# randa1/orleans

Measured on AMD Instinct MI355X. Metric: routed grain messages/sec (node), higher is better.
Workload: dtype u32/u64 integer; 1 GPU; config3: Zipf(1.1) over 16M long-key grains, 256M messages in total (256M per GPU), 8-silo ring, stages 1-4; grains=16000000, messages_total=268435456, messages_per_gpu=268435456, silos=8, ring=balanced (silo generations [5, 135, 167, 28, 221, 184, 42, 48]), parallelism=directory sharded by ring range over 1 GPU(s)

## Files before the change

### include/orleans_route.h

```cpp
#ifndef ORLEANS_ROUTE_H
#define ORLEANS_ROUTE_H

#include <stddef.h>
#include <stdint.h>

#ifdef __cplusplus
extern "C" {
#endif

#define ORL_ABI_VERSION 1u
#define ORL_MAX_SILOS 255u
#define ORL_NULL_SILO 0xFFu
#define ORL_NO_ACT 0xFFFFFFFFu
#define ORL_MAX_RING 256u

#define ORL_OK 0
#define ORL_E_INVALID (-1)
#define ORL_E_NOMEM (-2)
#define ORL_E_DEVICE (-3)
#define ORL_E_CAPACITY (-4)
#define ORL_E_STATE (-5)
#define ORL_E_OVERFLOW (-6)

#define ORL_CAT_NONE 0u
// ... 459 lines not shown
    uint64_t max_recv;
    uint32_t chunks;
    uint32_t flags;
} orl_node_config;

typedef struct orl_node_result {
    uint64_t n_owned;
    uint64_t n_hosted;
    uint64_t n_forwarded;
    uint64_t n_sent_remote;
    uint32_t hop2;
    uint32_t n_segments;
    const uint32_t* route;
    const uint32_t* act;
    const uint32_t* order;
    const uint32_t* bucket_offsets;
} orl_node_result;

typedef struct orl_node orl_node;
int orl_node_unique_id(uint8_t id[ORL_NODE_ID_BYTES]);
int orl_node_create(orl_ctx* ctx, const orl_node_config* cfg, orl_node** out);
int orl_node_destroy(orl_node* node);
const char* orl_node_last_error(const orl_node* node);
int orl_node_set_timeout(orl_node* node, uint32_t ms);
int orl_node_route_batch_device(orl_node* node, const orl_msg_hdr* d_in, size_t n, uint32_t opts, orl_node_result* out,
                                void* stream);
int orl_node_route_batch_keyext_device(orl_node* node, const orl_msg_hdr* d_in, size_t n, uint32_t opts, const orl_ext_ref* d_ext,
                                       const uint8_t* d_blob, uint64_t blob_bytes, orl_node_result* out, void* stream);
int orl_node_fanout_batch_device(orl_node* node, const uint64_t* d_csr_off, const uint32_t* d_csr_tgt,
                                 const orl_grain_key* d_follower_keys, uint64_t follower_tcd, const uint32_t* d_pubs,
                                 const uint8_t* d_pub_silo, size_t n_pub, uint32_t opts, uint64_t* d_pub_offsets,
                                 uint64_t* total, orl_node_result* out, void* stream);
int orl_node_segment(const orl_node* node, uint32_t i, const void** d_records, uint64_t* count, uint32_t* width);
typedef struct orl_node_stats {
    uint32_t comm_count;
    uint32_t chunks;
    uint64_t bytes_sent[ORL_NODE_MAX_RANKS];
    uint64_t host_wait_us;
    uint64_t host_waits;
    uint32_t exchange_mode;
    uint32_t reserved;
} orl_node_stats;
#define ORL_NODE_MODE_SPLIT_COMM 0x1u
#define ORL_NODE_MODE_HEAD_STREAM 0x2u
int orl_node_get_stats(const orl_node* node, orl_node_stats* out);

#define ORL_NODE_HEAD_WORDS 16u
typedef struct orl_node_chunk_plan {
    uint32_t width;
    uint32_t rewrite;
    uint64_t send[ORL_NODE_MAX_RANKS];
    uint64_t recv[ORL_NODE_MAX_RANKS];
    uint64_t n_recv;
    uint32_t act_lane;
    uint32_t ext_lane;
} orl_node_chunk_plan;
int orl_node_plan_chunk(const uint64_t* heads, uint32_t nranks, uint32_t me, uint32_t written, uint64_t max_recv,
                        uint64_t* owned_total, orl_node_chunk_plan* out);
typedef struct orl_node_hop2_plan {
    uint32_t forward;
    uint32_t width;
    uint64_t send[ORL_NODE_MAX_RANKS];
    uint64_t recv[ORL_NODE_MAX_RANKS];
    uint64_t n_hosted;
    uint64_t n_forwarded;
} orl_node_hop2_plan;
int orl_node_plan_hop2(const uint64_t* heads, uint32_t nranks, uint32_t me, uint64_t n_owned, uint32_t width_mask,
                       uint64_t max_recv, orl_node_hop2_plan* out);

int orl_sync(orl_ctx* ctx);

#define ORL_Q_PROBE_FORM 1u
#define ORL_Q_FULL_UPLOADS 2u
#define ORL_Q_SLOT_PATCHES 3u
#define ORL_Q_DEVICE 4u
#define ORL_Q_N_ACT 5u
#define ORL_Q_MAX_BATCH 6u
#define ORL_Q_RANK_MODE 7u
#define ORL_Q_WIRE_DIGEST 8u
#define ORL_Q_PART_ERROR 9u
#define ORL_Q_HOT_KEY 10u
#define ORL_Q_HOT_BATCHES 11u
#define ORL_Q_STAGE4_ERROR 12u
int orl_ctx_query(orl_ctx* ctx, uint32_t what, uint64_t* value);
int orl_ctx_set_rank_mode(orl_ctx* ctx, uint32_t mode);

#define ORL_TIMING_SLOTS 256u
int orl_set_timing(orl_ctx* ctx, int enable);
int orl_timing_summary(const orl_ctx* ctx, uint32_t* n_batches, float* route_kernel_ms, float* bucket_ms,
                       float* total_ms);

#ifdef __cplusplus
}
#endif
#endif
```

### orleans_amd/_lib.py

```python
from __future__ import annotations

import ctypes as C
import os

import numpy as np

LIB_NAME = "liborleans_route.so"
LIB_PATH = os.path.join(os.path.dirname(os.path.abspath(__file__)), LIB_NAME)

ABI_VERSION = 1
NULL_SILO = 0xFF
NO_ACT = 0xFFFFFFFF

OK, E_INVALID, E_NOMEM, E_DEVICE, E_CAPACITY, E_STATE, E_OVERFLOW = 0, -1, -2, -3, -4, -5, -6

CAT_NONE, CAT_SYSTEM_TARGET, CAT_SYSTEM_GRAIN, CAT_GRAIN, CAT_CLIENT, CAT_KEYEXT_GRAIN = 0, 1, 2, 3, 4, 6

HDR_ADDRESS_COMPLETE = 0x01
HDR_HASH_VALID = 0x02

ST_HIT = 0
ST_NEW_PLACEMENT = 1
ST_SYSTEM_TARGET = 2
ST_ADDRESS_COMPLETE = 3
ST_OWNER_NULL = 4
ST_NO_SEED = 5
ST_CLIENT_UNREGISTERED = 6
ST_KEYEXT_UNRESOLVED = 7
ST_REMOTE_OWNER = 8
ST_PAST_TOTAL = 9

RF_NEW_PLACEMENT = 0x01
RF_LOOPBACK = 0x02
RF_OWNER_IS_SEED = 0x04

POLICY_PREFER_LOCAL = 0
POLICY_HASH_SPREAD = 1

OPT_EXCLUDE_IF_STOPPING = 0x1
OPT_NO_BUCKETS = 0x2
OPT_TOTAL_GIVEN = 0x4
SPLIT_REMOVE = 0x1
RF_CACHED = 0x08
RF_CACHE_STALE = 0x10
RF_STATELESS = 0x20
MAX_SW_TYPES = 8
SW_MAX_LOCAL = 8
SW_ADDED, SW_DUPLICATE, SW_UNSUPPORTED = 0, 1, 2
RING_CONSISTENT, RING_VBUCKETS = 0, 1
CACHE_EVICT_DEVICE, CACHE_EVICT_HOST = 0, 1
CACHE_NO_ETAG = -1
TICKS_PER_SECOND = 10_000_000
OUTQ_LOOPBACK, OUTQ_PING, OUTQ_SYSTEM, OUTQ_REJECT, OUTQ_OVERFLOW, OUTQ_UNKNOWN_SILO = (
    0xFFFFFFF0, 0xFFFFFFF1, 0xFFFFFFF2, 0xFFFFFFF3, 0xFFFFFFF4, 0xFFFFFFF5)
DEC_OK, DEC_UNSUPPORTED, DEC_MALFORMED, DEC_UNKNOWN_SILO, DEC_NO_TARGET, DEC_NO_SENDER = 0, 1, 2, 3, 4, 5
SENDER_FROM_HEADER = 0xFF
STAMP_OK, STAMP_COMPLETE, STAMP_SKIPPED, STAMP_UNSUPPORTED, STAMP_MALFORMED, STAMP_OVERFLOW = 0, 1, 2, 3, 4, 5
STAMP_MAX_GROWTH = 72
MERGE_INSERTED, MERGE_KEPT, MERGE_REPLACED, MERGE_SAME, MERGE_DUPLICATE, MERGE_UNSUPPORTED = 0, 1, 2, 3, 4, 5
DIR_NO_ETAG = -1
LUM_UNCHANGED, LUM_ABSENT, LUM_UPDATED, LUM_UPDATED_EMPTY, LUM_UNSUPPORTED = 0, 1, 2, 3, 4

ACT_CREATE, ACT_ACTIVATING, ACT_VALID, ACT_DEACTIVATING, ACT_INVALID, ACT_ABSENT = 0, 1, 2, 3, 4, 5
ACTF_REENTRANT, ACTF_RUNNING_SET, ACTF_RUNNING_RO, ACTF_STATELESS = 0x01, 0x02, 0x04, 0x08
MF_DIR_MASK, MF_REQUEST, MF_RESPONSE, MF_ONE_WAY = 0x03, 0, 1, 2
MF_READ_ONLY, MF_ALWAYS_INTERLEAVE, MF_EXPIRED = 0x04, 0x08, 0x10
(ADM_RUN, ADM_ENQUEUE, ADM_RESPONSE, ADM_OVERLOADED, ADM_INVALID, ADM_NONEXISTENT, ADM_EXPIRED,
 ADM_UNRESOLVED) = range(8)
TOK_NONE, TOK_DRAIN = 0xFFFFFFFF, 0xFFFFFFFE
WQ_RUN, WQ_DRAINED = 0, 1
(CMP_COMPLETIONS, CMP_PUMPS, CMP_DRAINS, CMP_IGNORED, CMP_UNDERFLOWS, CMP_RUN, CMP_DRAINED,
 CMP_WAITING) = range(8)
COLF_EXEMPT, COLF_CANCELLED = 0x01, 0x02
COL_MOVED, COL_SAME, COL_EXPIRED, COL_CANCELLED_DROPPED, COL_BAD_TIMEOUT = 1, 2, 3, 4, 5
COL_TOUCHED, COL_RULE1_ONLY, COL_RULE7_ONLY = 0, 6, 7
COL_BECAME_IDLE, COL_IGNORED, COL_COMPLETIONS = 0, 6, 7
(SCAN_CANDIDATES, SCAN_BAD_STATE, SCAN_KEPT_ALIVE, SCAN_ACTIVE, SCAN_NOT_STALE, SCAN_CONDEMNED, SCAN_CANCELLED_SKIPPED,
 SCAN_UNSCHEDULED) = range(8)
(SCHED_DONE, SCHED_EXEMPT, SCHED_AGE_ZERO, SCHED_BAD_TIMEOUT, SCHED_TICKETED, SCHED_IGNORED) = range(6)
(CANCEL_DONE, CANCEL_EXEMPT, CANCEL_NO_TICKET, CANCEL_EXPIRED, CANCEL_ALREADY, CANCEL_IGNORED) = range(6)

Q_PROBE_FORM, Q_FULL_UPLOADS, Q_SLOT_PATCHES, Q_DEVICE, Q_N_ACT, Q_MAX_BATCH, Q_RANK_MODE = 1, 2, 3, 4, 5, 6, 7
Q_WIRE_DIGEST = 8
Q_PART_ERROR = 9
PART_CACHED = 0x8
Q_HOT_KEY = 10
Q_HOT_BATCHES = 11
Q_STAGE4_ERROR = 12
MAX_WIRE_TYPES = 16
PART_LOOKBACK_FAILED = 0x4
PART_KEYEXT = 0x10
PART_EXT_FULL = 0x20

INS_INSERTED, INS_EXISTING, INS_INVALID_SILO, INS_REMOTE_OWNER, INS_OWNER_NULL, INS_UNSUPPORTED = 0, 1, 2, 3, 4, 5

KEY_DTYPE = np.dtype([("tcd", "<u8"), ("n0", "<u8"), ("n1", "<u8")])
EXT_REF_DTYPE = np.dtype([("off", "<u4"), ("len", "<u4")])
MSG_DTYPE = np.dtype([("tcd", "<u8"), ("n0", "<u8"), ("n1", "<u8"), ("sending_silo", "u1"), ("category", "u1"),
                      ("flags", "u1"), ("target_silo", "u1"), ("aux", "<u4")])
assert KEY_DTYPE.itemsize == 24 and MSG_DTYPE.itemsize == 32
ACT_STATE_DTYPE = np.dtype([("state", "u1"), ("flags", "u1"), ("reserved", "<u2"), ("num_running", "<u4"),
                            ("in_flight", "<u4"), ("waiting", "<u4")])
assert ACT_STATE_DTYPE.itemsize == 16


class orl_config(C.Structure):
    _fields_ = [("abi_version", C.c_uint32), ("device", C.c_int32), ("dir_capacity", C.c_uint64),
                ("n_act", C.c_uint32), ("placement_policy", C.c_uint32), ("max_batch", C.c_uint64)]


NODE_ID_BYTES = 128
TRANSPORT_RCCL, TRANSPORT_LOCAL = 0, 1
NODE_WIDE_ONLY = 0x1
NODE_SPLIT_COMM = 0x2
NODE_MODE_SPLIT_COMM = 0x1
NODE_MODE_HEAD_STREAM = 0x2
NODE_MAX_RANKS = 8
NODE_MAX_CHUNKS = 16
NODE_HEAD_WORDS = 16


class orl_node_config(C.Structure):
    _fields_ = [("abi_version", C.c_uint32), ("nranks", C.c_uint32), ("rank", C.c_uint32), ("transport", C.c_uint32),
                ("group_id", C.c_uint8 * NODE_ID_BYTES), ("rank_of_silo", C.c_uint8 * 256), ("max_batch", C.c_uint64),
                ("max_recv", C.c_uint64), ("chunks", C.c_uint32), ("flags", C.c_uint32)]


class orl_node_result(C.Structure):
    _fields_ = [("n_owned", C.c_uint64), ("n_hosted", C.c_uint64), ("n_forwarded", C.c_uint64),
                ("n_sent_remote", C.c_uint64), ("hop2", C.c_uint32), ("n_segments", C.c_uint32), ("route", C.c_void_p),
                ("act", C.c_void_p), ("order", C.c_void_p), ("bucket_offsets", C.c_void_p)]


class orl_node_stats(C.Structure):
    _fields_ = [("comm_count", C.c_uint32), ("chunks", C.c_uint32), ("bytes_sent", C.c_uint64 * NODE_MAX_RANKS),
                ("host_wait_us", C.c_uint64), ("host_waits", C.c_uint64), ("exchange_mode", C.c_uint32),
                ("reserved", C.c_uint32)]


class orl_cache_stats(C.Structure):
    _fields_ = [("entries", C.c_uint64), ("tombstones", C.c_uint64), ("evictions", C.c_uint64),
                ("evict_batches", C.c_uint64), ("rebuilds", C.c_uint64), ("host_fallbacks", C.c_uint64)]


class orl_cache_sweep(C.Structure):
    _fields_ = [("d_keys", C.c_void_p), ("d_etags", C.c_void_p), ("d_owner_offsets", C.c_void_p), ("d_counts", C.c_void_p)]


class orl_admit_limits(C.Structure):
    _fields_ = [("hard", C.c_int32), ("hard_stateless", C.c_int32)]


class orl_waitq_view(C.Structure):
    _fields_ = [("d_off", C.c_void_p), ("d_tok", C.c_void_p), ("d_act", C.c_void_p), ("d_mflags", C.c_void_p),
                ("d_running_tok", C.c_void_p), ("d_out_tok", C.c_void_p), ("d_out_act", C.c_void_p),
                ("d_out_mflags", C.c_void_p), ("d_out_kind", C.c_void_p), ("d_out_n", C.c_void_p),
                ("d_waiting_n", C.c_void_p)]


class orl_collector_view(C.Structure):
    _fields_ = [("d_ticket", C.c_void_p), ("d_became_idle", C.c_void_p), ("d_keep_alive_until", C.c_void_p),
                ("d_age_limit", C.c_void_p), ("d_cflags", C.c_void_p), ("d_out_act", C.c_void_p), ("d_out_n", C.c_void_p),
                ("quantum", C.c_int64), ("next_ticket", C.c_int64)]


class orl_node_chunk_plan(C.Structure):
    _fields_ = [("width", C.c_uint32), ("rewrite", C.c_uint32), ("send", C.c_uint64 * NODE_MAX_RANKS),
                ("recv", C.c_uint64 * NODE_MAX_RANKS), ("n_recv", C.c_uint64), ("act_lane", C.c_uint32),
                ("ext_lane", C.c_uint32)]


# ... 196 lines not shown
```

### orleans_amd/csrc/orl_api.cpp

```cpp
#include <hip/hip_runtime.h>

#include <algorithm>
#include <cstdarg>
#include <cstdlib>
#include <cstdio>
#include <cstring>
#include <map>
#include <mutex>
#include <new>
#include <string>
#include <tuple>
#include <vector>

#include "orl_internal.h"
#include "cache_adaptive.h"
#include "admit.h"
#include "waitq.h"
#include "collect.h"
#include "dir_versions.h"
#include "cache_evict.h"

using namespace orl;

namespace {
// ... 758 lines not shown
        return ORL_E_NOMEM;
    }
    c->mask = slots - 1;
    rebuild_params(c);
    if (cfg->device >= 0) {
        c->device_mode = true;
        auto bail = [&](hipError_t e, const char* what) {
            int r = hipfail(c, e, what);
            free_device(c);
            delete c;
            return r;
        };
        hipError_t e;
        if ((e = hipSetDevice(cfg->device)) != hipSuccess) return bail(e, "hipSetDevice");
        if ((e = hipStreamCreateWithFlags(&c->stream, hipStreamNonBlocking)) != hipSuccess) return bail(e, "hipStreamCreate");
        if ((e = (hipError_t)ensure_rank_mode(cfg->device)) != hipSuccess) return bail(e, "stage-4 rank self-check");
        if ((e = hipMalloc((void**)&c->d_table, slots * sizeof(DirSlot))) != hipSuccess) return bail(e, "hipMalloc(directory)");
        if ((e = hipMalloc((void**)&c->d_probe, slots * sizeof(ProbeSlot))) != hipSuccess) return bail(e, "hipMalloc(probe table)");
        if ((e = hipMalloc((void**)&c->d_probe_bad, 4)) != hipSuccess) return bail(e, "hipMalloc(probe flag)");
        if ((e = hipMalloc((void**)&c->d_probe8, slots * 8)) != hipSuccess) return bail(e, "hipMalloc(probe table 8)");
        const char* np = getenv("ORL_NO_PROBE16");
        c->probe_off = np && np[0] == '1';
        const char* np8 = getenv("ORL_NO_PROBE8");
        c->probe8_off = np8 && np8[0] == '1';
        if ((e = hipMalloc((void**)&c->d_claim, slots * 4)) != hipSuccess) return bail(e, "hipMalloc(claim)");
        if ((e = hipMemset(c->d_claim, 0xFF, slots * 4)) != hipSuccess) return bail(e, "hipMemset(claim)");
        if ((e = hipMalloc((void**)&c->d_vr_hash, ORL_MAX_SILOS * ORL_MAX_VBUCKETS_PER_SILO * 4)) != hipSuccess)
            return bail(e, "hipMalloc(vring)");
        if ((e = hipMalloc((void**)&c->d_vr_silo, ORL_MAX_SILOS * ORL_MAX_VBUCKETS_PER_SILO)) != hipSuccess)
            return bail(e, "hipMalloc(vring silos)");
        if ((e = hipMalloc((void**)&c->d_silo_hash, 1024)) != hipSuccess) return bail(e, "hipMalloc(silo hashes)");
        if ((e = hipMalloc((void**)&c->d_silo_known, 256)) != hipSuccess) return bail(e, "hipMalloc(silo known)");
        if ((e = hipMalloc((void**)&c->d_silo_tab, kSiloAddrSlots * sizeof(SiloAddrEntry))) != hipSuccess)
            return bail(e, "hipMalloc(silo addresses)");
        if ((e = hipMalloc((void**)&c->d_decode_flag, 4)) != hipSuccess) return bail(e, "hipMalloc(decode flag)");
        if ((e = hipMalloc((void**)&c->d_silo_words, 256 * 24)) != hipSuccess) return bail(e, "hipMalloc(silo words)");
        if ((e = hipMalloc((void**)&c->d_gt, kGrainTypeSlots * sizeof(GrainTypeEntry))) != hipSuccess)
            return bail(e, "hipMalloc(grain types)");
        if ((e = hipMalloc((void**)&c->d_gt_blob, kGrainTypeBlob)) != hipSuccess) return bail(e, "hipMalloc(grain type names)");
        if ((e = hipMalloc((void**)&c->d_dirstate, 32)) != hipSuccess) return bail(e, "hipMalloc(dirstate)");
        if ((e = hipMemset(c->d_dirstate, 0, 32)) != hipSuccess) return bail(e, "hipMemset(dirstate)");
        if ((e = hipMalloc((void**)&c->d_params, sizeof(RouteParams))) != hipSuccess) return bail(e, "hipMalloc(params)");
        if ((e = hipMalloc((void**)&c->d_rank_of_silo, 256)) != hipSuccess) return bail(e, "hipMalloc(rank map)");
        const uint64_t mb = std::max<uint64_t>(cfg->max_batch, kTile);
        const uint64_t tiles = (mb + kTile - 1) / kTile;
        c->s.max_batch = mb;
        c->s.max_tiles = tiles;
        c->s.device = cfg->device;
        c->s.gap_cap = env_gap_cap();
        c->s.fan_u = env_fan_u();
        const uint64_t rows = std::max<uint64_t>(tiles, std::min<uint64_t>(kMaxRouteRows, (mb + 255) / 256));
        const uint64_t hist_words = (1ull << kMaxDigitBits) * rows;
        if ((e = hipMalloc((void**)&c->s.pairs_a, mb * 8)) != hipSuccess) return bail(e, "hipMalloc(pairs_a)");
        if ((e = hipMalloc((void**)&c->s.pairs_b, mb * 8)) != hipSuccess) return bail(e, "hipMalloc(pairs_b)");
        if ((e = hipMalloc((void**)&c->s.idx_a, (mb + 1) * 4)) != hipSuccess) return bail(e, "hipMalloc(idx)");
        if ((e = hipMalloc((void**)&c->s.sorted_keys, mb * 4)) != hipSuccess) return bail(e, "hipMalloc(sorted)");
        if ((e = hipMalloc((void**)&c->s.tile_hist, hist_words * 4)) != hipSuccess) return bail(e, "hipMalloc(tile_hist)");
        if ((e = hipMalloc((void**)&c->s.tile_cnt, hist_words * 2)) != hipSuccess) return bail(e, "hipMalloc(tile_cnt)");
        const uint64_t scan_words = std::max<uint64_t>(std::max<uint64_t>(hist_words, mb + 1), (uint64_t)cfg->n_act + 2);
        if ((e = hipMalloc((void**)&c->s.scan_sums, ((scan_words + 4095) / 4096 + 2) * 4)) != hipSuccess) return bail(e, "hipMalloc(scan)");
        const BucketPlan bp = make_bucket_plan(cfg->n_act);
        const uint64_t seg_rows = std::max<uint64_t>(max_segments(mb, bp.hb), max_segments(std::min<uint64_t>(mb, (16u << 20) - 1), bp.hb));
        const uint64_t seg_words = bp.two_level ? seg_rows << bp.lb : 1;
        if ((e = hipMalloc((void**)&c->s.seg_hist, seg_words * 4)) != hipSuccess) return bail(e, "hipMalloc(seg_hist)");
        const uint64_t lb_cap = bp.two_level ? (seg_rows + kSegLbMinRows - 1) / kSegLbMinRows + 1 : 1;
        c->s.seg_lb_cap = (uint32_t)lb_cap;
        const uint64_t carry_words = bp.two_level ? lb_cap << bp.lb : 1;
        if ((e = hipMalloc((void**)&c->s.seg_carry, carry_words * 4)) != hipSuccess) return bail(e, "hipMalloc(seg_carry)");
        if ((e = hipMalloc((void**)&c->s.seg_meta, (lb_cap + 1) * 4)) != hipSuccess) return bail(e, "hipMalloc(seg_meta)");
        if ((e = hipMalloc((void**)&c->s.seg_lb, 2 * carry_words * 4)) != hipSuccess) return bail(e, "hipMalloc(seg_lb)");
        if ((e = hipMalloc((void**)&c->s.seg_lbctl, (4 + lb_cap) * 4)) != hipSuccess) return bail(e, "hipMalloc(seg_lbctl)");
        if ((e = hipMemset(c->s.seg_lbctl, 0, (4 + lb_cap) * 4)) != hipSuccess) return bail(e, "hipMemset(seg_lbctl)");
        if ((e = hipMalloc((void**)&c->s.bstart, 4097 * 4)) != hipSuccess) return bail(e, "hipMalloc(bstart)");
        c->s.fan_blk_cap = (uint32_t)((mb + 255) / 256 + 2);
        if ((e = hipMalloc((void**)&c->s.fan_blk, (size_t)c->s.fan_blk_cap * 4)) != hipSuccess) return bail(e, "hipMalloc(fan_blk)");
        if ((e = hipMalloc((void**)&c->s.sstart, 4098 * 4)) != hipSuccess) return bail(e, "hipMalloc(sstart)");
        if ((e = hipMalloc((void**)&c->d_dslot, mb * 4)) != hipSuccess) return bail(e, "hipMalloc(dslot)");
        if ((e = hipMalloc((void**)&c->d_dflag, mb)) != hipSuccess) return bail(e, "hipMalloc(dflag)");
        for (auto& L : c->s.lb) {
            if ((e = hipMalloc((void**)&L.state, 16 + ((mb + 2047) / 2048) * 64)) != hipSuccess) return bail(e, "hipMalloc(lb_state)");
            if ((e = hipMemset(L.state, 0, 16 + ((mb + 2047) / 2048) * 64)) != hipSuccess) return bail(e, "hipMemset(lb_state)");
            if ((e = hipEventCreateWithFlags(&L.ev, hipEventDisableTiming)) != hipSuccess) return bail(e, "hipEventCreate(lb)");
        }
        if (const char* lh = getenv("ORL_LSD_HOT"); lh && lh[0] == '1')
            if ((e = hipMalloc((void**)&c->s.lsd_hot, 16)) != hipSuccess) return bail(e, "hipMalloc(lsd_hot)");
        if ((e = hipMalloc((void**)&c->s.s4_err, 4)) != hipSuccess) return bail(e, "hipMalloc(s4_err)");
        if ((e = hipMemset(c->s.s4_err, 0, 4)) != hipSuccess) return bail(e, "hipMemset(s4_err)");
        if ((e = hipMalloc((void**)&c->s.gap_q, kGapQueueWords * 4)) != hipSuccess) return bail(e, "hipMalloc(gap_q)");
        if ((e = hipMemset(c->s.gap_q, 0, kGapQueueWords * 4)) != hipSuccess) return bail(e, "hipMemset(gap_q)");
        if ((e = hipMalloc((void**)&c->s.digits, mb)) != hipSuccess) return bail(e, "hipMalloc(digits)");
        if ((e = hipMalloc((void**)&c->s.col_sums, ((rows + 63) / 64) * (1ull << kMaxDigitBits) * 4)) != hipSuccess)
            return bail(e, "hipMalloc(col_sums)");
        if ((e = hipMalloc((void**)&c->s.col_tot, ((1ull << kMaxDigitBits) + 1) * 4)) != hipSuccess) return bail(e, "hipMalloc(col_tot)");
        if ((e = hipMalloc((void**)&c->s.hot, 16)) != hipSuccess) return bail(e, "hipMalloc(hot)");
        {
            const uint32_t init[4] = {0xFFFFFFFFu, 0xFFFFFFFFu, 0u, 0u};
            if ((e = hipMemcpy(c->s.hot, init, 16, hipMemcpyHostToDevice)) != hipSuccess) return bail(e, "hipMemcpy(hot)");
        }
        if ((e = hipMalloc((void**)&c->s.hot_bmax, (((uint64_t)cfg->n_act + 2 + 4095) / 4096 + 1) * 8)) != hipSuccess)
            return bail(e, "hipMalloc(hot_bmax)");
        if ((e = hipMalloc((void**)&c->s.pick_word, 8)) != hipSuccess) return bail(e, "hipMalloc(pick_word)");
        if ((e = hipMemset(c->s.pick_word, 0, 8)) != hipSuccess) return bail(e, "hipMemset(pick_word)");
        if ((e = hipMalloc((void**)&c->s.hot_rows, (rows + (rows + 63) / 64 + 1) * 4)) != hipSuccess) return bail(e, "hipMalloc(hot_rows)");
        if ((e = hipHostMalloc((void**)&c->s.hot_host, 8, hipHostMallocMapped | hipHostMallocCoherent)) != hipSuccess)
            return bail(e, "hipHostMalloc(hot_host)");
        c->s.hot_host[0] = 0xFFFFFFFFu;
        c->s.hot_host[1] = 1u;
        if ((e = hipHostGetDevicePointer((void**)&c->s.hot_host_dev, c->s.hot_host, 0)) != hipSuccess)
            return bail(e, "hipHostGetDevicePointer(hot_host)");
        if ((e = hipMalloc((void**)&c->st_off, ((size_t)cfg->n_act + 2) * 4)) != hipSuccess) return bail(e, "hipMalloc(offsets)");
    }
    *out = c;
    return ORL_OK;
}

int orl_ctx_destroy(orl_ctx* c) {
    if (!c) return ORL_E_INVALID;
    if (c->device_mode) {
        (void)hipSetDevice(c->cfg.device);
        (void)hipStreamSynchronize(c->stream);
        free_device(c);
    }
    delete c;
    return ORL_OK;
}

const char* orl_last_error(const orl_ctx* c) { return c ? c->err.c_str() : "null context"; }

int orl_silos_set(orl_ctx* c, uint32_t n, const uint8_t* running, const uint8_t* functional, const uint8_t* local,
                  uint32_t seed) {
    if (!c) return ORL_E_INVALID;
    if (n == 0 || n > ORL_MAX_SILOS) return fail(c, ORL_E_INVALID, "n_silos must be in [1, %u]", ORL_MAX_SILOS);
    if (seed != ORL_NULL_SILO && seed >= n) return fail(c, ORL_E_INVALID, "seed %u out of range", seed);
    for (auto& e : c->ring)
        if (e.second >= n) return fail(c, ORL_E_STATE, "ring holds silo %u >= n_silos", e.second);
    c->n_silos = n;
    c->running.assign(n, 1); c->functional.assign(n, 1); c->local.assign(n, 1);
    for (uint32_t i = 0; i < n; ++i) {
        if (running) c->running[i] = running[i] ? 1 : 0;
        if (functional) c->functional[i] = functional[i] ? 1 : 0;
        if (local) c->local[i] = local[i] ? 1 : 0;
    }
    c->seed = seed;
    rebuild_params(c);
    return ORL_OK;
}

int orl_ring_add_server(orl_ctx* c, uint32_t silo, int32_t hash) {
    if (!c) return ORL_E_INVALID;
    if (!silo_ok(c, silo)) return fail(c, ORL_E_INVALID, "silo %u not in the silo table (call orl_silos_set first)", silo);
    for (auto& e : c->ring)
        if (e.second == silo) return ORL_OK;
    if (c->ring.size() >= ORL_MAX_RING) return fail(c, ORL_E_CAPACITY, "ring full");
    int idx = -1;
    for (int i = 0; i < (int)c->ring.size(); ++i)
        if (c->ring[i].first < hash) idx = i;
    c->ring.insert(c->ring.begin() + (idx + 1), std::make_pair(hash, (uint8_t)silo));
    c->silo_hash[silo] = hash;
    c->silo_known[silo] = 1;
    c->silo_hash_dirty = true;
    rebuild_params(c);
    return ORL_OK;
}

int orl_silo_hash_set(orl_ctx* c, uint32_t silo, int32_t hash) {
    if (!c) return ORL_E_INVALID;
    if (silo >= 256) return fail(c, ORL_E_INVALID, "silo %u out of range", silo);
    c->silo_hash[silo] = hash;
    c->silo_known[silo] = 1;
    c->silo_hash_dirty = true;
    return ORL_OK;
}

int orl_ring_remove_server(orl_ctx* c, uint32_t silo) {
    if (!c) return ORL_E_INVALID;
    auto it = std::find_if(c->ring.begin(), c->ring.end(), [&](const std::pair<int32_t, uint8_t>& e) { return e.second == silo; });
    if (it != c->ring.end()) c->ring.erase(it);
    rebuild_params(c);
    return ORL_OK;
}

int orl_ring_get(const orl_ctx* c, int32_t* hashes, uint8_t* silos, uint32_t cap, uint32_t* n_out) {
    if (!c || !n_out) return ORL_E_INVALID;
    *n_out = (uint32_t)c->ring.size();
    for (uint32_t i = 0; i < c->ring.size() && i < cap; ++i) {
        if (hashes) hashes[i] = c->ring[i].first;
        if (silos) silos[i] = c->ring[i].second;
    }
    return ORL_OK;
// ... 2195 lines not shown
    ORL_HIP(c, hipDeviceSynchronize());
    (void)hipFree(c->d_csr_off); (void)hipFree(c->d_csr_tgt);
    c->d_csr_off = nullptr; c->d_csr_tgt = nullptr; c->csr_nodes = 0;
    ORL_HIP(c, hipMalloc((void**)&c->d_csr_off, (n_nodes + 1) * 8));
    ORL_HIP(c, hipMalloc((void**)&c->d_csr_tgt, std::max<size_t>(n_edges, 1) * 4));
    ORL_HIP(c, hipMemcpy(c->d_csr_off, off, (n_nodes + 1) * 8, hipMemcpyHostToDevice));
    if (n_edges) ORL_HIP(c, hipMemcpy(c->d_csr_tgt, tgt, n_edges * 4, hipMemcpyHostToDevice));
    c->csr_nodes = n_nodes;
    c->h_csr_off.assign(off, off + n_nodes + 1);
    return ORL_OK;
}

int orl_fanout_batch(orl_ctx* c, const uint32_t* pubs, const uint8_t* pub_silo, size_t n_pub, uint64_t follower_tcd,
                     uint32_t opts, uint64_t* pub_offsets, uint32_t* route, uint32_t* act, uint32_t* order, uint32_t* offsets,
                     size_t cap, uint64_t* n_out) {
    if (!c || !n_out || !pub_offsets) return ORL_E_INVALID;
    if (!c->device_mode) return fail(c, ORL_E_STATE, "context was created without a device (device < 0)");
    if (!c->d_csr_off) return fail(c, ORL_E_STATE, "no follower graph (orl_csr_set)");
    const bool buckets = !(opts & ORL_OPT_NO_BUCKETS);
    if (n_pub && (!pubs || !pub_silo)) return fail(c, ORL_E_INVALID, "null publisher array");
    if (!route || !act || (buckets && (!order || !offsets))) return fail(c, ORL_E_INVALID, "null output array");
    uint64_t total = 0;
    for (size_t p = 0; p < n_pub; ++p) {
        if (pubs[p] >= c->csr_nodes) return fail(c, ORL_E_INVALID, "publisher %u >= %zu nodes", pubs[p], c->csr_nodes);
        total += c->h_csr_off[pubs[p] + 1] - c->h_csr_off[pubs[p]];
    }
    *n_out = total;
    if (total > cap) return fail(c, ORL_E_CAPACITY, "fan-out emits %llu > cap %zu", (unsigned long long)total, cap);
    if (total > c->s.max_batch || n_pub + 1 > c->s.max_batch) return fail(c, ORL_E_CAPACITY, "fan-out larger than max_batch");
    ORL_HIP(c, hipSetDevice(c->cfg.device));
    const size_t in_bytes = n_pub * 5 + 16, out_words = 3 * std::max<uint64_t>(total, 1) + 1 + 2 * (n_pub + 1);
    if (int r = ensure_staging(c, in_bytes, out_words)) return r;
    uint32_t* d_pubs = reinterpret_cast<uint32_t*>(c->st_in);
    uint8_t* d_psilo = c->st_in + ((n_pub * 4 + 15) & ~size_t(15));
    uint32_t* d_route = c->st_out;
    uint32_t* d_act = d_route + total;
    uint32_t* d_order = d_act + total;
    uint64_t* d_poff = reinterpret_cast<uint64_t*>(d_order + total + (total & 1));
    hipStream_t st = c->stream;
    if (n_pub) {
        ORL_HIP(c, hipMemcpyAsync(d_pubs, pubs, n_pub * 4, hipMemcpyHostToDevice, st));
        ORL_HIP(c, hipMemcpyAsync(d_psilo, pub_silo, n_pub, hipMemcpyHostToDevice, st));
    }
    uint64_t n_dev = total;
    int r = orl_fanout_route_device(c, c->d_csr_off, c->d_csr_tgt, d_pubs, d_psilo, n_pub, follower_tcd, opts | ORL_OPT_TOTAL_GIVEN,
                                    d_poff, d_route, d_act, d_order, c->st_off, &n_dev, st);
    if (r) return r;
    if (total) {
        ORL_HIP(c, hipMemcpyAsync(route, d_route, total * 4, hipMemcpyDeviceToHost, st));
        ORL_HIP(c, hipMemcpyAsync(act, d_act, total * 4, hipMemcpyDeviceToHost, st));
        if (buckets) ORL_HIP(c, hipMemcpyAsync(order, d_order, total * 4, hipMemcpyDeviceToHost, st));
    }
    ORL_HIP(c, hipMemcpyAsync(pub_offsets, d_poff, (n_pub + 1) * 8, hipMemcpyDeviceToHost, st));
    if (buckets) ORL_HIP(c, hipMemcpyAsync(offsets, c->st_off, ((size_t)c->cfg.n_act + 2) * 4, hipMemcpyDeviceToHost, st));
    ORL_HIP(c, hipStreamSynchronize(st));
    return ORL_OK;
}

int orl_ctx_query(orl_ctx* c, uint32_t what, uint64_t* v) {
    if (!c || !v) return ORL_E_INVALID;
    switch (what) {
        case ORL_Q_DEVICE: *v = (uint64_t)(int64_t)c->cfg.device; return ORL_OK;
        case ORL_Q_N_ACT: *v = c->cfg.n_act; return ORL_OK;
        case ORL_Q_MAX_BATCH: *v = c->s.max_batch; return ORL_OK;
        case ORL_Q_WIRE_DIGEST: *v = c->hp.wire_digest; return ORL_OK;
        case ORL_Q_RANK_MODE: {
            if (!c->device_mode) return fail(c, ORL_E_STATE, "no device");
            std::lock_guard<std::mutex> lk(g_rank_mu);
            *v = (uint64_t)(int64_t)g_rank_state[c->cfg.device];
            return ORL_OK;
        }
        case ORL_Q_HOT_BATCHES:
            *v = c->s.hot_batches;
            return ORL_OK;
        case ORL_Q_HOT_KEY: {
            if (!c->device_mode) return fail(c, ORL_E_STATE, "no device");
            ORL_HIP(c, hipSetDevice(c->cfg.device));
            ORL_HIP(c, hipDeviceSynchronize());
            uint32_t w = 0;
            ORL_HIP(c, hipMemcpy(&w, c->s.hot + (c->s.hot_parity & 1u), 4, hipMemcpyDeviceToHost));
            *v = w;
            return ORL_OK;
        }
        case ORL_Q_PART_ERROR: {
            if (!c->device_mode) return fail(c, ORL_E_STATE, "no device");
            ORL_HIP(c, hipSetDevice(c->cfg.device));
            ORL_HIP(c, hipDeviceSynchronize());
            uint32_t any = 0;
            for (auto& L : c->s.lb) {
                uint32_t w = 0;
                ORL_HIP(c, hipMemcpy(&w, L.state + 1, 4, hipMemcpyDeviceToHost));
                if (w) ORL_HIP(c, hipMemset(L.state + 1, 0, 4));
                any |= w;
            }
            *v = any ? 1u : 0u;
            return ORL_OK;
        }
        case ORL_Q_STAGE4_ERROR: {
            if (!c->device_mode) return fail(c, ORL_E_STATE, "no device");
            ORL_HIP(c, hipSetDevice(c->cfg.device));
            ORL_HIP(c, hipDeviceSynchronize());
            uint32_t w = 0;
            ORL_HIP(c, hipMemcpy(&w, c->s.s4_err, 4, hipMemcpyDeviceToHost));
            if (w) ORL_HIP(c, hipMemset(c->s.s4_err, 0, 4));
            *v = w ? 1u : 0u;
            return ORL_OK;
        }
        default: break;
    }
    if (int r = sync_device_state(c)) return r;
    switch (what) {
        case ORL_Q_PROBE_FORM:
            *v = c->probe8_valid ? 8 : c->probe_valid ? 16 : (c->probe_dev || c->probe_dev_stale) ? 17 : 32;
            return ORL_OK;
        case ORL_Q_FULL_UPLOADS: *v = c->n_full_uploads; return ORL_OK;
        case ORL_Q_SLOT_PATCHES: *v = c->n_patches; return ORL_OK;
        default: return fail(c, ORL_E_INVALID, "unknown query %u", what);
    }
}

int orl_ctx_set_rank_mode(orl_ctx* c, uint32_t mode) {
    if (!c || mode > 1) return ORL_E_INVALID;
    if (!c->device_mode) return fail(c, ORL_E_STATE, "no device");
    std::lock_guard<std::mutex> lk(g_rank_mu);
    const int st = g_rank_state[c->cfg.device];
    if (mode == 0 && (st & 2)) return fail(c, ORL_E_STATE, "the LDS lane-order self-check failed on this device: ballot ranking only");
    ORL_HIP(c, hipSetDevice(c->cfg.device));
    ORL_HIP(c, hipDeviceSynchronize());
    ORL_HIP(c, (hipError_t)set_rank_mode(c->cfg.device, mode));
    g_rank_state[c->cfg.device] = (int)(mode | (st & 2));
    return ORL_OK;
}

int orl_set_timing(orl_ctx* c, int enable) {
    if (!c) return ORL_E_INVALID;
    if (!c->device_mode) return fail(c, ORL_E_STATE, "no device");
    if (enable && c->tev.empty()) {
        c->tev.assign(4 * (size_t)ORL_TIMING_SLOTS, nullptr);
        for (auto& e : c->tev) ORL_HIP(c, hipEventCreate(&e));
    }
    c->timing = enable != 0;
    c->tcount = 0;
    return ORL_OK;
}

int orl_timing_summary(const orl_ctx* cc, uint32_t* n_batches, float* route_ms, float* bucket_ms, float* total_ms) {
    orl_ctx* c = const_cast<orl_ctx*>(cc);
    if (!c) return ORL_E_INVALID;
    if (n_batches) *n_batches = c->tcount;
    if (c->tcount == 0) return fail(c, ORL_E_STATE, "no timed batch");
    ORL_HIP(c, hipEventSynchronize(c->tev[4 * (size_t)(c->tcount - 1) + 3]));
    double a = 0, b = 0, t = 0;
    for (uint32_t i = 0; i < c->tcount; ++i) {
        const hipEvent_t* ev = &c->tev[4 * (size_t)i];
        float x = 0, y = 0, z = 0;
        ORL_HIP(c, hipEventElapsedTime(&x, ev[1], ev[2]));
        ORL_HIP(c, hipEventElapsedTime(&y, ev[2], ev[3]));
        ORL_HIP(c, hipEventElapsedTime(&z, ev[0], ev[3]));
        a += x; b += y; t += z;
    }
    if (route_ms) *route_ms = (float)(a / c->tcount);
    if (bucket_ms) *bucket_ms = (float)(b / c->tcount);
    if (total_ms) *total_ms = (float)(t / c->tcount);
    return ORL_OK;
}

// ... 2 lines not shown
```

### orleans_amd/csrc/orl_internal.h

```cpp
#pragma once

#include <hip/hip_runtime.h>
#include <stddef.h>
#include <stdint.h>
#include <stdlib.h>

#include <algorithm>

#include "../../include/orleans_route.h"

namespace orl {

enum : uint8_t { SLOT_EMPTY = 0, SLOT_FULL = 1, SLOT_TOMB = 2,
                 SLOT_CLAIMING = 3,
                 SLOT_CLAIMED = 4 };

struct alignas(32) DirSlot {
    uint64_t tcd;
    uint64_t n0;
    uint64_t n1;
    uint32_t act;
    uint8_t silo;
    uint8_t state;
    uint16_t pad;
// ... 157 lines not shown
    while ((max_key >> total) != 0 && total < 32) ++total;
    if (total == 0) total = 1;
    BucketPlan p{};
    p.two_level = total <= 2 * (int)kMaxDigitBits;
    static const bool lb_ceil = [] { const char* e = getenv("ORL_LB_CEIL"); return e && e[0] == '1'; }();
    p.lb = total <= (int)kMaxDigitBits ? total : lb_ceil ? (total + 1) / 2 : total / 2;
    p.hb = total - p.lb;
    p.lsd = make_plan(max_key);
    return p;
}

inline uint32_t seg_elems(uint64_t) { return kSegChunk; }
inline uint64_t max_segments(uint64_t n, int hb) {
    const uint64_t s = seg_elems(n);
    return (n + s - 1) / s + std::min<uint64_t>(1ull << hb, n);
}

inline uint64_t pad_to(uint64_t v, uint64_t m) { return (v + m - 1) / m * m; }

struct Carve {
    uint8_t* p;
    explicit Carve(void* base) : p(static_cast<uint8_t*>(base)) {}
    template <class T = uint8_t>
    T* take(uint64_t bytes) {
        T* r = reinterpret_cast<T*>(p);
        p += bytes;
        return r;
    }
};

struct SegAgg;

struct DirView {
    const DirSlot* dir;
    uint64_t mask;
    const DirSlot* cache;
    uint64_t cmask;
    const ProbeSlot* probe = nullptr;
    const uint32_t* probe_bad = nullptr;
    const void* probe8 = nullptr;
    bool lru = false;
};

struct CacheAdaptive {
    int64_t* ttl;
    int64_t* last_refreshed;
    unsigned long long* seen;
    int32_t* etag;
};
__host__ __device__ inline CacheAdaptive cache_adaptive(const DirSlot* cache, uint64_t mask) {
    const uint64_t slots = mask + 1;
    uint8_t* p = reinterpret_cast<uint8_t*>(const_cast<DirSlot*>(cache + slots)) + (slots + 1) * 8;
    CacheAdaptive a;
    a.ttl = reinterpret_cast<int64_t*>(p);
    a.last_refreshed = a.ttl + slots;
    a.seen = reinterpret_cast<unsigned long long*>(a.last_refreshed + slots);
    a.etag = reinterpret_cast<int32_t*>(a.seen + slots);
    return a;
}
inline size_t cache_table_bytes(uint64_t slots, bool adaptive) {
    return slots * sizeof(DirSlot) + (slots + 1) * 8 + (adaptive ? slots * 28 : 0);
}
struct CacheFresh {
    const int32_t* etags = nullptr;
    int64_t now = 0;
    int64_t initial_ttl = 0;
    uint32_t on = 0;
    uint32_t pad = 0;
};

struct DirTags {
    int32_t* slot = nullptr;
    const int32_t* in = nullptr;
    const int32_t* draws = nullptr;
    int32_t* winner = nullptr;
};

struct ExtSlot {
    uint64_t tcd, n0, n1;
    uint32_t hash, act, off, len;
    uint8_t silo, state, pad[6];
};
static_assert(sizeof(ExtSlot) == 48, "KeyExt slot layout");

constexpr uint32_t kSegLbMinRows = 8;

struct Scratch {
    uint2* pairs_a;
    uint2* pairs_b;
    uint32_t* idx_a;
    uint32_t* sorted_keys;
    uint32_t* tile_hist;
    uint16_t* tile_cnt;
    uint32_t* scan_sums;
    uint32_t* col_sums;
    uint32_t* col_tot;
    uint8_t* digits;
    uint32_t* seg_hist;
    uint32_t* seg_carry;
    uint32_t* seg_meta;
    uint32_t* seg_lb = nullptr;
    uint32_t* seg_lbctl = nullptr;
    uint32_t seg_lb_cap = 0;
    mutable uint32_t seg_epoch = 0;
    uint32_t* bstart;
    uint32_t* sstart;
    uint32_t* gap_q;
    struct LbSet {
        uint32_t* state = nullptr;
        uint32_t ticket = 0;
        uint32_t epoch = 0;
        hipStream_t stream = nullptr;
        hipEvent_t ev = nullptr;
        uint64_t last = 0;
    };
    static constexpr int kLbSets = 2;
    LbSet lb[kLbSets];
    uint64_t lb_clock = 0;
    uint64_t max_batch;
    uint64_t max_tiles;
    int device = -1;
    uint32_t* hot = nullptr;
    mutable uint32_t hot_parity = 0;
    unsigned long long* hot_bmax = nullptr;
    unsigned long long* pick_word = nullptr;
    uint32_t* hot_rows = nullptr;
    uint32_t* lsd_hot = nullptr;
    uint32_t* hot_host = nullptr;
    uint32_t* hot_host_dev = nullptr;
    mutable uint64_t hot_batches = 0;
    uint32_t* fan_blk = nullptr;
    uint32_t fan_blk_cap = 0;
    uint32_t gap_cap = 4096;
    int fan_u = 1;
    uint32_t* s4_err = nullptr;
};

uint32_t env_gap_cap();
int env_fan_u();

int launch_hash(const orl_grain_key* d_keys, size_t n, uint32_t* d_out, void* stream);
int launch_rank_selfcheck(int device, int mode, uint32_t* ballot_out);
int set_rank_mode(int device, uint32_t ballot);
int launch_dir_patch(const uint32_t* d_idx, const DirSlot* d_slots, const ProbeSlot* d_p16, const uint2* d_p8, uint32_t n,
                     DirSlot* d_dir, ProbeSlot* d_probe, uint2* d_probe8, void* stream);
int launch_probe_build(const DirSlot* d_dir, uint64_t slots, const RouteParams* d_params, ProbeSlot* d_probe,
                       uint32_t* d_bad, void* stream);
int launch_route_bucket(const RouteParams* d_params, const DirView& dv,
                        const void* d_in, int fmt, size_t n, uint32_t opts, uint32_t n_act, uint32_t* d_route,
                        uint32_t* d_act, uint32_t* d_order, uint32_t* d_offsets, const Scratch& s, void* stream,
                        void* ev_route_begin, void* ev_route_end, const uint32_t* d_in_act = nullptr,
                        const SwView* sw = nullptr);
int launch_fanout_route_bucket(const RouteParams* d_params, const DirView& dv, const orl_msg_hdr* d_direct, size_t n_direct,
                               const uint64_t* d_csr_off, const uint32_t* d_csr_tgt, const orl_grain_key* d_follower_keys,
                               const uint32_t* d_pubs, const uint8_t* d_pub_silo, size_t n_pub, uint64_t follower_tcd,
                               uint32_t opts, uint32_t n_act, uint64_t* d_pub_offsets, uint32_t* d_route, uint32_t* d_act,
                               uint32_t* d_order, uint32_t* d_offsets, uint64_t* n_out, uint64_t max_out,
                               const Scratch& s, void* stream, void* ev_route_begin, void* ev_route_end);
int launch_fanout_expand(const uint64_t* d_csr_off, const uint32_t* d_csr_tgt, const orl_grain_key* d_follower_keys,
                         const uint32_t* d_pubs, const uint8_t* d_pub_silo, size_t n_pub, uint64_t follower_tcd, uint32_t opts,
                         uint64_t* d_pub_offsets, orl_msg_hdr* d_out, uint64_t* n_out, uint64_t cap, const Scratch& s,
                         void* stream);
int launch_dir_insert(const RouteParams* d_params, DirSlot* d_dir, uint64_t dir_mask, uint32_t* d_claim, uint64_t* d_cnt,
                      const orl_grain_key* d_keys, const uint32_t* d_acts, const uint8_t* d_silos, size_t n, uint32_t n_act,
                      uint32_t n_silos, uint32_t* d_slot, uint32_t* d_wact, uint8_t* d_wsilo, uint8_t* d_status, uint32_t* d_err,
                      void* stream, const DirTags& vt = DirTags{});
// ... 87 lines not shown
```

### orleans_amd/csrc/route_kernels.hip

```cpp
#include <hip/hip_runtime.h>

#include <cstdlib>

#include "dir_table_dev.h"

namespace orl {

namespace {

constexpr uint32_t kWaves = kRouteThreads / 64;

__device__ __forceinline__ uint32_t pack_route(uint32_t owner, uint32_t host, uint32_t st, uint32_t fl) {
    return (owner & 0xFFu) | ((host & 0xFFu) << 8) | ((st & 0xFFu) << 16) | ((fl & 0xFFu) << 24);
}

struct Msg {
    uint64_t tcd, n0, n1;
    uint32_t meta;
    uint32_t aux;
};

using u32x4 = unsigned int __attribute__((ext_vector_type(4)));

__device__ __forceinline__ Msg decode_hdr(const u32x4& a, const u32x4& b) {
// ... 451 lines not shown
                ra = counter_add<true>(&ca[w][0], d, 1u);
                rb = wave_rank_ballot<10, true>(&cb[w][0], d, active, lt);
            } else {
                ra = counter_add<false>(&ca[w][0], d, 1u);
                rb = wave_rank_ballot<3, false>(&cb[w][0], d, active, lt);
            }
            bad |= ra != rb;
        }
        __syncthreads();
    }
    if (bad) atomicOr(err, 1u);
}

__device__ __forceinline__ uint32_t packed_get(const uint32_t* row, uint32_t d) { return (row[d >> 1] >> ((d & 1u) << 4)) & 0xFFFFu; }

__global__ __launch_bounds__(256) void k_probe_build(const DirSlot* __restrict__ dir, uint64_t slots,
                                                     const RouteParams* __restrict__ gp, ProbeSlot* __restrict__ probe,
                                                     uint32_t* __restrict__ bad) {
    __shared__ uint64_t types[kProbeTypes];
    __shared__ uint32_t nt;
    if (threadIdx.x < kProbeTypes) types[threadIdx.x] = gp->probe_tcd[threadIdx.x];
    if (threadIdx.x == 0) nt = gp->n_probe_types;
    __syncthreads();
    const uint32_t ntypes = nt;
    bool miss = false;
    for (uint64_t i = (uint64_t)blockIdx.x * 256u + threadIdx.x; i < slots; i += (uint64_t)gridDim.x * 256u) {
        const u32x4* d4 = reinterpret_cast<const u32x4*>(dir + i);
        const u32x4 a = d4[0], b = d4[1];
        const uint32_t st = (b.w >> 8) & 0xFFu;
        const uint64_t tcd = (uint64_t)a.x | ((uint64_t)a.y << 32);
        uint32_t t = 0;
        u32x4 q = {0u, 0u, 0u, st == SLOT_EMPTY ? (uint32_t)SLOT_EMPTY : (uint32_t)SLOT_TOMB};
        if (st == SLOT_FULL) {
            while (t < ntypes && types[t] != tcd) ++t;
            if (t == ntypes || (a.z | a.w) != 0u) {
                miss = true;
                t = 0;
            }
            q = u32x4{b.x, b.y, b.z, (uint32_t)SLOT_FULL | ((b.w & 0xFFu) << 8) | (t << 16)};
        }
        reinterpret_cast<u32x4*>(probe)[i] = q;
    }
    if (miss) atomicOr(bad, 1u);
}

__global__ __launch_bounds__(256) void k_dir_patch(const uint32_t* __restrict__ idx, const DirSlot* __restrict__ slots,
                                                   const ProbeSlot* __restrict__ p16, const uint2* __restrict__ p8, uint32_t n,
                                                   DirSlot* __restrict__ dir, ProbeSlot* __restrict__ probe,
                                                   uint2* __restrict__ probe8) {
    const uint32_t k = blockIdx.x * 256u + threadIdx.x;
    if (k >= n) return;
    const uint32_t i = idx[k];
    dir[i] = slots[k];
    if (probe) probe[i] = p16[k];
    if (probe8) probe8[i] = p8[k];
}

__global__ __launch_bounds__(256) void k_hash(const orl_grain_key* __restrict__ keys, uint32_t n, uint32_t* __restrict__ out) {
    const uint32_t i = blockIdx.x * blockDim.x + threadIdx.x;
    if (i < n) out[i] = jenkins3(keys[i].type_code_data, keys[i].n0, keys[i].n1);
}

__device__ __forceinline__ void store_drop(uint32_t* p, uint32_t v) {
#ifdef ORL_ROUTE_STORE_SC1
    __hip_atomic_store(p, v, __ATOMIC_RELAXED, __HIP_MEMORY_SCOPE_AGENT);
#else
    __builtin_nontemporal_store(v, p);
#endif
}

template <int HB>
struct RouteSmem {
    RouteParams P;
    uint32_t hist[HB ? (1u << HB) : 1u];
    uint32_t hot;
};

constexpr uint32_t kNoHotKey = 0xFFFFFFFFu;

__device__ __forceinline__ uint32_t hot_key_of(const uint32_t* hot) {
    return hot ? __builtin_amdgcn_readfirstlane(__hip_atomic_load(hot, __ATOMIC_RELAXED, __HIP_MEMORY_SCOPE_AGENT)) : kNoHotKey;
}

__device__ __forceinline__ void wave_add_hot(uint32_t* dst, uint32_t mine) {
    uint32_t v = mine;
#pragma unroll
    for (uint32_t d = 32; d >= 1; d >>= 1) v += (uint32_t)__shfl_xor((int)v, (int)d, 64);
    if ((threadIdx.x & 63u) == 0 && v) atomicAdd(dst, v);
}

template <int FMT>
__device__ __forceinline__ Msg load_msg(const RouteParams& P, const void* __restrict__ in, uint32_t e) {
    if (FMT == 16) return load_wire(static_cast<const orl_wire_msg*>(in), e);
    if (FMT == 8) return load_narrow(P, static_cast<const orl_wire8*>(in), e);
    return load_hdr(static_cast<const orl_msg_hdr*>(in), e);
}

#ifndef ORL_ROUTE_PF
#define ORL_ROUTE_PF 1
#endif
template <int FMT>
__device__ __forceinline__ void pf_record(const void* __restrict__ in, uint32_t e, u32x4* region) {
    using lds_t = __attribute__((address_space(3))) void*;
    if (FMT == 32) {
        const u32x4* g = reinterpret_cast<const u32x4*>(static_cast<const orl_msg_hdr*>(in) + e);
        __builtin_amdgcn_global_load_lds(g, (lds_t)region, 16, 0, 2);
        __builtin_amdgcn_global_load_lds(g + 1, (lds_t)(region + 64), 16, 0, 2);
    } else if (FMT == 16) {
        __builtin_amdgcn_global_load_lds(static_cast<const orl_wire_msg*>(in) + e, (lds_t)region, 16, 0, 2);
    } else {
        const uint32_t* g = reinterpret_cast<const uint32_t*>(static_cast<const orl_wire8*>(in) + e);
        __builtin_amdgcn_global_load_lds(g, (lds_t)region, 4, 0, 2);
        __builtin_amdgcn_global_load_lds(g + 1, (lds_t)(reinterpret_cast<uint32_t*>(region) + 64), 4, 0, 2);
    }
}

template <int FMT>
__device__ __forceinline__ Msg pf_decode(const RouteParams& P, const u32x4* region, uint32_t lane) {
    if (FMT == 32) return decode_hdr(region[lane], region[64u + lane]);
    if (FMT == 16) return decode_wire(region[lane]);
    const uint32_t* r = reinterpret_cast<const uint32_t*>(region);
    return decode_narrow(P, (uint64_t)r[lane] | ((uint64_t)r[64u + lane] << 32));
}

#define ORL_SGPR80 __attribute__((amdgpu_num_sgpr(80)))
#ifndef ORL_ROUTE_ATTR
#define ORL_ROUTE_ATTR ORL_SGPR80
#endif
#ifndef ORL_FAN_ATTR
#define ORL_FAN_ATTR __attribute__((amdgpu_num_sgpr(96)))
#endif
#ifndef ORL_PART_ATTR
#define ORL_PART_ATTR
#endif
template <int HB, int FMT, int PW, bool CIN, bool LRU, bool SW>
__device__ __forceinline__ void route_body(const RouteParams* __restrict__ gp, const DirSlot* __restrict__ dir,
                                           uint64_t dmask, const DirSlot* __restrict__ cache, uint64_t cmask,
                                           const ProbeSlot* __restrict__ probe, const uint32_t* __restrict__ probe_bad,
                                           const void* __restrict__ in, uint32_t n, uint32_t excl,
                                           uint32_t* __restrict__ route, uint32_t* __restrict__ act_out,
                                           uint16_t* __restrict__ tile_cnt, uint32_t bins, uint32_t shift, uint32_t items,
                                           const uint32_t* __restrict__ hot_words, uint32_t* __restrict__ hot_rows,
                                           const uint32_t* __restrict__ in_act, const SwView* sw) {
    static_assert(!SW || PW == 0, "the stateless-worker forms read the 32-B directory table");
    __shared__ RouteSmem<HB> sm;
    constexpr bool HIST = HB > 0;
    constexpr bool PF = ORL_ROUTE_PF == 2 || (ORL_ROUTE_PF == 1 && FMT == 32);
    constexpr uint32_t PFW = FMT == 32 ? 128u : FMT == 16 ? 64u : 32u;
    __shared__ u32x4 pre[PF ? kWaves * PFW : 1];
    u32x4* const pregion = pre + (PF ? (threadIdx.x >> 6) * PFW : 0u);
    const uint32_t plane = threadIdx.x & 63u;
    uint32_t pend_e = 0, pend_rr = 0, pend_act = 0;
    bool pend = false;
    stage_params(&sm.P, gp);
    if (HIST)
        for (uint32_t b = threadIdx.x; b < bins; b += blockDim.x) sm.hist[b] = 0;
    if (threadIdx.x == 0) sm.hot = 0;
    __syncthreads();
    const uint32_t n_act = sm.P.n_act;
    const uint32_t hk = (HIST && hot_rows) ? hot_key_of(hot_words) : kNoHotKey;
    uint32_t hot_mine = 0;
    const bool use16 = PW == 16 && (probe_bad == nullptr || *probe_bad == 0u);
    const uint32_t base = blockIdx.x * (kRouteThreads * items) + threadIdx.x;
    if (PF) pf_record<FMT>(in, base < n ? base : n - 1u, pregion);
    for (uint32_t j = 0; j < items; ++j) {
        const uint32_t e = base + j * kRouteThreads;
        Msg m;
        if (PF) {
            asm volatile("s_waitcnt vmcnt(0)" ::: "memory");
            if (pend) {
                store_drop(route + pend_e, pend_rr);
                store_drop(act_out + pend_e, pend_act);
                pend = false;
            }
            m = pf_decode<FMT>(sm.P, pregion, plane);
            asm volatile("s_waitcnt lgkmcnt(0)" ::: "memory");
            if (j + 1u < items) {
                const uint32_t en = e + kRouteThreads;
                pf_record<FMT>(in, en < n ? en : n - 1u, pregion);
            }
        } else if (e < n) {
            m = load_msg<FMT>(sm.P, in, e);
        }
        uint32_t h = 0, own = 0, rf = 0, r = 0;
        uint64_t slot = 0, mask = dmask;
        u32x4 sa, sb;
        const u32x4* dir4 = reinterpret_cast<const u32x4*>(dir);
        if (PW == 8) {
            bool can = false;
            uint2 q;
            uint32_t cact = ORL_NO_ACT, vact = ORL_NO_ACT;
            if (e < n) {
                r = route_head(sm.P, m, excl != 0, h, own, rf);
                if (CIN) r = sender_cached(sm.P, m, in_act[e], h, own, rf, r, cact, vact);
                if (r == kNeedProbe) {
                    can = probe8_key(sm.P, m);
                    slot = dir_slot(h, dmask);
                    if (can) q = reinterpret_cast<const uint2*>(probe)[slot];
                }
            }
            const uint32_t kb = (uint32_t)m.n1;
            int st = 3;
            uint32_t fact = 0, fsilo = 0;
            if (r == kNeedProbe) st = can ? probe_slot8(q, kb, fact, fsilo) : 1;
            for (uint64_t step = 0; st == 2 && step < dmask; ++step) {
                slot = (slot + 1) & dmask;
                q = reinterpret_cast<const uint2*>(probe)[slot];
                st = probe_slot8(q, kb, fact, fsilo);
            }
            if (e < n) {
                uint32_t act = cact, rr = r;
                if (rr == kNeedProbe) {
                    rr = route_tail(sm.P, m, h, own, rf, st == 0, fact, fsilo, act, false);
                    if (CIN) rr = cached_verdict(sm.P, m, h, own, rf, rr, act, vact, st == 0, fact, fsilo);
                } else if (rr == kNeedProbeCache) {
                    rr = route_msg<LRU>(sm.P, dir, dmask, cache, cmask, m, excl != 0, act, e);
                }
                if (PF) {
                    pend_e = e, pend_rr = rr, pend_act = act, pend = true;
                } else {
                    store_drop(route + e, rr);
                    store_drop(act_out + e, act);
                }
                if (HIST) {
                    const uint32_t k = bucket_key(act, n_act);
                    if (k == hk) ++hot_mine;
                    else atomicAdd(&sm.hist[(k >> shift) & (bins - 1)], 1u);
                }
            }
            continue;
        }
        if (use16) {
            uint32_t mk = kNoType;
            uint32_t cact = ORL_NO_ACT, vact = ORL_NO_ACT;
            if (e < n) {
                r = route_head(sm.P, m, excl != 0, h, own, rf);
                if (CIN) r = sender_cached(sm.P, m, in_act[e], h, own, rf, r, cact, vact);
                if (r == kNeedProbe) {
                    mk = probe_type(sm.P, m);
                    slot = dir_slot(h, dmask);
                    if (mk != kNoType) sa = reinterpret_cast<const u32x4*>(probe)[slot];
                }
            }
            int st = 3;
            uint32_t fact = 0, fsilo = 0;
            if (r == kNeedProbe) st = mk == kNoType ? 1 : probe_slot16(sa, m.n1, mk, fact, fsilo);
            for (uint64_t step = 0; st == 2 && step < dmask; ++step) {
                slot = (slot + 1) & dmask;
                sa = reinterpret_cast<const u32x4*>(probe)[slot];
                st = probe_slot16(sa, m.n1, mk, fact, fsilo);
            }
            if (e < n) {
                uint32_t act = cact, rr = r;
                if (rr == kNeedProbe) {
                    rr = route_tail(sm.P, m, h, own, rf, st == 0, fact, fsilo, act, false);
                    if (CIN) rr = cached_verdict(sm.P, m, h, own, rf, rr, act, vact, st == 0, fact, fsilo);
                } else if (rr == kNeedProbeCache) {
                    rr = route_msg<LRU>(sm.P, dir, dmask, cache, cmask, m, excl != 0, act, e);
                }
                if (PF) {
                    pend_e = e, pend_rr = rr, pend_act = act, pend = true;
                } else {
                    store_drop(route + e, rr);
                    store_drop(act_out + e, act);
                }
                if (HIST) {
                    const uint32_t k = bucket_key(act, n_act);
                    if (k == hk) ++hot_mine;
                    else atomicAdd(&sm.hist[(k >> shift) & (bins - 1)], 1u);
                }
            }
            continue;
        }
        uint32_t cact = ORL_NO_ACT, vact = ORL_NO_ACT;
        if (e < n) {
            r = route_head<SW>(sm.P, m, excl != 0, h, own, rf, sw);
            if (SW && r == kStateless) r = sw_route(*sw, m, h, cact);
            else if (CIN) r = sender_cached(sm.P, m, in_act[e], h, own, rf, r, cact, vact);
            if (r >= kNeedProbeCache) {
                if (r == kNeedProbeCache) {
                    dir4 = reinterpret_cast<const u32x4*>(cache);
                    mask = cmask;
                }
                slot = dir_slot(h, mask);
                sa = dir4[2 * slot];
                sb = dir4[2 * slot + 1];
            }
        }
        int st = 3;
        uint32_t fact = 0, fsilo = 0;
        if (r >= kNeedProbeCache) st = probe_slot(sa, sb, m, fact, fsilo);
        for (uint64_t step = 0; st == 2 && step < mask; ++step) {
            slot = (slot + 1) & mask;
            sa = dir4[2 * slot];
            sb = dir4[2 * slot + 1];
            st = probe_slot(sa, sb, m, fact, fsilo);
        }
        if (LRU && r == kNeedProbeCache && st == 0) cache_touch(cache, cmask, slot, e);
        if (e < n) {
            uint32_t act = cact, rr = r;
            if (rr >= kNeedProbeCache) {
                const bool vc = rr == kNeedProbeCache;
                rr = route_tail(sm.P, m, h, own, rf, st == 0, fact, fsilo, act, vc);
                if (CIN && !vc) rr = cached_verdict(sm.P, m, h, own, rf, rr, act, vact, st == 0, fact, fsilo);
            }
            if (PF) {
                pend_e = e, pend_rr = rr, pend_act = act, pend = true;
            } else {
                store_drop(route + e, rr);
                store_drop(act_out + e, act);
            }
            if (HIST) {
                const uint32_t k = bucket_key(act, n_act);
                if (k == hk) ++hot_mine;
                else atomicAdd(&sm.hist[(k >> shift) & (bins - 1)], 1u);
            }
        }
    }
    if (PF && pend) {
        store_drop(route + pend_e, pend_rr);
        store_drop(act_out + pend_e, pend_act);
    }
    if (HIST) {
        if (hot_rows) wave_add_hot(&sm.hot, hot_mine);
        __syncthreads();
        store_count_row(tile_cnt + (size_t)blockIdx.x * bins, sm.hist, bins);
        if (hot_rows && threadIdx.x == 0) hot_rows[blockIdx.x] = sm.hot;
    }
}

template <int HB, int FMT, int PW, bool CIN = false, bool LRU = false>
__global__ __launch_bounds__(kRouteThreads) ORL_ROUTE_ATTR void k_route(const RouteParams* __restrict__ gp, const DirSlot* __restrict__ dir,
                                                         uint64_t dmask, const DirSlot* __restrict__ cache, uint64_t cmask,
                                                         const ProbeSlot* __restrict__ probe,
                                                         const uint32_t* __restrict__ probe_bad,
                                                         const void* __restrict__ in, uint32_t n,
                                                         uint32_t excl, uint32_t* __restrict__ route,
                                                         uint32_t* __restrict__ act_out, uint16_t* __restrict__ tile_cnt,
                                                         uint32_t bins, uint32_t shift, uint32_t items,
                                                         const uint32_t* __restrict__ hot_words, uint32_t* __restrict__ hot_rows,
                                                         const uint32_t* __restrict__ in_act) {
    route_body<HB, FMT, PW, CIN, LRU, false>(gp, dir, dmask, cache, cmask, probe, probe_bad, in, n, excl, route, act_out, tile_cnt,
                                             bins, shift, items, hot_words, hot_rows, in_act, nullptr);
}

template <int HB, int FMT, bool CIN = false, bool LRU = false>
__global__ __launch_bounds__(kRouteThreads) ORL_ROUTE_ATTR void k_route_sw(const RouteParams* __restrict__ gp, const DirSlot* __restrict__ dir,
                                                            uint64_t dmask, const DirSlot* __restrict__ cache, uint64_t cmask,
                                                            const void* __restrict__ in, uint32_t n,
                                                            uint32_t excl, uint32_t* __restrict__ route,
                                                            uint32_t* __restrict__ act_out, uint16_t* __restrict__ tile_cnt,
                                                            uint32_t bins, uint32_t shift, uint32_t items,
                                                            const uint32_t* __restrict__ hot_words, uint32_t* __restrict__ hot_rows,
                                                            const uint32_t* __restrict__ in_act, SwView sw) {
    route_body<HB, FMT, 0, CIN, LRU, true>(gp, dir, dmask, cache, cmask, nullptr, nullptr, in, n, excl, route, act_out, tile_cnt,
                                           bins, shift, items, hot_words, hot_rows, in_act, &sw);
}

constexpr uint32_t kScanChunk = 4096;

__device__ __forceinline__ uint32_t wave_incl_scan(uint32_t v) {
    const uint32_t lane = threadIdx.x & 63u;
#pragma unroll
    for (uint32_t d = 1; d < 64; d <<= 1) {
        const uint32_t t = __shfl_up(v, d, 64);
        if (lane >= d) v += t;
    }
    return v;
}

__device__ __forceinline__ uint32_t block_excl_scan(uint32_t v, uint32_t* wsum, uint32_t& total) {
    const uint32_t lane = threadIdx.x & 63u, w = threadIdx.x >> 6;
    const uint32_t incl = wave_incl_scan(v);
    if (lane == 63) wsum[w] = incl;
    __syncthreads();
    uint32_t pre = 0;
    total = 0;
    for (uint32_t i = 0; i < kWaves; ++i) {
        const uint32_t s = wsum[i];
        if (i < w) pre += s;
        total += s;
    }
    __syncthreads();
    return pre + incl - v;
}

__device__ __forceinline__ unsigned long long wave_max_u64(unsigned long long v) {
#pragma unroll
    for (uint32_t d = 32; d >= 1; d >>= 1) {
        const unsigned long long o = __shfl_xor(v, (int)d, 64);
        v = o > v ? o : v;
    }
    return v;
}

template <int SRC, uint32_t CH = kScanChunk>
__global__ __launch_bounds__(256) void k_scan_reduce(uint32_t* __restrict__ a, uint64_t m, uint32_t* __restrict__ sums,
                                                     const uint64_t* __restrict__ csr_off, const uint32_t* __restrict__ pubs,
                                                     uint64_t* __restrict__ pstart, unsigned long long* __restrict__ bmax = nullptr,
                                                     uint32_t nkeys = 0, uint32_t* __restrict__ zero_p = nullptr,
                                                     uint32_t zero_n = 0) {
    __shared__ uint32_t wsum[kWaves];
    __shared__ unsigned long long wmax[kWaves];
    for (uint32_t i = blockIdx.x * 256u + threadIdx.x; i < zero_n; i += gridDim.x * 256u) zero_p[i] = 0;
    const uint64_t base = (uint64_t)blockIdx.x * CH;
    constexpr uint32_t J = CH / 256;
    uint32_t s = 0;
    if (SRC != 1) {
        unsigned long long best = 0;
#pragma unroll
        for (uint32_t j = 0; j < J; ++j) {
            const uint64_t e = base + j * 256 + threadIdx.x;
            const uint32_t v = e < m ? a[e] : 0u;
            s += v;
            if (SRC == 2 && e < nkeys) {
                const unsigned long long c = ((unsigned long long)v << 32) | (uint32_t)e;
                best = c > best ? c : best;
            }
        }
        if (SRC == 2) {
            best = wave_max_u64(best);
            if ((threadIdx.x & 63u) == 0) wmax[threadIdx.x >> 6] = best;
            __syncthreads();
            if (threadIdx.x == 0) {
                for (uint32_t q = 1; q < kWaves; ++q) best = wmax[q] > best ? wmax[q] : best;
// ... 91 lines not shown
        unsigned long long best = 0;
        for (uint32_t i = threadIdx.x; i < gridDim.x; i += 256) best = bmax[i] > best ? bmax[i] : best;
        best = wave_max_u64(best);
        if ((threadIdx.x & 63u) == 0) wmax[threadIdx.x >> 6] = best;
        __syncthreads();
        if (threadIdx.x == 0) {
            for (uint32_t q = 1; q < kWaves; ++q) best = wmax[q] > best ? wmax[q] : best;
            const uint32_t c = (uint32_t)(best >> 32), k = (uint32_t)best;
            const uint32_t key = ((uint64_t)c * kHotShare >= n && c >= kHotMinCount) ? k : kNoHotKey;
            __hip_atomic_store(next_key, key, __ATOMIC_RELAXED, __HIP_MEMORY_SCOPE_AGENT);
            if (host_word) __hip_atomic_store(host_word, key, __ATOMIC_RELAXED, __HIP_MEMORY_SCOPE_SYSTEM);
        }
    }
    constexpr int E = (int)(CH / 256);
    const uint64_t base = (uint64_t)blockIdx.x * CH + (uint64_t)threadIdx.x * E;
    uint32_t v[E];
    load_e<E>(a, base, m, 0u, v);
    uint32_t s = 0;
#pragma unroll
    for (int i = 0; i < E; ++i) s += v[i];
    uint32_t pre;
    if (DIRECT) {
        uint32_t q = 0;
        for (uint32_t i = threadIdx.x; i < blockIdx.x; i += 256) q += sums[i];
        block_excl_scan(q, wsum, pre);
    } else {
        pre = sums[blockIdx.x];
    }
    uint32_t total;
    uint32_t run = block_excl_scan(s, wsum, total) + pre;
    uint32_t o[E];
#pragma unroll
    for (int i = 0; i < E; ++i) {
        o[i] = run;
        const bool live = base + i < m;
        if (WIDEN && live) out64[base + i] = add64 + run;
        if (WIDEN && fblk) {
            const uint32_t k0 = (run + kFanBlk - 1u) >> kFanBlkShift;
            uint32_t k1 = k0;
            if (live && base + i + 1 < m)
                k1 = (uint32_t)std::min<uint64_t>(((uint64_t)run + v[i] + kFanBlk - 1u) >> kFanBlkShift, fblk_cap);
            else if (live && m > 1 && k0 < fblk_cap)
                fblk[k0] = (uint32_t)(m - 2);
            const uint32_t cnt = k1 > k0 ? k1 - k0 : 0u;
            if (cnt <= kFblkSerial)
                for (uint32_t k = k0; k < k1; ++k) fblk[k] = (uint32_t)(base + i);
            uint64_t big = __ballot(cnt > kFblkSerial);
            while (big) {
                const int src = __builtin_ctzll(big);
                big &= big - 1;
                const uint32_t b0 = __shfl(k0, src, 64), b1 = __shfl(k1, src, 64);
                const uint32_t p = __shfl((uint32_t)(base + i), src, 64);
                for (uint32_t k = b0 + (threadIdx.x & 63u); k < b1; k += 64u) fblk[k] = p;
            }
        }
        run += v[i];
    }
    store_e<E>(a, base, m, o);
}

#ifndef ORL_STAGE4_NT
#define ORL_STAGE4_NT 1
#endif
__device__ __forceinline__ uint32_t ld_s4(const uint32_t* p) {
    if (ORL_STAGE4_NT) return __builtin_nontemporal_load(p);
    return *p;
}
__device__ __forceinline__ uint2 ld_s4(const uint2* p) {
    using v2 = unsigned int __attribute__((ext_vector_type(2)));
    if (ORL_STAGE4_NT) {
        const v2 v = __builtin_nontemporal_load(reinterpret_cast<const v2*>(p));
        return make_uint2(v.x, v.y);
    }
    return *p;
}
__device__ __forceinline__ uint4 ld_s4(const uint4* p) {
    if (ORL_STAGE4_NT) {
        const u32x4 v = __builtin_nontemporal_load(reinterpret_cast<const u32x4*>(p));
        return make_uint4(v.x, v.y, v.z, v.w);
    }
    return *p;
}

template <bool ACTS>
__global__ __launch_bounds__(256) void k_hist_pairs(const void* __restrict__ in, uint32_t n, uint32_t n_act, uint32_t shift,
                                                    uint32_t bins, uint16_t* __restrict__ tile_cnt,
                                                    const uint32_t* __restrict__ hot_words = nullptr,
                                                    uint32_t* __restrict__ hot_rows = nullptr,
                                                    const uint32_t* __restrict__ n_dev = nullptr) {
    if (n_dev) n = min(__builtin_amdgcn_readfirstlane(__hip_atomic_load(n_dev, __ATOMIC_RELAXED, __HIP_MEMORY_SCOPE_AGENT)), n);
    __shared__ uint32_t hist[1u << kMaxDigitBits];
    __shared__ uint32_t hot;
    for (uint32_t b = threadIdx.x; b < bins; b += 256) hist[b] = 0;
    if (threadIdx.x == 0) hot = 0;
    __syncthreads();
    const uint32_t hk = (ACTS && hot_rows) ? hot_key_of(hot_words) : kNoHotKey;
    uint32_t hot_mine = 0;
    const uint32_t base = blockIdx.x * kTile;
    uint32_t k[kItems];
    if (ACTS) {
#pragma unroll
        for (uint32_t j = 0; j < kItems; ++j) {
            const uint32_t e = base + j * 256 + threadIdx.x;
            k[j] = bucket_key(ld_s4(static_cast<const uint32_t*>(in) + (e < n ? e : n - 1)), n_act);
        }
#pragma unroll
        for (uint32_t j = 0; j < kItems; ++j)
            if (base + j * 256 + threadIdx.x < n) {
                if (k[j] == hk) ++hot_mine;
                else atomicAdd(&hist[(k[j] >> shift) & (bins - 1)], 1u);
            }
        if (hot_rows) wave_add_hot(&hot, hot_mine);
    } else {
        const uint32_t lane = threadIdx.x & 63u;
#pragma unroll
        for (uint32_t j = 0; j < kItems; ++j) {
            const uint32_t e = base + j * 256 + threadIdx.x;
            k[j] = ld_s4(static_cast<const uint2*>(in) + (e < n ? e : (n ? n - 1 : 0u))).x;
        }
#pragma unroll
        for (uint32_t j = 0; j < kItems; ++j) {
            const uint32_t e = base + j * 256 + threadIdx.x;
            const uint32_t d = e < n ? (k[j] >> shift) & (bins - 1) : 0xFFFFFFFFu;
            const uint32_t prev = __shfl_up(d, 1, 64);
            const bool head = lane == 0 || d != prev;
            const uint64_t heads = __ballot(head);
            if (head && d != 0xFFFFFFFFu) {
                const uint64_t after = lane == 63 ? 0ull : heads >> (lane + 1);
                const uint32_t len = after ? (uint32_t)__builtin_ctzll(after) + 1u : 64u - lane;
                atomicAdd(&hist[d], len);
            }
        }
    }
    __syncthreads();
    store_count_row(tile_cnt + (size_t)blockIdx.x * bins, hist, bins);
    if (ACTS && hot_rows && threadIdx.x == 0) hot_rows[blockIdx.x] = hot;
}

template <uint32_t Q = 4, uint32_t TW = 1>
__global__ __launch_bounds__(256) void k_hist_dig8_wave(const uint8_t* __restrict__ dig, uint32_t n, uint32_t bins,
                                                        uint32_t ntiles, uint16_t* __restrict__ tile_cnt,
                                                        const uint32_t* __restrict__ n_dev) {
    constexpr uint32_t PL = 16u * Q;
    if (n_dev) n = min(__builtin_amdgcn_readfirstlane(__hip_atomic_load(n_dev, __ATOMIC_RELAXED, __HIP_MEMORY_SCOPE_AGENT)), n);
    __shared__ uint32_t hist[kWaves][256];
    const uint32_t lane = threadIdx.x & 63u, w = threadIdx.x >> 6;
    const uint32_t tile0 = (blockIdx.x * kWaves + w) * TW;
    if (tile0 >= ntiles) return;
    uint32_t* h = hist[w];
    uint32_t v[TW][4 * Q];
#pragma unroll
    for (uint32_t tw = 0; tw < TW; ++tw) {
        const uint32_t e0 = (tile0 + tw) * (64u * PL) + lane * PL;
        if (e0 + PL <= n) {
            const uint4* p = reinterpret_cast<const uint4*>(dig + e0);
#pragma unroll
            for (uint32_t q = 0; q < Q; ++q) {
                const uint4 x = ld_s4(p + q);
                v[tw][4 * q] = x.x; v[tw][4 * q + 1] = x.y; v[tw][4 * q + 2] = x.z; v[tw][4 * q + 3] = x.w;
            }
        } else {
#pragma unroll
            for (uint32_t q = 0; q < 4 * Q; ++q) v[tw][q] = 0;
            for (uint32_t i = 0; e0 + i < n && i < PL; ++i) v[tw][i >> 2] |= (uint32_t)dig[e0 + i] << (8u * (i & 3u));
        }
    }
#pragma unroll
    for (uint32_t tw = 0; tw < TW; ++tw) {
        const uint32_t tile = tile0 + tw;
        if (tile >= ntiles) break;
#pragma unroll
        for (uint32_t q = 0; q < 4; ++q) h[lane + 64u * q] = 0;
        __builtin_amdgcn_wave_barrier();
        asm volatile("s_waitcnt lgkmcnt(0)" ::: "memory");
        const uint32_t e0 = tile * (64u * PL) + lane * PL;
        const uint32_t m = e0 < n ? min(PL, n - e0) : 0u;
        if (m) {
            uint32_t cur = v[tw][0] & 0xFFu, len = 1;
#pragma unroll
            for (uint32_t i = 1; i < PL; ++i) {
                if (i < m) {
                    const uint32_t b = (v[tw][i >> 2] >> (8u * (i & 3u))) & 0xFFu;
                    if (b == cur) {
                        ++len;
                    } else {
                        atomicAdd(&h[cur], len);
                        cur = b;
                        len = 1;
                    }
                }
            }
            atomicAdd(&h[cur], len);
// ... 72 lines not shown
        tot += v;
    }
    if (d < bins) {
#pragma unroll 8
        for (uint32_t c = c0; c < c1; ++c) {
            const uint32_t v = S[(size_t)c * bins + d];
            S[(size_t)c * bins + d] = pre;
            pre += v;
        }
        if (grp == 0) T[d] = tot;
    }
}

template <uint32_t NT>
__device__ void seg_plan_body(const uint32_t* __restrict__ col_tot, uint32_t nbk, uint32_t n, uint32_t seg,
                              uint32_t* __restrict__ bstart, uint32_t* __restrict__ sstart, uint32_t (*wsum)[16]);

constexpr uint32_t kSelfScanChunks = 64;
constexpr uint32_t kApplyCols = 64;
constexpr uint32_t kApplyGroups = 256 / kApplyCols;
constexpr uint32_t kApplyRows = kScanRows / kApplyGroups;

__global__ __launch_bounds__(256) void k_col_apply(const uint16_t* __restrict__ C, uint32_t* __restrict__ M, uint32_t ntiles, uint32_t bins,
                                                   const uint32_t* __restrict__ S, const uint32_t* __restrict__ T,
                                                   uint32_t row_step, uint32_t* __restrict__ hot_rows, uint32_t plan_n,
                                                   uint32_t plan_seg, uint32_t* __restrict__ plan_bstart,
                                                   uint32_t* __restrict__ plan_sstart) {
    __shared__ uint32_t red;
    __shared__ uint32_t gsum[kApplyGroups][kApplyCols];
    __shared__ uint32_t pw[3][16];
    if (plan_bstart && blockIdx.x == gridDim.x - 1) {
        if (blockIdx.y == 0) seg_plan_body<256>(T, bins, plan_n, plan_seg, plan_bstart, plan_sstart, pw);
        return;
    }
    if (hot_rows && blockIdx.y == gridDim.y - 1) {
        if (threadIdx.x >= 64) return;
        const uint32_t t = blockIdx.x * kScanRows + threadIdx.x;
        const uint32_t v = t < ntiles ? hot_rows[t] : 0u;
        const uint32_t ex = wave_incl_scan(v) - v + hot_rows[ntiles + blockIdx.x];
        if (t < ntiles) hot_rows[t] = ex;
        return;
    }
    const uint32_t col = threadIdx.x % kApplyCols, grp = threadIdx.x / kApplyCols;
    const uint32_t d0 = blockIdx.y * kApplyCols;
    const uint32_t d = d0 + col;
    const bool live = d < bins;
    uint32_t before = 0;
    for (uint32_t i = threadIdx.x; i < d0; i += 256) before += T[i];
    if (threadIdx.x == 0) red = 0;
    const uint32_t t0 = blockIdx.x * kScanRows + grp * kApplyRows;
    const uint32_t t1 = min(t0 + kApplyRows, ntiles);
    uint32_t v[kApplyRows];
#pragma unroll
    for (uint32_t k = 0; k < kApplyRows; ++k) v[k] = live && t0 + k < t1 ? C[(size_t)(t0 + k) * bins + d] : 0u;
    uint32_t rs = 0;
#pragma unroll
    for (uint32_t k = 0; k < kApplyRows; ++k) rs += v[k];
    gsum[grp][col] = rs;
    __syncthreads();
    atomicAdd(&red, before);
    const uint32_t tot_d = live ? T[d] : 0u;
    const uint32_t ex = wave_incl_scan(tot_d) - tot_d;
    uint32_t gpre = 0;
    for (uint32_t g = 0; g < grp; ++g) gpre += gsum[g][col];
    __syncthreads();
    if (!live) return;
    uint32_t run = red + ex + S[(size_t)blockIdx.x * bins + d] + gpre;
#pragma unroll
    for (uint32_t k = 0; k < kApplyRows; ++k) {
        if (t0 + k < t1 && (t0 + k) % row_step == 0) M[(size_t)(t0 + k) * bins + d] = run;
        run += v[k];
    }
}

__device__ __forceinline__ uint32_t xcd_tile(uint32_t b, uint32_t nb) {
#ifdef ORL_NO_XCD_TILE
    return b;
#endif
    const uint32_t q = nb / 8, r = nb % 8, x = b % 8;
    return (x < r ? x * (q + 1) : r * (q + 1) + (x - r) * q) + b / 8;
}

enum : int { IN_ACT = 0, IN_PAIR = 1 };
enum : int { OUT_PAIR = 0, OUT_FINAL = 1, OUT_LSD_PAIR = 4, OUT_PAIR_SMALL = 5, OUT_FINAL_GAPS = 6, OUT_PAIR_DIG = 7 };

__device__ __forceinline__ uint32_t wave_find_pub(const uint32_t* __restrict__ poff, uint32_t n_pub, uint32_t v) {
    const uint32_t lane = threadIdx.x & 63u;
    uint32_t lo = 0, hi = n_pub - 1;
    while (lo < hi) {
        const uint32_t step = (hi - lo + 64u) / 64u;
        const uint32_t sl = min(lo + lane * step, hi);
        const uint64_t le = __ballot(poff[sl] <= v);
        const uint32_t L = 63u - (uint32_t)__builtin_clzll(le);
        const uint32_t nlo = min(lo + L * step, hi);
        if (L < 63u) {
            const uint32_t nx = min(lo + (L + 1u) * step, hi);
            if (nx > nlo) hi = nx - 1u;
        }
        lo = nlo;
    }
    return lo;
}


template <int BITS>
constexpr uint32_t kDigitsPerThread = (1u << BITS) / 256u > 2u ? (1u << BITS) / 256u : 2u;

template <int BITS>
__device__ __forceinline__ void round_starts(uint32_t (*cnt)[(1u << BITS) / 2u], uint32_t* wsum,
                                             uint32_t (&tot)[kDigitsPerThread<BITS>],
                                             uint32_t (&start)[kDigitsPerThread<BITS>]) {
    constexpr uint32_t B = 1u << BITS, P = kDigitsPerThread<BITS>;
    const uint32_t d0 = threadIdx.x * P;
    uint32_t s = 0;
#pragma unroll
    for (uint32_t q = 0; q < P; q += 2) {
        uint32_t lo = 0, hi = 0;
        if (d0 + q < B) {
            const uint32_t k = (d0 + q) >> 1;
#pragma unroll
            for (uint32_t ww = 0; ww < kWaves; ++ww) {
                const uint32_t c = cnt[ww][k];
                cnt[ww][k] = lo | (hi << 16);
                lo += c & 0xFFFFu;
                hi += c >> 16;
            }
        }
        tot[q] = lo;
        tot[q + 1] = hi;
        s += lo + hi;
    }
    uint32_t total;
    uint32_t run = block_excl_scan(s, wsum, total);
#pragma unroll
    for (uint32_t q = 0; q < P; ++q) {
        start[q] = run;
        run += tot[q];
    }
#pragma unroll
    for (uint32_t q = 0; q < P; q += 2) {
        if (d0 + q < B) {
            const uint32_t add = start[q] | (start[q + 1] << 16);
#pragma unroll
            for (uint32_t ww = 0; ww < kWaves; ++ww) cnt[ww][(d0 + q) >> 1] += add;
        }
    }
}

constexpr uint32_t kScatterLdsFloor = 160u * 1024u / 4u + 16u;

template <int BITS, int ITEMS>
struct PassSmemCore {
    uint32_t cnt[kWaves][(1u << BITS) / 2u];
    uint2 stage[256 * ITEMS];
};

template <int BITS, int ITEMS>
struct PassSmem : PassSmemCore<BITS, ITEMS> {
    static constexpr uint32_t kCore = sizeof(PassSmemCore<BITS, ITEMS>);
    uint8_t pad[BITS == 10 && kCore < kScatterLdsFloor ? kScatterLdsFloor - kCore : 4];
};

constexpr uint32_t kFlEmpty = 0x0000FFFFu;
constexpr uint32_t kGapWave = 16, kGapChunk = 32768, kGapCap = 4096, kGapLds = 4096, kGapPer = 8, kGapBlock = 256 * kGapPer;

__device__ __forceinline__ void write_gap(uint32_t* __restrict__ offsets, uint32_t lo, uint32_t len, uint32_t val,
                                          uint32_t* __restrict__ q, uint32_t cap) {
    const uint32_t lane = threadIdx.x & 63u;
    if (len <= kGapWave)
        for (uint32_t b = 0; b < len; ++b) offsets[lo + b] = val;
    uint64_t m = __ballot(len > kGapWave);
    while (m) {
        const uint32_t src = (uint32_t)__builtin_ctzll(m);
        m &= m - 1;
        const uint32_t glo = (uint32_t)__shfl((int)lo, (int)src, 64);
        const uint32_t gl = (uint32_t)__shfl((int)len, (int)src, 64);
        const uint32_t gv = (uint32_t)__shfl((int)val, (int)src, 64);
        uint32_t done = 0;
        if (gl > kGapChunk) {
            const uint32_t pieces = gl / kGapChunk;
            uint32_t first = 0;
            if (lane == 0) first = atomicAdd(&q[0], pieces);
            first = (uint32_t)__shfl((int)first, 0, 64);
            const uint32_t took = first >= cap ? 0u : min(pieces, cap - first);
            for (uint32_t p = lane; p < took; p += 64) {
                uint32_t* t = q + 2 + 3 * (size_t)(first + p);
                t[0] = glo + p * kGapChunk;
                t[1] = kGapChunk;
                t[2] = gv;
            }
            done = took * kGapChunk;
        }
        for (uint32_t b = done + lane; b < gl; b += 64) offsets[glo + b] = gv;
    }
}

template <int BITS, int IN, int OUT, int ITEMS, int RM>
__global__ __launch_bounds__(256) void k_radix_pass(const void* __restrict__ in, uint32_t n_all, uint32_t n_act, uint32_t shift,
                                                    const uint32_t* __restrict__ tile_off, uint32_t row_step, uint32_t ntiles,
                                                    uint2* __restrict__ pair_out, uint32_t* __restrict__ order_out,
                                                    uint32_t* __restrict__ key_out, const uint32_t* __restrict__ hot_words,
                                                    const uint32_t* __restrict__ hot_rows, uint32_t* __restrict__ hot_idx,
                                                    uint32_t* __restrict__ offsets, uint32_t nb, uint32_t* __restrict__ gap_q,
                                                    uint32_t gap_cap, uint32_t dsel, const uint32_t* __restrict__ lsd_hot) {
    constexpr uint32_t B = 1u << BITS;
    constexpr uint32_t PER = kDigitsPerThread<BITS>;
    constexpr uint32_t TILE = 256u * ITEMS;
    constexpr bool HOTP = IN == IN_ACT && (OUT == OUT_PAIR || OUT == OUT_PAIR_DIG);
    const bool lh = IN != IN_ACT && lsd_hot != nullptr;
    const uint32_t lhk = lh ? __builtin_amdgcn_readfirstlane(lsd_hot[0]) : kNoHotKey;
    const uint32_t lhc = lh ? __builtin_amdgcn_readfirstlane(lsd_hot[1]) : 0u;
    const uint32_t n = lh ? min(__builtin_amdgcn_readfirstlane(lsd_hot[2]), n_all) : n_all;
    __shared__ PassSmem<BITS, ITEMS> sm;
    __shared__ uint32_t hotw[kWaves];
    const uint32_t rflags = rank_flags();
    const uint32_t lane = threadIdx.x & 63u, w = threadIdx.x >> 6;
    const uint32_t tile = xcd_tile(blockIdx.x, ntiles);
    for (uint32_t b = threadIdx.x; b < B / 2u; b += 256) {
#pragma unroll
        for (uint32_t q = 0; q < kWaves; ++q) sm.cnt[q][b] = 0;
    }
    const uint32_t tbase = tile * TILE;
    const uint32_t wbase = tbase + w * (ITEMS * 64u);
    uint32_t key[ITEMS], idx[ITEMS], rank[ITEMS];
#pragma unroll
    for (uint32_t j = 0; j < ITEMS; ++j) {
        const uint32_t e = wbase + j * 64u + lane;
        const uint32_t ec = e < n ? e : (n ? n - 1 : 0u);
        if (IN == IN_ACT) {
            key[j] = bucket_key(ld_s4(static_cast<const uint32_t*>(in) + ec), n_act);
            idx[j] = e;
        } else {
            const uint2 v = ld_s4(static_cast<const uint2*>(in) + ec);
            key[j] = v.x;
            idx[j] = v.y;
        }
    }
    const uint32_t hk = (HOTP && hot_rows) ? hot_key_of(hot_words) : kNoHotKey;
    bool ishot[ITEMS];
    uint32_t hrank[ITEMS];
    if (HOTP && hk != kNoHotKey) {
        uint32_t run = 0;
#pragma unroll
        for (uint32_t j = 0; j < ITEMS; ++j) {
            ishot[j] = wbase + j * 64u + lane < n && key[j] == hk;
            const uint64_t b = __ballot(ishot[j]);
            hrank[j] = run + (uint32_t)__popcll(b & lanes_below());
            run += (uint32_t)__popcll(b);
        }
        if (lane == 0) hotw[w] = run;
    }
    __syncthreads();
    {
        uint32_t dg[ITEMS];
#pragma unroll
        for (uint32_t j = 0; j < ITEMS; ++j) dg[j] = (key[j] >> shift) & (B - 1u);
        if (HOTP && hk != kNoHotKey) rank_steps<BITS, true, ITEMS, RM>(&sm.cnt[w][0], dg, n > wbase ? n - wbase : 0u, rank, rflags, ishot);
        else rank_steps<BITS, true, ITEMS, RM>(&sm.cnt[w][0], dg, n > wbase ? n - wbase : 0u, rank, rflags);
    }
    __syncthreads();
    const uint32_t* orow = tile_off + (size_t)tile * row_step * B;
    uint32_t tile_hot = 0;
    if (HOTP && hk != kNoHotKey) {
        uint32_t before = 0;
#pragma unroll
        for (uint32_t q = 0; q < kWaves; ++q) {
            before += q < w ? hotw[q] : 0u;
            tile_hot += hotw[q];
        }
        const uint32_t hb = hot_rows[(size_t)tile * row_step] + before;
#pragma unroll
        for (uint32_t j = 0; j < ITEMS; ++j)
            if (ishot[j] && hb + hrank[j] < n) hot_idx[hb + hrank[j]] = idx[j];
    }
    uint32_t tot[PER], start[PER], dl[PER];
    round_starts<BITS>(sm.cnt, reinterpret_cast<uint32_t*>(&sm.stage[0]), tot, start);
#pragma unroll
    for (uint32_t q = 0; q < PER; ++q) {
        const uint32_t b = threadIdx.x * PER + q;
        dl[q] = b < B ? orow[b] - start[q] : 0u;
    }
    __syncthreads();
#pragma unroll
    for (uint32_t j = 0; j < ITEMS; ++j) {
        if (wbase + j * 64u + lane < n && !(HOTP && hk != kNoHotKey && ishot[j])) {
            const uint32_t d = (key[j] >> shift) & (B - 1u);
            const uint32_t lpos = packed_get(sm.cnt[w], d) + rank[j];
            sm.stage[lpos] = make_uint2(key[j], idx[j]);
        }
    }
    __syncthreads();
    if (OUT == OUT_FINAL_GAPS) {
#pragma unroll
        for (uint32_t q = 0; q < PER; ++q) {
            const uint32_t d = threadIdx.x * PER + q;
            if (d < B)
                key_out[(size_t)tile * B + d] = tot[q] ? (sm.stage[start[q]].x & 0xFFFFu) |
                                                             ((sm.stage[start[q] + tot[q] - 1u].x & 0xFFFFu) << 16)
                                                       : kFlEmpty;
        }
    }
    uint32_t* delta = &sm.cnt[0][0];
#pragma unroll
    for (uint32_t q = 0; q < PER; ++q)
        if (threadIdx.x * PER + q < B) delta[threadIdx.x * PER + q] = dl[q];
    __syncthreads();
    const uint32_t cnt = (n > tbase ? min(n - tbase, TILE) : 0u) - tile_hot;
#pragma unroll
    for (uint32_t j = 0; j < ITEMS; ++j) {
        const uint32_t i = j * 256u + threadIdx.x;
        if (OUT == OUT_FINAL_GAPS) {
            uint32_t lo = 0, len = 0, g = 0;
            if (i < cnt) {
                const uint2 kv = sm.stage[i];
                const uint32_t d = (kv.x >> shift) & (B - 1u);
                g = delta[d] + i;
                if (g < n) {
                    const uint32_t ga = g + (kv.x > lhk && lhk != kNoHotKey ? lhc : 0u);
                    if (ga < n_all) order_out[ga] = kv.y;
                    if (i > 0) {
                        const uint32_t pk = sm.stage[i - 1u].x;
                        if (((pk >> shift) & (B - 1u)) == d && pk < kv.x) {
                            lo = pk + 1u;
                            len = lo < nb ? min(kv.x - pk, nb - lo) : 0u;
                        }
                    }
                }
            }
            write_gap(offsets, lo, len, g, gap_q, gap_cap);
            continue;
        }
        if (i < cnt) {
            const uint2 kv = sm.stage[i];
            const uint32_t k = kv.x;
            const uint32_t g = delta[(k >> shift) & (B - 1u)] + i;
            if (g >= n) continue;
            if (OUT == OUT_PAIR) {
                pair_out[g] = kv;
            } else if (OUT == OUT_PAIR_DIG) {
                pair_out[g] = kv;
                reinterpret_cast<uint8_t*>(key_out)[g] = (uint8_t)((k >> (dsel & 31u)) & ((1u << (dsel >> 8)) - 1u));
            } else {
                key_out[g] = k;
                order_out[g] = kv.y;
            }
        }
    }
}

static_assert(kGapQueueWords == 2 + 3 * (size_t)kGapCap, "gap queue size");

__global__ __launch_bounds__(256) void k_offsets_gaps(const uint32_t* __restrict__ sorted, uint32_t n, uint32_t nb,
                                                      uint32_t* __restrict__ offsets, uint32_t* __restrict__ q, uint32_t cap) {
    __shared__ uint32_t span[kGapLds];
    __shared__ uint32_t range[2];
    const uint64_t p0 = (uint64_t)blockIdx.x * kGapBlock, i0 = p0 + threadIdx.x * kGapPer;
    const uint32_t lane = threadIdx.x & 63u, top = nb - 1u;
    if (threadIdx.x == 0) {
        const uint64_t pl = min<uint64_t>(p0 + kGapBlock - 1u, n);
        range[0] = p0 == 0 ? 0u : min(sorted[p0 - 1], top) + 1u;
        range[1] = (pl < n ? min(sorted[pl], top) : top) + 1u;
    }
    uint32_t k[kGapPer];
    if (i0 + kGapPer <= n) {
        const uint4* p = reinterpret_cast<const uint4*>(sorted + i0);
#pragma unroll
        for (uint32_t j = 0; j < kGapPer / 4; ++j) {
            const uint4 v = ld_s4(p + j);
            k[4 * j] = v.x; k[4 * j + 1] = v.y; k[4 * j + 2] = v.z; k[4 * j + 3] = v.w;
        }
    } else {
#pragma unroll
        for (uint32_t j = 0; j < kGapPer; ++j) k[j] = (i0 + j < n) ? sorted[i0 + j] : top;
    }
    uint32_t lo = i0 == 0 ? 0u : i0 <= n ? min(sorted[i0 - 1], top) + 1u : nb;
    __syncthreads();
    const uint32_t r0 = range[0], r1 = range[1];
    const bool in_lds = r1 - r0 <= kGapLds;
    auto put = [&](uint32_t b, uint32_t v) {
        if (in_lds) span[b - r0] = v; else offsets[b] = v;
    };
#pragma unroll
    for (uint32_t j = 0; j < kGapPer; ++j) {
        const uint32_t hi = min(k[j], top) + 1u;
        const uint32_t len = hi > lo ? hi - lo : 0u, val = (uint32_t)(i0 + j);
        if (len <= kGapWave)
            for (uint32_t b = 0; b < len; ++b) put(lo + b, val);
        uint64_t m = __ballot(len > kGapWave);
        while (m) {
            const uint32_t src = (uint32_t)__builtin_ctzll(m);
            m &= m - 1;
            const uint32_t glo = (uint32_t)__shfl((int)lo, (int)src, 64);
            const uint32_t gl = (uint32_t)__shfl((int)len, (int)src, 64);
            const uint32_t gv = (uint32_t)__shfl((int)val, (int)src, 64);
            uint32_t done = 0;
            if (!in_lds && gl > kGapChunk) {
                const uint32_t pieces = gl / kGapChunk;
                uint32_t first = 0;
                if (lane == 0) first = atomicAdd(&q[0], pieces);
                first = (uint32_t)__shfl((int)first, 0, 64);
                const uint32_t took = first >= cap ? 0u : min(pieces, cap - first);
                for (uint32_t p = lane; p < took; p += 64) {
                    uint32_t* t = q + 2 + 3 * (size_t)(first + p);
                    t[0] = glo + p * kGapChunk;
                    t[1] = kGapChunk;
                    t[2] = gv;
                }
                done = took * kGapChunk;
            }
            for (uint32_t b = done + lane; b < gl; b += 64) put(glo + b, gv);
        }
        lo = hi > lo ? hi : lo;
    }
    if (in_lds) {
        __syncthreads();
        for (uint32_t b = threadIdx.x; b < r1 - r0; b += 256u) offsets[r0 + b] = span[b];
    }
// ... 1908 lines not shown
                                                        uint32_t* __restrict__ bucket) {
    const uint32_t e = blockIdx.x * 256u + threadIdx.x;
    if (e >= n) return;
    const Msg m = load_hdr(msgs, e);
    const uint32_t u = ((m.meta >> 16) & ORL_HDR_HASH_VALID) ? m.aux : jenkins3(m.tcd, m.n0, m.n1);
    const int32_t key = (int32_t)u, mod = (int32_t)n_buckets;
    bucket[e] = (uint32_t)(((key % mod) + mod) % mod);
}

inline uint32_t ceil_div(uint64_t a, uint64_t b) { return (uint32_t)((a + b - 1) / b); }

constexpr uint32_t kScanDirectChunks = 1024;
constexpr uint32_t kScanSmallChunk = 1024;

int scan_inplace(uint32_t* a, uint64_t m, const Scratch& s, hipStream_t st) {
    const uint32_t nb = ceil_div(m, kScanChunk);
    if (nb == 0) return 0;
    hipLaunchKernelGGL(k_scan_reduce<0>, dim3(nb), dim3(256), 0, st, a, m, s.scan_sums, nullptr, nullptr, nullptr, nullptr, 0u);
    if (nb <= kScanDirectChunks) {
        hipLaunchKernelGGL((k_scan_down<true, false>), dim3(nb), dim3(256), 0, st, a, m, s.scan_sums, nullptr, 0ull, nullptr, 0u,
                           nullptr, nullptr);
    } else {
        hipLaunchKernelGGL(k_scan_sums, dim3(1), dim3(256), 0, st, s.scan_sums, nb);
        hipLaunchKernelGGL((k_scan_down<false, false>), dim3(nb), dim3(256), 0, st, a, m, s.scan_sums, nullptr, 0ull, nullptr, 0u,
                           nullptr, nullptr);
    }
    return (int)hipGetLastError();
}

uint32_t* hot_cur(const Scratch& s) { return s.hot + (s.hot_parity & 1u); }

int scan_offsets_pick(uint32_t* a, uint64_t m, uint32_t nkeys, uint32_t n, const Scratch& s, hipStream_t st) {
    const uint32_t nb = ceil_div(m, kScanChunk);
    if (nb == 0) return 0;
    uint32_t* next = s.hot + ((s.hot_parity + 1u) & 1u);
    hipLaunchKernelGGL(k_scan_reduce<2>, dim3(nb), dim3(256), 0, st, a, m, s.scan_sums, nullptr, nullptr, nullptr, s.hot_bmax, nkeys);
    if (nb <= kScanDirectChunks) {
        hipLaunchKernelGGL((k_scan_down<true, false, true>), dim3(nb), dim3(256), 0, st, a, m, s.scan_sums, nullptr, 0ull,
                           s.hot_bmax, n, next, s.hot_host_dev);
    } else {
        hipLaunchKernelGGL(k_scan_sums, dim3(1), dim3(256), 0, st, s.scan_sums, nb);
        hipLaunchKernelGGL((k_scan_down<false, false, true>), dim3(nb), dim3(256), 0, st, a, m, s.scan_sums, nullptr, 0ull,
                           s.hot_bmax, n, next, s.hot_host_dev);
    }
    s.hot_parity ^= 1u;
    return (int)hipGetLastError();
}

constexpr uint32_t kMsdItems = 16;
constexpr uint32_t kMsdItemsSmall = 8;
constexpr uint32_t kMsdSmallMax = 8u << 20;
uint32_t msd_items(uint32_t n, uint32_t route_items) {
    static const bool off = [] { const char* e = getenv("ORL_MSD_SMALL"); return e && e[0] == '0'; }();
    return (!off && n <= kMsdSmallMax && route_items <= kMsdItemsSmall) ? kMsdItemsSmall : kMsdItems;
}
static_assert(kRouteThreads * kMsdItems <= 65535u, "a route tile's digit counts must fit the u16 count rows (store_count_row)");

__global__ void k_hot_finish(const uint32_t* __restrict__ hot_words, const uint32_t* __restrict__ hot_total, uint32_t nb,
                             uint32_t* __restrict__ offsets) {
    const uint32_t hk = hot_key_of(hot_words);
    if (threadIdx.x == 0 && hk < nb) offsets[hk] += *hot_total;
}

constexpr uint32_t kTailUnroll = 8;
__global__ __launch_bounds__(256) void k_hot_tail(const uint32_t* __restrict__ hot_words, const uint32_t* __restrict__ hot_total,
                                                  uint32_t n, uint32_t nkeys, const uint32_t* __restrict__ hot_idx,
                                                  const uint32_t* __restrict__ offsets, uint32_t* __restrict__ order) {
    const uint32_t hk = hot_key_of(hot_words);
    if (hk >= nkeys) return;
    const uint32_t cnt = *hot_total, off = offsets[hk];
    if (cnt > n || off > n - cnt) return;
    const uint32_t stride = gridDim.x * 256u;
    uint32_t i = blockIdx.x * 256u + threadIdx.x;
    for (; i + (kTailUnroll - 1) * stride < cnt; i += kTailUnroll * stride) {
        uint32_t v[kTailUnroll];
#pragma unroll
        for (uint32_t u = 0; u < kTailUnroll; ++u) v[u] = ld_s4(hot_idx + i + u * stride);
#pragma unroll
        for (uint32_t u = 0; u < kTailUnroll; ++u) order[off + i + u * stride] = v[u];
    }
    for (; i < cnt; i += stride) order[off + i] = hot_idx[i];
}

__global__ void k_lsd_hot_prep(const uint32_t* __restrict__ hot_words, const uint32_t* __restrict__ hot_total, uint32_t n,
                               uint32_t* __restrict__ out) {
    if (threadIdx.x != 0) return;
    const uint32_t hk = hot_key_of(hot_words);
    const uint32_t hc = hk == kNoHotKey ? 0u : min(*hot_total, n);
    out[0] = hk;
    out[1] = hc;
    out[2] = n - hc;
}

__global__ __launch_bounds__(256) void k_lsd_hot_fix(uint32_t* __restrict__ offsets, uint32_t nb, const uint32_t* __restrict__ lh) {
    const uint32_t hk = __builtin_amdgcn_readfirstlane(lh[0]), hc = __builtin_amdgcn_readfirstlane(lh[1]);
    if (hk == kNoHotKey || hc == 0) return;
    for (uint32_t b = hk + 1u + blockIdx.x * 256u + threadIdx.x; b < nb; b += gridDim.x * 256u) offsets[b] += hc;
}

__global__ __launch_bounds__(256) void k_lsd_pick(const uint32_t* __restrict__ offsets, uint32_t nkeys,
                                                  unsigned long long* __restrict__ pick_word) {
    __shared__ unsigned long long wbest[kWaves];
    unsigned long long best = 0;
    for (uint32_t b = blockIdx.x * 256u + threadIdx.x; b < nkeys; b += gridDim.x * 256u) {
        const unsigned long long c = (unsigned long long)(offsets[b + 1] - offsets[b]) << 32 | b;
        best = c > best ? c : best;
    }
    best = wave_max_u64(best);
    if ((threadIdx.x & 63u) == 0) wbest[threadIdx.x >> 6] = best;
    __syncthreads();
    if (threadIdx.x == 0) {
        for (uint32_t q = 1; q < kWaves; ++q) best = wbest[q] > best ? wbest[q] : best;
        if (best >> 32) atomicMax(pick_word, best);
    }
}

__global__ void k_lsd_pick_finish(unsigned long long* __restrict__ pick_word, uint32_t n, uint32_t* __restrict__ next_key,
                                  uint32_t* __restrict__ host_word) {
    if (threadIdx.x != 0) return;
    const unsigned long long best = *pick_word;
    *pick_word = 0;
    const uint32_t c = (uint32_t)(best >> 32), k = (uint32_t)best;
    const uint32_t key = ((uint64_t)c * kHotShare >= n && c >= kHotMinCount) ? k : kNoHotKey;
    __hip_atomic_store(next_key, key, __ATOMIC_RELAXED, __HIP_MEMORY_SCOPE_AGENT);
    if (host_word) __hip_atomic_store(host_word, key, __ATOMIC_RELAXED, __HIP_MEMORY_SCOPE_SYSTEM);
}

uint32_t max_route_items(uint32_t n_act) {
    const BucketPlan bp = make_bucket_plan(n_act);
    return bp.two_level && bp.hb > 0 ? kMsdItems : kItems;
}

uint32_t route_min_wgs() {
    static const uint32_t v = [] {
        const char* e = getenv("ORL_ROUTE_MIN_WG");
        const long x = e ? atol(e) : 0;
        return x > 0 ? (uint32_t)x : 2048u;
    }();
    return v;
}

bool fan_probe16() {
    static const bool on = [] {
        const char* e = getenv("ORL_FAN_PROBE16");
        return e && e[0] == '1';
    }();
    return on;
}

uint32_t fan_min_wgs() {
    static const uint32_t v = [] {
        const char* e = getenv("ORL_FAN_MIN_WG");
        const long x = e ? atol(e) : 0;
        return x > 0 ? (uint32_t)x : 4096u;
    }();
    return v;
}

uint32_t route_items(uint64_t n, uint32_t max_items, uint32_t min_wg = 0) {
    uint32_t items = max_items;
    if (min_wg == 0) min_wg = route_min_wgs();
    while (items > 1 && ceil_div(n, (uint64_t)kRouteThreads * items) < min_wg &&
           ceil_div(n, (uint64_t)kRouteThreads * (items >> 1)) <= kMaxRouteRows)
        items >>= 1;
    return items;
}

constexpr uint32_t kItems12 = 12;

template <int BITS>
void launch_pass_bits(int rm, int in, int out, const void* kin, uint32_t n, uint32_t n_act, uint32_t shift, const uint32_t* toff,
                      uint32_t row_step, uint32_t ntiles, uint2* pout, uint32_t* order, uint32_t* keys, hipStream_t st,
                      const uint32_t* hot_words, const uint32_t* hot_rows, uint32_t* hot_idx, uint32_t* offsets, uint32_t nb,
                      uint32_t* gap_q, uint32_t gap_cap, uint32_t dsel, const uint32_t* lsd_hot, uint32_t items) {
    const dim3 g(ntiles), b(256);
#define ORL_RP3(I, O, IT, R) hipLaunchKernelGGL((k_radix_pass<BITS, I, O, IT, R>), g, b, 0, st, kin, n, n_act, shift, toff,    \
                                                row_step, ntiles, pout, order, keys, hot_words, hot_rows, hot_idx, offsets, nb,   \
                                                gap_q, gap_cap, dsel, lsd_hot)
#define ORL_RP(I, O, IT) do { const int rm_ = rm; if (rm_ == kRmPlain) ORL_RP3(I, O, IT, kRmPlain);                      \
                              else if (rm_ == kRmHot) ORL_RP3(I, O, IT, kRmHot); else ORL_RP3(I, O, IT, kRmBallot); } while (0)
    if (in == IN_ACT) {
        switch (out) {
            case OUT_PAIR: ORL_RP(IN_ACT, OUT_PAIR, kMsdItems); break;
            case OUT_PAIR_SMALL: ORL_RP(IN_ACT, OUT_PAIR, kMsdItemsSmall); break;
            case OUT_LSD_PAIR: ORL_RP(IN_ACT, OUT_PAIR, kItems); break;
            case OUT_PAIR_DIG: ORL_RP(IN_ACT, OUT_PAIR_DIG, kItems); break;
            default: ORL_RP(IN_ACT, OUT_FINAL, kItems); break;
        }
    } else if (out == OUT_PAIR || out == OUT_LSD_PAIR) {
        ORL_RP(IN_PAIR, OUT_PAIR, kItems);
    } else if (out == OUT_PAIR_DIG) {
        if (items == kItems12) ORL_RP(IN_PAIR, OUT_PAIR_DIG, kItems12);
        else ORL_RP(IN_PAIR, OUT_PAIR_DIG, kItems);
    } else if (out == OUT_FINAL_GAPS) {
        if (items == kItems12) ORL_RP(IN_PAIR, OUT_FINAL_GAPS, kItems12);
        else ORL_RP(IN_PAIR, OUT_FINAL_GAPS, kItems);
    } else {
        ORL_RP(IN_PAIR, OUT_FINAL, kItems);
    }
#undef ORL_RP
#undef ORL_RP3
}

void launch_pass(int rm, int bits, int in, int out, const void* kin, uint32_t n, uint32_t n_act, uint32_t shift, const uint32_t* toff,
                 uint32_t row_step, uint32_t ntiles, uint2* pout, uint32_t* order, uint32_t* keys, hipStream_t st,
                 const uint32_t* hot_words = nullptr, const uint32_t* hot_rows = nullptr, uint32_t* hot_idx = nullptr,
                 uint32_t* offsets = nullptr, uint32_t nb = 0, uint32_t* gap_q = nullptr, uint32_t gap_cap = 0,
                 uint32_t dsel = 0, const uint32_t* lsd_hot = nullptr, uint32_t items = kItems) {
    switch (bits) {
#define ORL_CASE(B) case B: launch_pass_bits<B>(rm, in, out, kin, n, n_act, shift, toff, row_step, ntiles, pout, order, keys, st, \
                                                hot_words, hot_rows, hot_idx, offsets, nb, gap_q, gap_cap, dsel, lsd_hot, items); break;
        ORL_CASE(1) ORL_CASE(2) ORL_CASE(3) ORL_CASE(4) ORL_CASE(5) ORL_CASE(6)
        ORL_CASE(7) ORL_CASE(8) ORL_CASE(9) ORL_CASE(10) ORL_CASE(11)
#undef ORL_CASE
        default: break;
    }
}

void col_scan(uint32_t* M, uint32_t ntiles, uint32_t bins, uint32_t row_step, const Scratch& s, hipStream_t st,
              uint32_t* hot_rows = nullptr, uint32_t plan_n = 0, uint32_t plan_seg = 0, bool self_sums = false) {
    const uint16_t* C = s.tile_cnt;
    const uint32_t nch = ceil_div(ntiles, kScanRows);
    const uint32_t cb = ceil_div(bins, 256);
    const uint32_t hy = hot_rows ? 1u : 0u;
    if (!self_sums || hot_rows || nch > kSelfScanChunks)
        hipLaunchKernelGGL(k_col_sum, dim3(nch, cb + hy), dim3(256), 0, st, C, ntiles, bins, s.col_sums, hot_rows);
    hipLaunchKernelGGL(k_col_scan, dim3(ceil_div(bins, kColScanCols) + hy), dim3(256), 0, st, s.col_sums, nch, bins, s.col_tot,
                       hot_rows, ntiles);
    const bool plan = plan_n > 0;
    hipLaunchKernelGGL(k_col_apply, dim3(nch + (plan ? 1u : 0u), ceil_div(bins, kApplyCols) + hy), dim3(256), 0, st, C, M, ntiles,
                       bins, s.col_sums, s.col_tot, row_step, hot_rows, plan_n, plan_seg, plan ? s.bstart : nullptr,
                       plan ? s.sstart : nullptr);
}

struct RouteHist {
    bool on;
    uint32_t bins, shift;
};

RouteHist route_hist(uint32_t n_act) {
    const BucketPlan bp = make_bucket_plan(n_act);
    if (bp.two_level) return {bp.hb > 0, 1u << bp.hb, (uint32_t)bp.lb};
    return {true, 1u << bp.lsd.bits[0], (uint32_t)bp.lsd.shift[0]};
}

uint32_t next_seg_epoch(const Scratch& s) {
    s.seg_epoch = (s.seg_epoch + 1u) & 0x3FFFFFFFu;
    if (s.seg_epoch == 0) s.seg_epoch = 1;
    return s.seg_epoch;
}

template <int LB>
void launch_seg_bits(int in, const void* kin, uint32_t n, uint32_t n_act, uint32_t nbk, uint32_t seg, uint32_t grid,
                     uint32_t* d_order, uint32_t* d_offsets, const Scratch& s, hipStream_t st, bool hot, bool pick) {
    const uint32_t nb = n_act + 2;
    const uint32_t solo = s.hot_host && !__atomic_load_n(s.hot_host + 1, __ATOMIC_ACQUIRE) ? 1u : 0u;
    const uint32_t direct = solo && !hot ? 1u : 0u;
    unsigned long long* pick_word = direct && pick ? s.pick_word : nullptr;
    uint32_t* next_key = s.hot + ((s.hot_parity + 1u) & 1u);
    uint32_t* skew_host = s.hot_host_dev ? s.hot_host_dev + 1 : nullptr;
    const uint32_t fgrid = std::max(nbk, std::min(solo ? ceil_div(grid, kLbRows) : grid, solo ? 2048u : 1024u));
    const uint32_t epoch = solo ? next_seg_epoch(s) : 0u;
#define ORL_SF(I) hipLaunchKernelGGL((k_seg_count_scan<LB, I>), dim3(fgrid), dim3(256), 0, st, kin, n, n_act, nbk, nb, seg, s.bstart, \
                                     s.sstart, s.seg_hist, d_offsets, solo, direct, skew_host, pick_word, n_act + 1, s.seg_carry,  \
                                     s.seg_meta, s.seg_lb, s.seg_lbctl, s.seg_lb_cap, epoch, s.s4_err)
#define ORL_SS3(I, R) hipLaunchKernelGGL((k_seg_scatter<LB, I, R>), dim3(grid), dim3(256), 0, st, kin, n, n_act, nbk, seg, s.bstart,\
                                         s.sstart, s.seg_hist, d_offsets, nb, n, s.seg_carry, s.seg_meta, d_order,         \
                                         solo ? kLbRows : kScanRows,                                                         \
                                         pick_word, next_key, s.hot_host_dev)
#define ORL_SS(I) do { const int rm_ = host_rm(s.device); if (rm_ == kRmPlain) ORL_SS3(I, kRmPlain); else if (rm_ == kRmHot)             \
                           ORL_SS3(I, kRmHot); else ORL_SS3(I, kRmBallot); } while (0)
    if (in == IN_ACT) ORL_SF(IN_ACT); else ORL_SF(IN_PAIR);
    const uint32_t cb = ceil_div(1u << LB, 256);
    const uint32_t nch = ceil_div(grid, kScanRows);
    if (!solo) {
        hipLaunchKernelGGL((k_seg_scan<LB>), dim3(nch, cb), dim3(256), 0, st, s.seg_hist, s.sstart, nbk, nb,
                           s.seg_carry, s.seg_meta, d_offsets);
        hipLaunchKernelGGL((k_seg_carry<LB>), dim3(ceil_div(1u << LB, 16)), dim3(256), 0, st, s.sstart, nbk, nb, s.seg_meta,
                           s.seg_carry, d_offsets);
    }
    const uint32_t* hw = hot_cur(s);
    if (hot) hipLaunchKernelGGL(k_hot_finish, dim3(1), dim3(64), 0, st, hw, s.col_tot + nbk, nb, d_offsets);
    if (pick && !direct)
        scan_offsets_pick(d_offsets, nb, n_act + 1, n, s, st);
    else if (pick)
        s.hot_parity ^= 1u;
    else if (!direct)
        scan_inplace(d_offsets, nb, s, st);
    if (in == IN_ACT) ORL_SS(IN_ACT); else ORL_SS(IN_PAIR);
    if (hot)
        hipLaunchKernelGGL(k_hot_tail, dim3(std::min<uint32_t>(ceil_div(n / 4u, 256u * kTailUnroll), 2048u)), dim3(256), 0, st,
                           hw, s.col_tot + nbk, n, n_act + 1, s.sorted_keys, d_offsets, d_order);
#undef ORL_SF
#undef ORL_SS
#undef ORL_SS3
}

void launch_seg(int lb, int in, const void* kin, uint32_t n, uint32_t n_act, uint32_t nbk, uint32_t seg, uint32_t grid,
                uint32_t* d_order, uint32_t* d_offsets, const Scratch& s, hipStream_t st, bool hot, bool pick) {
    switch (lb) {
#define ORL_CASE(B) case B: launch_seg_bits<B>(in, kin, n, n_act, nbk, seg, grid, d_order, d_offsets, s, st, hot, pick); break;
        ORL_CASE(1) ORL_CASE(2) ORL_CASE(3) ORL_CASE(4) ORL_CASE(5) ORL_CASE(6)
        ORL_CASE(7) ORL_CASE(8) ORL_CASE(9) ORL_CASE(10) ORL_CASE(11)
#undef ORL_CASE
        default: break;
    }
}

bool lsd_gaps(const RadixPlan& plan, uint64_t n, uint32_t n_act) {
    return plan.shift[plan.passes - 1] <= 16 && n >= 2ull * (n_act + 2ull);
}

bool hot_path_on(uint64_t n, uint32_t n_act, const Scratch& s) {
    static const bool off = [] {
        const char* e = getenv("ORL_NO_HOT");
        return e && e[0] == '1';
    }();
    if (off || !s.hot || n < kHotMinBatch) return false;
    const BucketPlan bp = make_bucket_plan(n_act);
    if (bp.two_level) return bp.hb > 0;
    return s.lsd_hot && lsd_gaps(bp.lsd, n, n_act);
}

bool hot_known(const Scratch& s) {
    const bool on = s.hot_host && __atomic_load_n(s.hot_host, __ATOMIC_ACQUIRE) != kNoHotKey;
    s.hot_batches += on ? 1u : 0u;
    return on;
}

int bucket_after_route(const uint32_t* d_act, uint32_t n, uint32_t n_act, uint32_t route_items, uint32_t* d_order,
                       uint32_t* d_offsets, const Scratch& s, hipStream_t st, bool hot, bool pick = false,
                       bool self_cols = false) {
    const BucketPlan bp = make_bucket_plan(n_act);
    const uint32_t ntiles = ceil_div(n, kTile);
    const uint32_t nb = n_act + 2;
    const uint32_t nrows0 = ceil_div(n, kRouteThreads * route_items);
    if (bp.two_level) {
        const uint32_t mitems = msd_items(n, route_items);
        const uint32_t row_step0 = mitems / route_items;
        const uint32_t ntiles = ceil_div(n, kRouteThreads * mitems);
        const uint32_t nbk = 1u << bp.hb;
        const uint32_t seg = seg_elems(n);
        const uint32_t grid = (uint32_t)max_segments(n, bp.hb);
        const void* kin = d_act;
        if (bp.hb > 0) {
            col_scan(s.tile_hist, nrows0, nbk, row_step0, s, st, hot ? s.hot_rows : nullptr, n, seg, self_cols);
            launch_pass(host_rm(s.device), bp.hb, IN_ACT, mitems == kMsdItems ? OUT_PAIR : OUT_PAIR_SMALL, d_act, n, n_act, (uint32_t)bp.lb, s.tile_hist,
                        row_step0, ntiles, s.pairs_a, nullptr, nullptr, st, hot ? hot_cur(s) : nullptr, hot ? s.hot_rows : nullptr,
                        hot ? s.sorted_keys : nullptr);
            kin = s.pairs_a;
        }
        if (bp.hb == 0)
            hipLaunchKernelGGL(k_seg_plan, dim3(1), dim3(1024), 0, st, nullptr, nbk, n, seg, s.bstart, s.sstart);
        launch_seg(bp.lb, bp.hb == 0 ? IN_ACT : IN_PAIR, kin, n, n_act, nbk, seg, grid, d_order, d_offsets, s, st, hot && bp.hb > 0, (hot || pick) && bp.hb > 0);
        return (int)hipGetLastError();
    }
    const RadixPlan& plan = bp.lsd;
    const uint32_t row_step0 = kItems / route_items;
    const bool gaps = lsd_gaps(plan, n, n_act);
    const bool lhot = hot && gaps && s.lsd_hot;
    const bool lpick = pick && gaps && s.lsd_hot;
    const uint32_t* hw = hot_cur(s);
    uint2* pbuf[2] = {s.pairs_a, s.pairs_b};
    uint8_t* dig = reinterpret_cast<uint8_t*>(s.sorted_keys);
    bool have_dig = false;
    bool t12 = gaps && plan.passes >= 2;
    for (int p = 1; p < plan.passes; ++p) t12 = t12 && plan.bits[p] <= 8;
    const uint32_t ntiles12 = ceil_div(n, kRouteThreads * kItems12);
    const uint32_t ntl = t12 ? ntiles12 : ntiles;
    for (int p = 0; p < plan.passes; ++p) {
        const uint32_t bins = 1u << plan.bits[p];
        const uint32_t row_step = (p == 0) ? row_step0 : 1u;
        const uint32_t ntp = p == 0 ? ntiles : ntl;
        const uint32_t nrows = (p == 0) ? nrows0 : ntl;
        const uint32_t* n_dev = (p > 0 && lhot) ? s.lsd_hot + 2 : nullptr;
        if (p > 0 && t12)
            hipLaunchKernelGGL((k_hist_dig8_wave<3, 1>), dim3(ceil_div(ntl, kWaves)), dim3(256), 0, st, dig, n, bins, ntl,
                               s.tile_cnt, n_dev);
        else if (p > 0 && have_dig)
            hipLaunchKernelGGL((k_hist_dig8_wave<4, 1>), dim3(ceil_div(ntiles, kWaves)), dim3(256), 0, st, dig, n, bins, ntiles,
                               s.tile_cnt, n_dev);
        else if (p > 0)
            hipLaunchKernelGGL(k_hist_pairs<false>, dim3(ntiles), dim3(256), 0, st, pbuf[(p - 1) & 1], n, n_act,
                               (uint32_t)plan.shift[p], bins, s.tile_cnt, nullptr, nullptr, n_dev);
        col_scan(s.tile_hist, nrows, bins, row_step, s, st, (p == 0 && lhot) ? s.hot_rows : nullptr, 0, 0, p == 0 && self_cols);
        if (p == 0 && lhot)
            hipLaunchKernelGGL(k_lsd_hot_prep, dim3(1), dim3(64), 0, st, hw, s.col_tot + bins, n, s.lsd_hot);
        const bool last = p == plan.passes - 1;
        const bool wdig = !last && plan.bits[p + 1] <= 8;
        const void* kin = (p == 0) ? static_cast<const void*>(d_act) : static_cast<const void*>(pbuf[(p - 1) & 1]);
        const int out = !last ? (wdig ? OUT_PAIR_DIG : OUT_LSD_PAIR) : gaps ? OUT_FINAL_GAPS : OUT_FINAL;
        const uint32_t dsel = wdig ? (uint32_t)plan.shift[p + 1] | ((uint32_t)plan.bits[p + 1] << 8) : 0u;
        const bool hp = p == 0 && lhot;
        launch_pass(host_rm(s.device), plan.bits[p], p == 0 ? IN_ACT : IN_PAIR, out, kin, n, n_act, (uint32_t)plan.shift[p],
                    s.tile_hist, row_step, ntp, pbuf[p & 1], d_order, wdig ? reinterpret_cast<uint32_t*>(dig) : s.sorted_keys,
                    st, hp ? hw : nullptr, hp ? s.hot_rows : nullptr, hp ? s.idx_a : nullptr, d_offsets, nb, s.gap_q, s.gap_cap,
                    dsel, (p > 0 && lhot) ? s.lsd_hot : nullptr, (p > 0 && t12) ? kItems12 : kItems);
        have_dig = wdig;
    }
    if (gaps) {
        const int lp = plan.passes - 1;
        const uint32_t ntiles = ntl;
        const uint32_t bins = 1u << plan.bits[lp], nch = ceil_div(ntiles, kScanRows);
        const bool bt = bins % kBoundCols == 0;
        if (bt) hipLaunchKernelGGL(k_bound_last_t, dim3(nch), dim3(256), 0, st, s.sorted_keys, ntiles, bins, s.col_sums);
        else hipLaunchKernelGGL(k_bound_last, dim3(nch), dim3(256), 0, st, s.sorted_keys, ntiles, bins, s.col_sums);
        hipLaunchKernelGGL(k_bound_scan, dim3(ceil_div(bins, kColScanCols)), dim3(256), 0, st, s.col_sums, nch, bins,
                           s.sorted_keys + (size_t)ntiles * bins);
        if (bt)
            hipLaunchKernelGGL(k_bound_apply_t, dim3(nch), dim3(256), 0, st, s.sorted_keys, s.tile_hist, s.col_sums, ntiles, bins,
                               (uint32_t)plan.shift[lp], nb, d_offsets, s.gap_q, s.gap_cap);
        else
            hipLaunchKernelGGL(k_bound_apply, dim3(nch), dim3(256), 0, st, s.sorted_keys, s.tile_hist, s.col_sums, ntiles, bins,
                               (uint32_t)plan.shift[lp], nb, d_offsets, s.gap_q, s.gap_cap);
        hipLaunchKernelGGL(k_offsets_tail, dim3(bins), dim3(256), 0, st, s.col_tot, s.sorted_keys + (size_t)ntiles * bins,
                           (uint32_t)plan.bits[lp], (uint32_t)plan.shift[lp], nb, d_offsets, s.gap_q, s.gap_cap);
        if (lhot) {
            hipLaunchKernelGGL(k_lsd_hot_fix, dim3(std::min<uint32_t>(ceil_div(nb, 256u * 16u), 2048u)), dim3(256), 0, st, d_offsets,
                               nb, s.lsd_hot);
            hipLaunchKernelGGL(k_hot_tail, dim3(std::min<uint32_t>(ceil_div(n / 4u, 256u * kTailUnroll), 2048u)), dim3(256), 0,
                               st, hw, s.lsd_hot + 1, n, n_act + 1, s.idx_a, d_offsets, d_order);
        }
        if (lpick) {
            hipLaunchKernelGGL(k_lsd_pick, dim3(std::min<uint32_t>(ceil_div(n_act + 1u, 256u * 16u), 512u)), dim3(256), 0, st,
                               d_offsets, n_act + 1u, s.pick_word);
            hipLaunchKernelGGL(k_lsd_pick_finish, dim3(1), dim3(64), 0, st, s.pick_word, n, s.hot + ((s.hot_parity + 1u) & 1u),
                               s.hot_host_dev);
            s.hot_parity ^= 1u;
        }
        return (int)hipGetLastError();
    }
    hipLaunchKernelGGL(k_offsets_gaps, dim3(ceil_div(n + 1, kGapBlock)), dim3(256), 0, st, s.sorted_keys, n, nb,
                       d_offsets, s.gap_q, s.gap_cap);
    hipLaunchKernelGGL(k_offsets_long, dim3(256), dim3(256), 0, st, d_offsets, s.gap_q, s.gap_cap);
    return (int)hipGetLastError();
}

}

uint32_t env_gap_cap() {
    const char* e = getenv("ORL_GAP_CAP");
    const long v = e ? atol(e) : (long)kGapCap;
    return (uint32_t)std::min<long>(std::max<long>(v, 0), (long)kGapCap);
}


int env_fan_u() {
    const char* e = getenv("ORL_FAN_U");
    const int v = e ? atoi(e) : kFanIlp;
    return v == 4 ? 4 : v == 2 ? 2 : 1;
}

int launch_rank_selfcheck(int device, int mode, uint32_t* ballot_out) {
    uint32_t* d_err = nullptr;
    uint32_t err = 0;
    hipError_t e = hipMalloc((void**)&d_err, 4);
    if (e == hipSuccess) e = hipMemset(d_err, 0, 4);
    if (e == hipSuccess) {
        hipLaunchKernelGGL(k_rank_selfcheck, dim3(1024), dim3(256), 0, nullptr, 0x5EEDu, d_err);
        e = hipGetLastError();
    }
    if (e == hipSuccess) e = hipMemcpy(&err, d_err, 4, hipMemcpyDeviceToHost);
    if (d_err) (void)hipFree(d_err);
    if (e != hipSuccess) return (int)e;
    const uint32_t ballot = (mode == 1 || err) ? 1u : 0u;
    e = (hipError_t)set_rank_mode(device, ballot);
    *ballot_out = ballot | (err << 1);
    return (int)e;
}

int set_rank_mode(int device, uint32_t ballot) {
    if (device < 0 || device >= kMaxDevices) return (int)hipErrorInvalidDevice;
    const char* u = getenv("ORL_RANK_UNIFORM");
    const uint32_t flags = (ballot ? kRankBallot : 0u) | ((u && u[0] == '0') ? 0u : kRankUniform);
    const hipError_t e = hipMemcpyToSymbol(HIP_SYMBOL(g_rank_flags), &flags, 4);
    if (e == hipSuccess) __atomic_store_n(&g_host_rank_flags[device], flags | kRankSet, __ATOMIC_RELEASE);
    return (int)e;
}

int launch_hash(const orl_grain_key* d_keys, size_t n, uint32_t* d_out, void* stream) {
    if (n == 0) return 0;
    hipLaunchKernelGGL(k_hash, dim3(ceil_div(n, 256)), dim3(256), 0, (hipStream_t)stream, d_keys, (uint32_t)n, d_out);
    return (int)hipGetLastError();
}

int launch_dir_patch(const uint32_t* d_idx, const DirSlot* d_slots, const ProbeSlot* d_p16, const uint2* d_p8, uint32_t n,
                     DirSlot* d_dir, ProbeSlot* d_probe, uint2* d_probe8, void* stream) {
    if (n == 0) return 0;
    hipLaunchKernelGGL(k_dir_patch, dim3(ceil_div(n, 256)), dim3(256), 0, (hipStream_t)stream, d_idx, d_slots, d_p16, d_p8, n,
                       d_dir, d_probe, d_probe8);
    return (int)hipGetLastError();
}

int launch_probe_build(const DirSlot* d_dir, uint64_t slots, const RouteParams* d_params, ProbeSlot* d_probe,
                       uint32_t* d_bad, void* stream) {
    hipStream_t st = (hipStream_t)stream;
    int e = (int)hipMemsetAsync(d_bad, 0, 4, st);
    if (e) return e;
    const uint64_t blocks = std::min<uint64_t>((slots + 255) / 256, 256ull * 64ull);
    hipLaunchKernelGGL(k_probe_build, dim3((uint32_t)blocks), dim3(256), 0, st, d_dir, slots, d_params, d_probe, d_bad);
    return (int)hipGetLastError();
}

int launch_route_bucket(const RouteParams* d_params, const DirView& dv, const void* d_in, int fmt,
                        size_t n, uint32_t opts, uint32_t n_act, uint32_t* d_route, uint32_t* d_act, uint32_t* d_order,
                        uint32_t* d_offsets, const Scratch& s, void* stream, void* ev_begin, void* ev_end,
                        const uint32_t* d_in_act, const SwView* sw) {
    hipStream_t st = (hipStream_t)stream;
    const bool buckets = !(opts & ORL_OPT_NO_BUCKETS);
    const uint32_t excl = (opts & ORL_OPT_EXCLUDE_IF_STOPPING) ? 1u : 0u;
    if (fmt != 8 && fmt != 16 && fmt != 32) return (int)hipErrorInvalidValue;
    if (n == 0) {
        if (buckets) return (int)hipMemsetAsync(d_offsets, 0, sizeof(uint32_t) * ((size_t)n_act + 2), st);
        return 0;
    }
    const uint32_t items = route_items(n, max_route_items(n_act));
    const uint32_t nwg = ceil_div(n, kRouteThreads * items);
    const RouteHist rh = route_hist(n_act);
    if (ev_begin) (void)hipEventRecord((hipEvent_t)ev_begin, st);
    const bool hist = buckets && rh.on;
    const bool pick = hist && hot_path_on(n, n_act, s);
    const bool hot = pick && hot_known(s);
    const uint32_t* hw = hot ? hot_cur(s) : nullptr;
    uint32_t* hr = hot ? s.hot_rows : nullptr;
    uint16_t* th = hist ? s.tile_cnt : nullptr;
    const uint32_t bins = hist ? rh.bins : 1u, shift = hist ? rh.shift : 0u;
    if (d_in_act && hist) return (int)hipErrorInvalidValue;
#define ORL_ROUTE_L(H, W, Q, C, LR) hipLaunchKernelGGL((k_route<H, W, Q, C, LR>), dim3(nwg), dim3(kRouteThreads), 0, st, d_params,\
                                                   dv.dir, dv.mask, dv.cache, dv.cmask, dv.probe, dv.probe_bad, d_in,                 \
                                                   (uint32_t)n, excl, d_route, d_act, th, bins, shift, items, hw, hr, d_in_act)
#define ORL_ROUTE_C(H, W, Q, C) do { if (dv.lru) ORL_ROUTE_L(H, W, Q, C, true); else ORL_ROUTE_L(H, W, Q, C, false); } while (0)
#define ORL_ROUTE(H, W, Q) do { if (H == 0 && d_in_act) ORL_ROUTE_C(0, W, Q, true); else ORL_ROUTE_C(H, W, Q, false); } while (0)
#define ORL_ROUTE_W(H, Q) do { if (fmt == 16) ORL_ROUTE(H, 16, Q); else if (fmt == 8) ORL_ROUTE(H, 8, Q); else ORL_ROUTE(H, 32, Q); } while (0)
    if (sw && sw->n) {
        const SwView swv = *sw;
#define ORL_ROUTE_SL(H, W, C, LR) hipLaunchKernelGGL((k_route_sw<H, W, C, LR>), dim3(nwg), dim3(kRouteThreads), 0, st, d_params,  \
                                                 dv.dir, dv.mask, dv.cache, dv.cmask, d_in, (uint32_t)n, excl, d_route, d_act, th,  \
                                                 bins, shift, items, hw, hr, d_in_act, swv)
#define ORL_ROUTE_SC(H, W, C) do { if (dv.lru) ORL_ROUTE_SL(H, W, C, true); else ORL_ROUTE_SL(H, W, C, false); } while (0)
#define ORL_ROUTE_SW(W) do { if (hist) ORL_ROUTE_SC(kMaxDigitBits, W, false); else if (d_in_act) ORL_ROUTE_SC(0, W, true);           \
                             else ORL_ROUTE_SC(0, W, false); } while (0)
        if (fmt == 16) ORL_ROUTE_SW(16); else if (fmt == 8) ORL_ROUTE_SW(8); else ORL_ROUTE_SW(32);
#undef ORL_ROUTE_SW
#undef ORL_ROUTE_SC
#undef ORL_ROUTE_SL
    } else if (dv.probe8) {
        const ProbeSlot* p8 = static_cast<const ProbeSlot*>(dv.probe8);
#define ORL_ROUTE8L(H, W, C, LR) hipLaunchKernelGGL((k_route<H, W, 8, C, LR>), dim3(nwg), dim3(kRouteThreads), 0, st, d_params,   \
                                                dv.dir, dv.mask, dv.cache, dv.cmask, p8, nullptr, d_in, (uint32_t)n, excl, d_route,  \
                                                d_act, th, bins, shift, items, hw, hr, d_in_act)
#define ORL_ROUTE8C(H, W, C) do { if (dv.lru) ORL_ROUTE8L(H, W, C, true); else ORL_ROUTE8L(H, W, C, false); } while (0)
#define ORL_ROUTE8(H, W) do { if (H == 0 && d_in_act) ORL_ROUTE8C(0, W, true); else ORL_ROUTE8C(H, W, false); } while (0)
        if (hist) {
            if (fmt == 16) ORL_ROUTE8(kMaxDigitBits, 16); else if (fmt == 8) ORL_ROUTE8(kMaxDigitBits, 8); else ORL_ROUTE8(kMaxDigitBits, 32);
        } else {
            if (fmt == 16) ORL_ROUTE8(0, 16); else if (fmt == 8) ORL_ROUTE8(0, 8); else ORL_ROUTE8(0, 32);
        }
#undef ORL_ROUTE8
#undef ORL_ROUTE8C
#undef ORL_ROUTE8L
    } else if (dv.probe) {
        if (hist) ORL_ROUTE_W(kMaxDigitBits, 16); else ORL_ROUTE_W(0, 16);
    } else {
        if (hist) ORL_ROUTE_W(kMaxDigitBits, 0); else ORL_ROUTE_W(0, 0);
    }
#undef ORL_ROUTE_W
#undef ORL_ROUTE
#undef ORL_ROUTE_C
#undef ORL_ROUTE_L
    if (ev_end) (void)hipEventRecord((hipEvent_t)ev_end, st);
    int e = (int)hipGetLastError();
    if (e) return e;
    if (!buckets) return 0;
    return bucket_after_route(d_act, (uint32_t)n, n_act, items, d_order, d_offsets, s, st, hot, pick);
}

int launch_fanout_route_bucket(const RouteParams* d_params, const DirView& dv, const orl_msg_hdr* d_direct, size_t n_direct,
                               const uint64_t* d_csr_off, const uint32_t* d_csr_tgt, const orl_grain_key* d_follower_keys,
                               const uint32_t* d_pubs, const uint8_t* d_pub_silo, size_t n_pub, uint64_t follower_tcd,
                               uint32_t opts, uint32_t n_act,
                               uint64_t* d_pub_offsets, uint32_t* d_route, uint32_t* d_act, uint32_t* d_order,
                               uint32_t* d_offsets, uint64_t* n_out, uint64_t max_out, const Scratch& s, void* stream,
                               void* ev_route_begin, void* ev_route_end) {
    hipStream_t st = (hipStream_t)stream;
    const bool buckets = !(opts & ORL_OPT_NO_BUCKETS);
    const uint32_t excl = (opts & ORL_OPT_EXCLUDE_IF_STOPPING) ? 1u : 0u;
    uint32_t* poff32 = s.idx_a;
    uint64_t* pstart = reinterpret_cast<uint64_t*>(s.pairs_b);
    const uint32_t m = (uint32_t)n_pub + 1;
    const uint32_t fcap = s.fan_blk ? (uint32_t)std::min<uint64_t>((max_out + kFanBlk - 1) / kFanBlk + 1, s.fan_blk_cap) : 0u;
    const bool small = m <= kScanSmallChunk * kScanDirectChunks;
    const uint32_t nbs = ceil_div(m, small ? kScanSmallChunk : kScanChunk);
    const RouteHist rh = route_hist(n_act);
    const uint64_t nch_max = ceil_div(ceil_div(std::max<uint64_t>(max_out, 1), (uint64_t)kRouteThreads), (uint64_t)kScanRows);
    const uint32_t zero_n = (buckets && rh.on) ?(uint32_t)std::min<uint64_t>(nch_max, kSelfScanChunks) * rh.bins : 0u;
    uint32_t* zero_p = zero_n ? s.col_sums : nullptr;
    if (small) {
        hipLaunchKernelGGL((k_scan_reduce<1, kScanSmallChunk>), dim3(nbs), dim3(256), 0, st, poff32, (uint64_t)m, s.scan_sums,
                           d_csr_off, d_pubs, pstart, nullptr, 0u, zero_p, zero_n);
        hipLaunchKernelGGL((k_scan_down<true, true, false, kScanSmallChunk>), dim3(nbs), dim3(256), 0, st, poff32, (uint64_t)m,
                           s.scan_sums, d_pub_offsets, (uint64_t)n_direct, nullptr, 0u, nullptr, nullptr, s.fan_blk, fcap);
    } else if (nbs <= kScanDirectChunks) {
        hipLaunchKernelGGL(k_scan_reduce<1>, dim3(nbs), dim3(256), 0, st, poff32, (uint64_t)m, s.scan_sums, d_csr_off, d_pubs, pstart,
                           nullptr, 0u, zero_p, zero_n);
        hipLaunchKernelGGL((k_scan_down<true, true>), dim3(nbs), dim3(256), 0, st, poff32, (uint64_t)m, s.scan_sums,
                           d_pub_offsets, (uint64_t)n_direct, nullptr, 0u, nullptr, nullptr, s.fan_blk, fcap);
    } else {
        hipLaunchKernelGGL(k_scan_reduce<1>, dim3(nbs), dim3(256), 0, st, poff32, (uint64_t)m, s.scan_sums, d_csr_off, d_pubs, pstart,
                           nullptr, 0u, zero_p, zero_n);
        hipLaunchKernelGGL(k_scan_sums, dim3(1), dim3(256), 0, st, s.scan_sums, nbs);
        hipLaunchKernelGGL((k_scan_down<false, true>), dim3(nbs), dim3(256), 0, st, poff32, (uint64_t)m, s.scan_sums,
                           d_pub_offsets, (uint64_t)n_direct, nullptr, 0u, nullptr, nullptr, s.fan_blk, fcap);
    }
    uint64_t total = *n_out;
    if (!(opts & ORL_OPT_TOTAL_GIVEN)) {
        uint32_t t32 = 0;
        int e = (int)hipMemcpyAsync(&t32, poff32 + n_pub, sizeof(uint32_t), hipMemcpyDeviceToHost, st);
        if (e) return e;
        e = (int)hipStreamSynchronize(st);
        if (e) return e;
        total = n_direct + t32;
        *n_out = total;
    }
    if (total > max_out) return -1;
    if (total == 0) {
        if (buckets) return (int)hipMemsetAsync(d_offsets, 0, sizeof(uint32_t) * ((size_t)n_act + 2), st);
        return 0;
    }
    const uint32_t items = route_items(total, max_route_items(n_act), fan_min_wgs());
    const uint32_t* fblk = (fcap && (total + kFanBlk - 1) / kFanBlk < fcap) ? s.fan_blk : nullptr;
    const uint32_t nwg = ceil_div(total, kRouteThreads * items);
    if (ev_route_begin) (void)hipEventRecord((hipEvent_t)ev_route_begin, st);
    const bool hist = buckets && rh.on;
    const bool self_cols = hist && zero_n && (uint64_t)ceil_div(nwg, kScanRows) * rh.bins <= zero_n;
    uint32_t* col_atomic = self_cols ? s.col_sums : nullptr;

#define ORL_FAN(H, TH, BINS, SHIFT) do { const int u_ = s.fan_u;                                                          \
        if (dv.probe8 && !fan_probe16()) ORL_FAN_(H, 8, 1, static_cast<const ProbeSlot*>(dv.probe8), nullptr, TH, BINS, SHIFT);        \
        else if (dv.probe) { if (u_ == 4) ORL_FAN_(H, 16, 4, dv.probe, dv.probe_bad, TH, BINS, SHIFT);                            \
                             else if (u_ == 2) ORL_FAN_(H, 16, 2, dv.probe, dv.probe_bad, TH, BINS, SHIFT);                       \
                             else ORL_FAN_(H, 16, 1, dv.probe, dv.probe_bad, TH, BINS, SHIFT); }                                  \
        else ORL_FAN_(H, 0, 1, dv.probe, dv.probe_bad, TH, BINS, SHIFT); } while (0)
#define ORL_FAN_(H, Q, U, PROBE, PBAD, TH, BINS, SHIFT) hipLaunchKernelGGL((k_fanout_route<H, Q, U>), dim3(nwg), dim3(kRouteThreads), 0, st, d_params, dv.dir, \
                                                       dv.mask, dv.cache, dv.cmask, PROBE, PBAD, pstart, d_csr_tgt, d_pub_silo, poff32, (uint32_t)n_pub,            \
                                                       follower_tcd, d_follower_keys, d_direct, (uint32_t)n_direct, (uint32_t)total,    \
                                                       excl, d_route, d_act, TH, BINS, \
                                                       SHIFT, items, fblk, col_atomic)
    if (hist) ORL_FAN(kMaxDigitBits, s.tile_cnt, rh.bins, rh.shift);
    else ORL_FAN(0, nullptr, 1u, 0u);
#undef ORL_FAN
#undef ORL_FAN_
    if (ev_route_end) (void)hipEventRecord((hipEvent_t)ev_route_end, st);
    int e = (int)hipGetLastError();
    if (e || !buckets) return e;
    return bucket_after_route(d_act, (uint32_t)total, n_act, items, d_order, d_offsets, s, st, false, false, self_cols);
}

// ... 67 lines not shown
    KxRebase rb{};
    for (uint32_t r = 0; r < nranks && r < ORL_NODE_MAX_RANKS; ++r) {
        rb.cnt[r] = cnt[r];
        rb.base[r] = base[r];
    }
    hipLaunchKernelGGL(k_ext_rebase, dim3((uint32_t)((n + 255) / 256)), dim3(256), 0, (hipStream_t)stream, d_refs, n, nranks, rb);
    return (int)hipGetLastError();
}

int launch_dir_split(const RouteParams* d_params, DirSlot* d_dir, uint64_t slots, uint32_t me, bool remove, uint64_t* d_cnt,
                     orl_grain_key* d_keys, uint32_t* d_acts, uint8_t* d_silos, uint64_t cap, uint64_t* d_n_out,
                     const Scratch& s, void* stream) {
    hipStream_t st = (hipStream_t)stream;
    const uint32_t ntiles = ceil_div(slots, kTile);
    hipLaunchKernelGGL(k_split_count, dim3(ntiles), dim3(256), 0, st, d_params, d_dir, slots, me, s.tile_hist);
    scan_inplace(s.tile_hist, ntiles, s, st);
    hipLaunchKernelGGL(k_split_emit, dim3(ntiles), dim3(256), 0, st, d_params, d_dir, slots, me, remove ? 1u : 0u, s.tile_hist,
                       d_keys, d_acts, d_silos, cap, d_n_out, d_cnt);
    return (int)hipGetLastError();
}

int launch_ring_owner(uint32_t kind, const RouteParams* d_params, const uint32_t* d_vr_hash, const uint8_t* d_vr_silo,
                      uint32_t vr_n, const uint32_t* d_keys, size_t n, uint32_t me, bool excl_me, uint8_t* d_owner,
                      void* stream) {
    if (n == 0) return 0;
    hipStream_t st = (hipStream_t)stream;
    const dim3 g(std::min<uint32_t>(ceil_div(n, 256), 8192)), b(256);
    if (kind == ORL_RING_CONSISTENT)
        hipLaunchKernelGGL(k_ring_owner<ORL_RING_CONSISTENT>, g, b, sizeof(RouteParams), st, d_params, d_vr_hash, d_vr_silo, vr_n,
                           d_keys, (uint32_t)n, me, excl_me ? 1u : 0u, d_owner);
    else
        hipLaunchKernelGGL(k_ring_owner<ORL_RING_VBUCKETS>, g, b, 5 * (size_t)vr_n + 16, st, d_params, d_vr_hash, d_vr_silo,
                           vr_n, d_keys, (uint32_t)n, me, excl_me ? 1u : 0u, d_owner);
    return (int)hipGetLastError();
}

int launch_stream_queue(uint32_t kind, const RouteParams* d_params, const uint32_t* d_vr_hash, const uint8_t* d_vr_silo,
                        uint32_t vr_n, const uint8_t* d_guids, size_t n, uint32_t n_queues, uint32_t me, bool excl_me,
                        uint32_t* d_queue, uint8_t* d_silo, void* stream) {
    if (n == 0) return 0;
    hipStream_t st = (hipStream_t)stream;
    const dim3 g(std::min<uint32_t>(ceil_div(n, 256), 8192)), b(256);
    const u32x4* gu = reinterpret_cast<const u32x4*>(d_guids);
    if (kind == ORL_RING_CONSISTENT)
        hipLaunchKernelGGL(k_stream_queue<ORL_RING_CONSISTENT>, g, b, d_silo ? sizeof(RouteParams) : 0, st, d_params, d_vr_hash,
                           d_vr_silo, vr_n, gu, (uint32_t)n, n_queues, me, excl_me ? 1u : 0u, d_queue, d_silo);
    else
        hipLaunchKernelGGL(k_stream_queue<ORL_RING_VBUCKETS>, g, b, d_silo ? 5 * (size_t)vr_n + 16 : 0, st, d_params, d_vr_hash,
                           d_vr_silo, vr_n, gu, (uint32_t)n, n_queues, me, excl_me ? 1u : 0u, d_queue, d_silo);
    return (int)hipGetLastError();
}

int launch_outbound_queues(const orl_msg_hdr* d_msgs, const uint32_t* d_route, size_t n, uint32_t n_senders,
                           const int32_t* d_silo_hash, const uint8_t* d_silo_known, uint32_t* d_queue, void* stream) {
    if (n == 0) return 0;
    hipLaunchKernelGGL(k_outbound_queues, dim3(ceil_div(n, 256)), dim3(256), 0, (hipStream_t)stream, d_msgs, d_route, (uint32_t)n,
                       n_senders, d_silo_hash, d_silo_known, d_queue);
    return (int)hipGetLastError();
}

int launch_client_buckets(const orl_msg_hdr* d_msgs, size_t n, uint32_t n_buckets, uint32_t* d_bucket, void* stream) {
    if (n == 0) return 0;
    hipLaunchKernelGGL(k_client_buckets, dim3(ceil_div(n, 256)), dim3(256), 0, (hipStream_t)stream, d_msgs, (uint32_t)n, n_buckets,
                       d_bucket);
    return (int)hipGetLastError();
}

int launch_keyext_route(const RouteParams* d_params, const orl_msg_hdr* d_in, size_t n, const orl_ext_ref* d_ext,
                        const uint8_t* d_blob, uint64_t blob_bytes, const ExtSlot* d_table, uint64_t mask,
                        const uint8_t* d_tblob, uint32_t excl, uint32_t* d_route, uint32_t* d_act, void* stream) {
    if (n == 0) return 0;
    hipLaunchKernelGGL(k_keyext_route, dim3(ceil_div(n, 256)), dim3(256), 0, (hipStream_t)stream, d_params, d_in, (uint32_t)n,
                       d_ext, d_blob, blob_bytes, d_table, mask, d_tblob, excl, d_route, d_act);
    return (int)hipGetLastError();
}

int launch_bucket_acts(const uint32_t* d_act, size_t n, uint32_t n_act, uint32_t* d_order, uint32_t* d_offsets, const Scratch& s,
                       void* stream) {
    hipStream_t st = (hipStream_t)stream;
    if (n == 0) return (int)hipMemsetAsync(d_offsets, 0, sizeof(uint32_t) * ((size_t)n_act + 2), st);
    const RouteHist rh = route_hist(n_act);
    const uint32_t ntiles = ceil_div(n, kTile);
    const bool pick = rh.on && hot_path_on(n, n_act, s);
    const bool hot = pick && hot_known(s);
    if (rh.on)
        hipLaunchKernelGGL(k_hist_pairs<true>, dim3(ntiles), dim3(256), 0, st, d_act, (uint32_t)n, n_act, rh.shift, rh.bins,
                           s.tile_cnt, hot ? hot_cur(s) : nullptr, hot ? s.hot_rows : nullptr);
    int e = (int)hipGetLastError();
    if (e) return e;
    return bucket_after_route(d_act, (uint32_t)n, n_act, kItems, d_order, d_offsets, s, st, hot, pick);
}

int launch_host_rank_count(const uint32_t* d_route, size_t n, const uint8_t* d_ros, uint32_t my_rank, uint64_t* d_counts,
                           void* stream) {
    hipStream_t st = (hipStream_t)stream;
    int e = (int)hipMemsetAsync(d_counts, 0, 8 * sizeof(uint64_t), st);
    if (e || n == 0) return e;
    const uint32_t g = std::min<uint32_t>(ceil_div(n, 256 * 16), 2048);
    hipLaunchKernelGGL(k_host_rank_count, dim3(g), dim3(256), 0, st, d_route, (uint32_t)n, d_ros, my_rank,
                       reinterpret_cast<unsigned long long*>(d_counts));
    return (int)hipGetLastError();
}

size_t part_state_bytes(size_t n) { return 16 + (size_t)ceil_div(n, kPartTile) * 64; }

__global__ void k_node_stall(const uint32_t* __restrict__ flag) {
    if (threadIdx.x != 0) return;
    for (uint32_t i = 0; i < (1u << 21); ++i) {
        if (__hip_atomic_load(flag, __ATOMIC_RELAXED, __HIP_MEMORY_SCOPE_SYSTEM) != 0u) return;
        __builtin_amdgcn_s_sleep(127);
    }
}

int launch_node_stall(const uint32_t* flag, void* stream) {
    hipLaunchKernelGGL(k_node_stall, dim3(1), dim3(64), 0, (hipStream_t)stream, flag);
    return (int)hipGetLastError();
}

int launch_part_routed(const uint8_t* d_ros, const void* d_in, int win, int wout, const uint32_t* d_route, const uint32_t* d_act,
                       size_t n, uint32_t my_rank, uint32_t nranks, uint64_t stride, void* d_out, uint32_t* d_route_out,
                       uint32_t* d_act_out, uint32_t* d_state, const uint64_t* d_base_in, uint64_t* d_counts,
                       const uint64_t* d_wire_tcd, uint32_t* d_err, void* stream) {
    hipStream_t st = (hipStream_t)stream;
    hipError_t e = d_base_in ? hipMemcpyAsync(d_counts, d_base_in, sizeof(uint64_t) * nranks, hipMemcpyDeviceToDevice, st)
                             : hipMemsetAsync(d_counts, 0, sizeof(uint64_t) * nranks, st);
    if (e != hipSuccess || n == 0) return (int)e;
    const uint32_t ntiles = ceil_div(n, kPartTile);
    if ((e = hipMemsetAsync(d_state, 0, part_state_bytes(n), st)) != hipSuccess) return (int)e;
#define ORL_PR(WI, WO) hipLaunchKernelGGL((k_part_routed<WI, WO>), dim3(ntiles), dim3(kRouteThreads), 0, st, d_ros, d_in, d_route,  \
                                          d_act, (uint32_t)n, my_rank, nranks, stride, d_out, d_route_out, d_act_out, d_state,   \
                                          ntiles, d_base_in, d_counts, d_wire_tcd, d_err)
    if (win == 8 && wout == 8) ORL_PR(8, 8);
    else if (win == 8) ORL_PR(8, 32);
    else if (win == 16 && wout == 16) ORL_PR(16, 16);
    else if (win == 16) ORL_PR(16, 32);
    else ORL_PR(32, 32);
#undef ORL_PR
    return (int)hipGetLastError();
}

int launch_partition_padded(const RouteParams* d_params, const orl_msg_hdr* d_in, size_t n, uint32_t opts,
                            const uint8_t* d_rank_of_silo, uint32_t nranks, uint32_t my_rank, uint64_t stride,
                            void* d_out, int fmt, uint32_t* d_src_index, uint64_t* d_counts, uint32_t* d_wire_status,
                            Scratch& s, void* stream, const DirSlot* d_cache, uint64_t cmask, uint32_t* d_act_out,
                            const KxLanes* kxl, const SwView* sw) {
    hipStream_t st = (hipStream_t)stream;
    hipError_t e = hipSuccess;
    if (fmt != 8 && fmt != 16 && fmt != 32) return (int)hipErrorInvalidValue;
    if (fmt != 32 && !d_wire_status) return (int)hipErrorInvalidValue;
    if (d_wire_status) e = hipMemsetAsync(d_wire_status, 0, sizeof(uint32_t), st);
    if (e == hipSuccess && n == 0) e = hipMemsetAsync(d_counts, 0, sizeof(uint64_t) * nranks, st);
    if (e != hipSuccess || n == 0) return (int)e;
    const uint32_t excl = (opts & ORL_OPT_EXCLUDE_IF_STOPPING) ? 1u : 0u;
    const uint32_t ntiles = ceil_div(n, kPartTile);
    Scratch::LbSet* L = nullptr;
    for (auto& x : s.lb)
        if (x.stream == st) L = &x;
    if (!L) {
        L = &s.lb[0];
        for (auto& x : s.lb)
            if (x.last < L->last) L = &x;
        if (L->last && (e = hipStreamWaitEvent(st, L->ev, 0)) != hipSuccess) return (int)e;
        L->stream = st;
    }
    L->last = ++s.lb_clock;
    const size_t lb_bytes = 16 + (size_t)ceil_div(s.max_batch, kPartTile) * 64;
    if (++L->epoch >= (1u << 30)) {
        if ((e = hipMemsetAsync(L->state, 0, lb_bytes, st)) != hipSuccess) return (int)e;
// ... 98 lines not shown
```

Before: 39.10 billion messages/s.

## Extend LSD hot-key handling from single key to a hot set of up to 255 keys

New measurement: 37.94 billion messages/s. 0.97x the previous value.

```diff
diff --git a/include/orleans_route.h b/include/orleans_route.h
--- a/include/orleans_route.h
+++ b/include/orleans_route.h
@@ -565,6 +565,7 @@
 #define ORL_Q_HOT_KEY 10u
 #define ORL_Q_HOT_BATCHES 11u
 #define ORL_Q_STAGE4_ERROR 12u
+#define ORL_Q_HOT_SET 13u
 int orl_ctx_query(orl_ctx* ctx, uint32_t what, uint64_t* value);
 int orl_ctx_set_rank_mode(orl_ctx* ctx, uint32_t mode);
 
diff --git a/orleans_amd/_lib.py b/orleans_amd/_lib.py
--- a/orleans_amd/_lib.py
+++ b/orleans_amd/_lib.py
@@ -87,6 +87,7 @@
 Q_HOT_KEY = 10
 Q_HOT_BATCHES = 11
 Q_STAGE4_ERROR = 12
+Q_HOT_SET = 13
 MAX_WIRE_TYPES = 16
 PART_LOOKBACK_FAILED = 0x4
 PART_KEYEXT = 0x10
diff --git a/orleans_amd/csrc/orl_api.cpp b/orleans_amd/csrc/orl_api.cpp
--- a/orleans_amd/csrc/orl_api.cpp
+++ b/orleans_amd/csrc/orl_api.cpp
@@ -864,8 +864,16 @@
             if ((e = hipMemset(L.state, 0, 16 + ((mb + 2047) / 2048) * 64)) != hipSuccess) return bail(e, "hipMemset(lb_state)");
             if ((e = hipEventCreateWithFlags(&L.ev, hipEventDisableTiming)) != hipSuccess) return bail(e, "hipEventCreate(lb)");
         }
-        if (const char* lh = getenv("ORL_LSD_HOT"); lh && lh[0] == '1')
-            if ((e = hipMalloc((void**)&c->s.lsd_hot, 16)) != hipSuccess) return bail(e, "hipMalloc(lsd_hot)");
+        const char* lh = getenv("ORL_LSD_HOT");
+        if (!bp.two_level && lh && lh[0] == '1') {
+            if ((e = hipMalloc((void**)&c->s.lsd_hot, kLsdSetWords * 4)) != hipSuccess) return bail(e, "hipMalloc(lsd_hot)");
+            if ((e = hipMemset(c->s.lsd_hot, 0xFF, 2 * kLsdSetSlotWords * 4)) != hipSuccess) return bail(e, "hipMemset(lsd_hot)");
+            if ((e = hipMemset(c->s.lsd_hot + 2 * kLsdSetSlotWords, 0, (kLsdSetWords - 2 * kLsdSetSlotWords) * 4)) != hipSuccess)
+                return bail(e, "hipMemset(lsd_hot)");
+            for (uint32_t slot = 0; slot < 2; ++slot)
+                if ((e = hipMemset(c->s.lsd_hot + slot * kLsdSetSlotWords + kLsdSetSize, 0, 4)) != hipSuccess)
+                    return bail(e, "hipMemset(lsd_hot)");
+        }
         if ((e = hipMalloc((void**)&c->s.s4_err, 4)) != hipSuccess) return bail(e, "hipMalloc(s4_err)");
         if ((e = hipMemset(c->s.s4_err, 0, 4)) != hipSuccess) return bail(e, "hipMemset(s4_err)");
         if ((e = hipMalloc((void**)&c->s.gap_q, kGapQueueWords * 4)) != hipSuccess) return bail(e, "hipMalloc(gap_q)");
@@ -886,7 +894,7 @@
         if ((e = hipMalloc((void**)&c->s.hot_rows, (rows + (rows + 63) / 64 + 1) * 4)) != hipSuccess) return bail(e, "hipMalloc(hot_rows)");
         if ((e = hipHostMalloc((void**)&c->s.hot_host, 8, hipHostMallocMapped | hipHostMallocCoherent)) != hipSuccess)
             return bail(e, "hipHostMalloc(hot_host)");
-        c->s.hot_host[0] = 0xFFFFFFFFu;
+        c->s.hot_host[0] = bp.two_level ? 0xFFFFFFFFu : 0u;
         c->s.hot_host[1] = 1u;
         if ((e = hipHostGetDevicePointer((void**)&c->s.hot_host_dev, c->s.hot_host, 0)) != hipSuccess)
             return bail(e, "hipHostGetDevicePointer(hot_host)");
@@ -3248,6 +3256,18 @@
             *v = w;
             return ORL_OK;
         }
+        case ORL_Q_HOT_SET: {
+            if (!c->device_mode) return fail(c, ORL_E_STATE, "no device");
+            uint32_t w = 0;
+            if (c->s.lsd_hot) {
+                ORL_HIP(c, hipSetDevice(c->cfg.device));
+                ORL_HIP(c, hipDeviceSynchronize());
+                ORL_HIP(c, hipMemcpy(&w, c->s.lsd_hot + (c->s.hot_parity & 1u) * kLsdSetSlotWords + kLsdSetSize, 4,
+                                     hipMemcpyDeviceToHost));
+            }
+            *v = w;
+            return ORL_OK;
+        }
         case ORL_Q_PART_ERROR: {
             if (!c->device_mode) return fail(c, ORL_E_STATE, "no device");
             ORL_HIP(c, hipSetDevice(c->cfg.device));
diff --git a/orleans_amd/csrc/orl_internal.h b/orleans_amd/csrc/orl_internal.h
--- a/orleans_amd/csrc/orl_internal.h
+++ b/orleans_amd/csrc/orl_internal.h
@@ -263,6 +263,14 @@
     uint8_t silo, state, pad[6];
 };
 static_assert(sizeof(ExtSlot) == 48, "KeyExt slot layout");
+
+constexpr uint32_t kLsdSetMax = 255, kLsdSetTab = 1024, kLsdSetCands = 2048;
+constexpr uint32_t kLsdSetSize = 255, kLsdSetTabK = 256;
+constexpr uint32_t kLsdSetSlotWords = kLsdSetTabK + kLsdSetTab;
+constexpr uint32_t kLsdSetCnt = 2 * kLsdSetSlotWords, kLsdSetPre = kLsdSetCnt + 256, kLsdSetNp = kLsdSetPre + 256;
+constexpr uint32_t kLsdSetCandN = kLsdSetNp + 1, kLsdSetCand = kLsdSetCandN + 1;
+constexpr uint32_t kLsdSetWords = kLsdSetCand + 2 * kLsdSetCands;
+static_assert(kLsdSetCand % 2 == 0, "the candidate list is read as 8-B words");
 
 constexpr uint32_t kSegLbMinRows = 8;
 
diff --git a/orleans_amd/csrc/route_kernels.hip b/orleans_amd/csrc/route_kernels.hip
--- a/orleans_amd/csrc/route_kernels.hip
+++ b/orleans_amd/csrc/route_kernels.hip
@@ -557,6 +557,48 @@
     return hot ? __builtin_amdgcn_readfirstlane(__hip_atomic_load(hot, __ATOMIC_RELAXED, __HIP_MEMORY_SCOPE_AGENT)) : kNoHotKey;
 }
 
+struct SetLds {
+    uint32_t tab[kLsdSetTab];
+};
+constexpr uint32_t kSetKeyMask = 0x00FFFFFFu;
+
+constexpr uint32_t kSetHotBit = 0x80000000u;
+
+__device__ __forceinline__ uint32_t set_hash(uint32_t k) { return (k * 2654435761u) >> (32u - 10u); }
+static_assert(kLsdSetTab == 1024, "set_hash gives 10 bits");
+
+__device__ __forceinline__ void set_stage(SetLds& t, const uint32_t* __restrict__ slot) {
+    reinterpret_cast<uint4*>(t.tab)[threadIdx.x] = reinterpret_cast<const uint4*>(slot + kLsdSetTabK)[threadIdx.x];
+}
+static_assert(kLsdSetTab == 4 * 256 && kLsdSetTabK % 4 == 0 && kLsdSetSlotWords % 4 == 0, "set_stage's 16-B copies");
+
+__device__ __forceinline__ uint32_t set_digit(const SetLds& t, uint32_t k) {
+    const uint32_t h = set_hash(k);
+    const uint32_t a = t.tab[h], b = t.tab[(h + 1u) & (kLsdSetTab - 1u)];
+    if (a == kNoHotKey) return k & 255u;
+    if ((a & kSetKeyMask) == k) return 256u + (a >> 24);
+    if (b == kNoHotKey) return k & 255u;
+    if ((b & kSetKeyMask) == k) return 256u + (b >> 24);
+    for (uint32_t i = 2; i < kLsdSetTab; ++i) {
+        const uint32_t x = t.tab[(h + i) & (kLsdSetTab - 1u)];
+        if (x == kNoHotKey) break;
+        if ((x & kSetKeyMask) == k) return 256u + (x >> 24);
+    }
+    return k & 255u;
+}
+
+__device__ __forceinline__ uint32_t set_below(const uint32_t* keys, uint32_t k) {
+    uint32_t lo = 0;
+#pragma unroll
+    for (uint32_t step = 128; step; step >>= 1)
+        if (keys[lo + step - 1u] < k) lo += step;
+    return lo;
+}
+
+#ifndef ORL_LSD_SET_FUSED
+#define ORL_LSD_SET_FUSED 1
+#endif
+
 __device__ __forceinline__ void wave_add_hot(uint32_t* dst, uint32_t mine) {
     uint32_t v = mine;
 #pragma unroll
@@ -608,7 +650,7 @@
 #ifndef ORL_PART_ATTR
 #define ORL_PART_ATTR
 #endif
-template <int HB, int FMT, int PW, bool CIN, bool LRU, bool SW>
+template <int HB, int FMT, int PW, bool CIN, bool LRU, bool SW, bool SET = false>
 __device__ __forceinline__ void route_body(const RouteParams* __restrict__ gp, const DirSlot* __restrict__ dir,
                                            uint64_t dmask, const DirSlot* __restrict__ cache, uint64_t cmask,
                                            const ProbeSlot* __restrict__ probe, const uint32_t* __restrict__ probe_bad,
@@ -631,9 +673,16 @@
     if (HIST)
         for (uint32_t b = threadIdx.x; b < bins; b += blockDim.x) sm.hist[b] = 0;
     if (threadIdx.x == 0) sm.hot = 0;
+    const SetLds* setl = nullptr;
+    if constexpr (SET) {
+        static_assert(HB >= 9, "the hot set's digits need 512 bins");
+        __shared__ SetLds set_lds;
+        set_stage(set_lds, hot_words);
+        setl = &set_lds;
+    }
     __syncthreads();
     const uint32_t n_act = sm.P.n_act;
-    const uint32_t hk = (HIST && hot_rows) ? hot_key_of(hot_words) : kNoHotKey;
+    const uint32_t hk = (HIST && !SET && hot_rows) ? hot_key_of(hot_words) : kNoHotKey;
     uint32_t hot_mine = 0;
     const bool use16 = PW == 16 && (probe_bad == nullptr || *probe_bad == 0u);
     const uint32_t base = blockIdx.x * (kRouteThreads * items) + threadIdx.x;
@@ -699,7 +748,8 @@
                 }
                 if (HIST) {
                     const uint32_t k = bucket_key(act, n_act);
-                    if (k == hk) ++hot_mine;
+                    if (SET) atomicAdd(&sm.hist[set_digit(*setl, k)], 1u);
+                    else if (k == hk) ++hot_mine;
                     else atomicAdd(&sm.hist[(k >> shift) & (bins - 1)], 1u);
                 }
             }
@@ -741,7 +791,8 @@
                 }
                 if (HIST) {
                     const uint32_t k = bucket_key(act, n_act);
-                    if (k == hk) ++hot_mine;
+                    if (SET) atomicAdd(&sm.hist[set_digit(*setl, k)], 1u);
+                    else if (k == hk) ++hot_mine;
                     else atomicAdd(&sm.hist[(k >> shift) & (bins - 1)], 1u);
                 }
             }
@@ -787,7 +838,8 @@
             }
             if (HIST) {
                 const uint32_t k = bucket_key(act, n_act);
-                if (k == hk) ++hot_mine;
+                if (SET) atomicAdd(&sm.hist[set_digit(*setl, k)], 1u);
+                else if (k == hk) ++hot_mine;
                 else atomicAdd(&sm.hist[(k >> shift) & (bins - 1)], 1u);
             }
         }
@@ -804,7 +856,7 @@
     }
 }
 
-template <int HB, int FMT, int PW, bool CIN = false, bool LRU = false>
+template <int HB, int FMT, int PW, bool CIN = false, bool LRU = false, bool SET = false>
 __global__ __launch_bounds__(kRouteThreads) ORL_ROUTE_ATTR void k_route(const RouteParams* __restrict__ gp, const DirSlot* __restrict__ dir,
                                                          uint64_t dmask, const DirSlot* __restrict__ cache, uint64_t cmask,
                                                          const ProbeSlot* __restrict__ probe,
@@ -815,7 +867,7 @@
                                                          uint32_t bins, uint32_t shift, uint32_t items,
                                                          const uint32_t* __restrict__ hot_words, uint32_t* __restrict__ hot_rows,
                                                          const uint32_t* __restrict__ in_act) {
-    route_body<HB, FMT, PW, CIN, LRU, false>(gp, dir, dmask, cache, cmask, probe, probe_bad, in, n, excl, route, act_out, tile_cnt,
+    route_body<HB, FMT, PW, CIN, LRU, false, SET>(gp, dir, dmask, cache, cmask, probe, probe_bad, in, n, excl, route, act_out, tile_cnt,
                                              bins, shift, items, hot_words, hot_rows, in_act, nullptr);
 }
 
@@ -1073,7 +1125,7 @@
     return *p;
 }
 
-template <bool ACTS>
+template <bool ACTS, bool SET = false>
 __global__ __launch_bounds__(256) void k_hist_pairs(const void* __restrict__ in, uint32_t n, uint32_t n_act, uint32_t shift,
                                                     uint32_t bins, uint16_t* __restrict__ tile_cnt,
                                                     const uint32_t* __restrict__ hot_words = nullptr,
@@ -1084,8 +1136,15 @@
     __shared__ uint32_t hot;
     for (uint32_t b = threadIdx.x; b < bins; b += 256) hist[b] = 0;
     if (threadIdx.x == 0) hot = 0;
-    __syncthreads();
-    const uint32_t hk = (ACTS && hot_rows) ? hot_key_of(hot_words) : kNoHotKey;
+    const SetLds* setl = nullptr;
+    if constexpr (SET) {
+        static_assert(ACTS, "the hot set's histogram reads the handles");
+        __shared__ SetLds set_lds;
+        set_stage(set_lds, hot_words);
+        setl = &set_lds;
+    }
+    __syncthreads();
+    const uint32_t hk = (ACTS && !SET && hot_rows) ? hot_key_of(hot_words) : kNoHotKey;
     uint32_t hot_mine = 0;
     const uint32_t base = blockIdx.x * kTile;
     uint32_t k[kItems];
@@ -1098,7 +1157,8 @@
 #pragma unroll
         for (uint32_t j = 0; j < kItems; ++j)
             if (base + j * 256 + threadIdx.x < n) {
-                if (k[j] == hk) ++hot_mine;
+                if (SET) atomicAdd(&hist[set_digit(*setl, k[j])], 1u);
+                else if (k[j] == hk) ++hot_mine;
                 else atomicAdd(&hist[(k[j] >> shift) & (bins - 1)], 1u);
             }
         if (hot_rows) wave_add_hot(&hot, hot_mine);
@@ -1337,7 +1397,8 @@
 }
 
 enum : int { IN_ACT = 0, IN_PAIR = 1 };
-enum : int { OUT_PAIR = 0, OUT_FINAL = 1, OUT_LSD_PAIR = 4, OUT_PAIR_SMALL = 5, OUT_FINAL_GAPS = 6, OUT_PAIR_DIG = 7 };
+enum : int { OUT_PAIR = 0, OUT_FINAL = 1, OUT_LSD_PAIR = 4, OUT_PAIR_SMALL = 5, OUT_FINAL_GAPS = 6, OUT_PAIR_DIG = 7,
+              OUT_PAIR_DIG_SET = 8, OUT_FINAL_GAPS_SET = 9 };
 
 __device__ __forceinline__ uint32_t wave_find_pub(const uint32_t* __restrict__ poff, uint32_t n_pub, uint32_t v) {
     const uint32_t lane = threadIdx.x & 63u;
@@ -1450,7 +1511,7 @@
     }
 }
 
-template <int BITS, int IN, int OUT, int ITEMS, int RM>
+template <int BITS, int IN, int OUT_T, int ITEMS, int RM>
 __global__ __launch_bounds__(256) void k_radix_pass(const void* __restrict__ in, uint32_t n_all, uint32_t n_act, uint32_t shift,
                                                     const uint32_t* __restrict__ tile_off, uint32_t row_step, uint32_t ntiles,
                                                     uint2* __restrict__ pair_out, uint32_t* __restrict__ order_out,
@@ -1461,16 +1522,41 @@
     constexpr uint32_t B = 1u << BITS;
     constexpr uint32_t PER = kDigitsPerThread<BITS>;
     constexpr uint32_t TILE = 256u * ITEMS;
-    constexpr bool HOTP = IN == IN_ACT && (OUT == OUT_PAIR || OUT == OUT_PAIR_DIG);
+    constexpr bool SETP = OUT_T == OUT_PAIR_DIG_SET, SETF = OUT_T == OUT_FINAL_GAPS_SET;
+    constexpr int OUT = SETP ? OUT_PAIR_DIG : SETF ? OUT_FINAL_GAPS : OUT_T;
+    static_assert(!SETP || (IN == IN_ACT && BITS == 9), "the hot set's first pass: 256 low digits + up to 255 keys");
+    static_assert(!SETF || IN == IN_PAIR, "the hot set's last pass reads pairs");
+    constexpr bool HOTP = IN == IN_ACT && (OUT_T == OUT_PAIR || OUT_T == OUT_PAIR_DIG);
     const bool lh = IN != IN_ACT && lsd_hot != nullptr;
-    const uint32_t lhk = lh ? __builtin_amdgcn_readfirstlane(lsd_hot[0]) : kNoHotKey;
-    const uint32_t lhc = lh ? __builtin_amdgcn_readfirstlane(lsd_hot[1]) : 0u;
-    const uint32_t n = lh ? min(__builtin_amdgcn_readfirstlane(lsd_hot[2]), n_all) : n_all;
+    const uint32_t n = lh ? min(__builtin_amdgcn_readfirstlane(lsd_hot[kLsdSetNp]), n_all) : n_all;
     __shared__ PassSmem<BITS, ITEMS> sm;
     __shared__ uint32_t hotw[kWaves];
+    const SetLds* setl = nullptr;
+    if constexpr (SETP) {
+        static_assert(sizeof(SetLds) <= sizeof(sm.stage), "the set's table fits the stage area");
+        SetLds* tl = reinterpret_cast<SetLds*>(&sm.stage[0]);
+        set_stage(*tl, hot_words);
+        setl = tl;
+    }
+    const uint32_t *skeys = nullptr, *spre = nullptr;
+    uint32_t* smix = nullptr;
+    if constexpr (SETF) {
+        static_assert(B <= 256, "one thread per digit fills smix");
+        __shared__ uint32_t set_keys[256], set_pre[256], set_mix[256];
+        set_keys[threadIdx.x] = threadIdx.x < kLsdSetMax ? hot_words[threadIdx.x] : kNoHotKey;
+        set_pre[threadIdx.x] = lsd_hot[kLsdSetPre + threadIdx.x];
+        skeys = set_keys;
+        spre = set_pre;
+        smix = set_mix;
+    }
     const uint32_t rflags = rank_flags();
     const uint32_t lane = threadIdx.x & 63u, w = threadIdx.x >> 6;
     const uint32_t tile = xcd_tile(blockIdx.x, ntiles);
+    if (IN != IN_ACT && lh && tile * TILE >= n) {
+        if (OUT == OUT_FINAL_GAPS)
+            for (uint32_t d = threadIdx.x; d < B; d += 256u) key_out[(size_t)tile * B + d] = kFlEmpty;
+        return;
+    }
     for (uint32_t b = threadIdx.x; b < B / 2u; b += 256) {
 #pragma unroll
         for (uint32_t q = 0; q < kWaves; ++q) sm.cnt[q][b] = 0;
@@ -1506,10 +1592,21 @@
         if (lane == 0) hotw[w] = run;
     }
     __syncthreads();
+    if constexpr (SETF) {
+        if (threadIdx.x < B) {
+            const uint32_t j0 = set_below(skeys, threadIdx.x << shift);
+            const uint32_t j1 = threadIdx.x == B - 1u ? set_below(skeys, kNoHotKey) : set_below(skeys, (threadIdx.x + 1u) << shift);
+            smix[threadIdx.x] = j0 | (j1 - j0) << 8;
+        }
+    }
+    uint32_t sdg[SETP ? ITEMS : 1];
     {
         uint32_t dg[ITEMS];
 #pragma unroll
-        for (uint32_t j = 0; j < ITEMS; ++j) dg[j] = (key[j] >> shift) & (B - 1u);
+        for (uint32_t j = 0; j < ITEMS; ++j) {
+            if constexpr (SETP) dg[j] = sdg[j] = set_digit(*setl, key[j]);
+            else dg[j] = (key[j] >> shift) & (B - 1u);
+        }
         if (HOTP && hk != kNoHotKey) rank_steps<BITS, true, ITEMS, RM>(&sm.cnt[w][0], dg, n > wbase ? n - wbase : 0u, rank, rflags, ishot);
         else rank_steps<BITS, true, ITEMS, RM>(&sm.cnt[w][0], dg, n > wbase ? n - wbase : 0u, rank, rflags);
     }
@@ -1539,9 +1636,15 @@
 #pragma unroll
     for (uint32_t j = 0; j < ITEMS; ++j) {
         if (wbase + j * 64u + lane < n && !(HOTP && hk != kNoHotKey && ishot[j])) {
-            const uint32_t d = (key[j] >> shift) & (B - 1u);
+            uint32_t d, kx = key[j];
+            if constexpr (SETP) {
+                d = sdg[j];
+                if (d >= 256u) kx = kSetHotBit | d;
+            } else {
+                d = (key[j] >> shift) & (B - 1u);
+            }
             const uint32_t lpos = packed_get(sm.cnt[w], d) + rank[j];
-            sm.stage[lpos] = make_uint2(key[j], idx[j]);
+            sm.stage[lpos] = make_uint2(kx, idx[j]);
         }
     }
     __syncthreads();
@@ -1571,7 +1674,13 @@
                 const uint32_t d = (kv.x >> shift) & (B - 1u);
                 g = delta[d] + i;
                 if (g < n) {
-                    const uint32_t ga = g + (kv.x > lhk && lhk != kNoHotKey ? lhc : 0u);
+                    uint32_t ga = g;
+                    if constexpr (SETF) {
+                        const uint32_t mx = smix[d];
+                        uint32_t hj = mx & 255u;
+                        for (uint32_t c = mx >> 8; c && skeys[hj] < kv.x; --c) ++hj;
+                        ga += spre[hj];
+                    }
                     if (ga < n_all) order_out[ga] = kv.y;
                     if (i > 0) {
                         const uint32_t pk = sm.stage[i - 1u].x;
@@ -1588,6 +1697,18 @@
         if (i < cnt) {
             const uint2 kv = sm.stage[i];
             const uint32_t k = kv.x;
+            if constexpr (SETP) {
+                const bool hotm = (k & kSetHotBit) != 0u;
+                const uint32_t g = delta[hotm ? k & (B - 1u) : k & 255u] + i;
+                if (g >= n) continue;
+                if (hotm) {
+                    hot_idx[g] = kv.y;
+                    continue;
+                }
+                pair_out[g] = kv;
+                reinterpret_cast<uint8_t*>(key_out)[g] = (uint8_t)((k >> (dsel & 31u)) & ((1u << (dsel >> 8)) - 1u));
+                continue;
+            }
             const uint32_t g = delta[(k >> shift) & (B - 1u)] + i;
             if (g >= n) continue;
             if (OUT == OUT_PAIR) {
@@ -3662,48 +3783,140 @@
     for (; i < cnt; i += stride) order[off + i] = hot_idx[i];
 }
 
-__global__ void k_lsd_hot_prep(const uint32_t* __restrict__ hot_words, const uint32_t* __restrict__ hot_total, uint32_t n,
-                               uint32_t* __restrict__ out) {
-    if (threadIdx.x != 0) return;
-    const uint32_t hk = hot_key_of(hot_words);
-    const uint32_t hc = hk == kNoHotKey ? 0u : min(*hot_total, n);
-    out[0] = hk;
-    out[1] = hc;
-    out[2] = n - hc;
-}
-
-__global__ __launch_bounds__(256) void k_lsd_hot_fix(uint32_t* __restrict__ offsets, uint32_t nb, const uint32_t* __restrict__ lh) {
-    const uint32_t hk = __builtin_amdgcn_readfirstlane(lh[0]), hc = __builtin_amdgcn_readfirstlane(lh[1]);
-    if (hk == kNoHotKey || hc == 0) return;
-    for (uint32_t b = hk + 1u + blockIdx.x * 256u + threadIdx.x; b < nb; b += gridDim.x * 256u) offsets[b] += hc;
-}
-
-__global__ __launch_bounds__(256) void k_lsd_pick(const uint32_t* __restrict__ offsets, uint32_t nkeys,
-                                                  unsigned long long* __restrict__ pick_word) {
-    __shared__ unsigned long long wbest[kWaves];
-    unsigned long long best = 0;
+__global__ __launch_bounds__(256) void k_lsd_set_prep(const uint32_t* __restrict__ slot, const uint32_t* __restrict__ col_tot,
+                                                      uint32_t n, uint32_t* __restrict__ lh) {
+    __shared__ uint32_t wsum[kWaves];
+    const uint32_t H = min(slot[kLsdSetSize], kLsdSetMax);
+    const uint32_t c = threadIdx.x < H ? col_tot[256u + threadIdx.x] : 0u;
+    uint32_t total;
+    const uint32_t ex = block_excl_scan(c, wsum, total);
+    lh[kLsdSetCnt + threadIdx.x] = c;
+    lh[kLsdSetPre + threadIdx.x] = min(ex, n);
+    if (threadIdx.x == 0) lh[kLsdSetNp] = n - min(total, n);
+}
+
+__global__ __launch_bounds__(256) void k_lsd_set_fix(uint32_t* __restrict__ offsets, uint32_t nb, const uint32_t* __restrict__ slot,
+                                                     const uint32_t* __restrict__ lh) {
+    __shared__ uint32_t skeys[256], spre[256];
+    skeys[threadIdx.x] = threadIdx.x < kLsdSetMax ? slot[threadIdx.x] : kNoHotKey;
+    spre[threadIdx.x] = lh[kLsdSetPre + threadIdx.x];
+    __syncthreads();
+    const uint32_t first = skeys[0];
+    if (first == kNoHotKey || spre[255] == 0u) return;
+    for (uint64_t b = (uint64_t)first + 1u + blockIdx.x * 256u + threadIdx.x; b < nb; b += gridDim.x * 256u)
+        offsets[b] += spre[set_below(skeys, (uint32_t)b)];
+}
+
+__global__ __launch_bounds__(256) void k_lsd_set_tail(const uint32_t* __restrict__ slot, const uint32_t* __restrict__ lh, uint32_t n,
+                                                      uint32_t nkeys, const uint32_t* __restrict__ hot_idx,
+                                                      const uint32_t* __restrict__ offsets, uint32_t* __restrict__ order) {
+    __shared__ uint32_t spre[256], soff[256];
+    {
+        const uint32_t k = threadIdx.x < kLsdSetMax ? slot[threadIdx.x] : kNoHotKey;
+        spre[threadIdx.x] = lh[kLsdSetPre + threadIdx.x];
+        soff[threadIdx.x] = k < nkeys ? offsets[k] : n;
+    }
+    __syncthreads();
+    const uint32_t total = spre[255], np = lh[kLsdSetNp];
+    if (total > n || np != n - total) return;
+    auto place = [&](uint32_t i) {
+        uint32_t j = 0;
+#pragma unroll
+        for (uint32_t step = 128; step; step >>= 1)
+            if (spre[j + step] <= i) j += step;
+        const uint32_t off = soff[j], r = i - spre[j];
+        return off < n && r < n - off ? off + r : n;
+    };
+    const uint32_t stride = gridDim.x * 256u;
+    uint32_t i = blockIdx.x * 256u + threadIdx.x;
+    for (; i + (kTailUnroll - 1) * stride < total; i += kTailUnroll * stride) {
+        uint32_t v[kTailUnroll];
+#pragma unroll
+        for (uint32_t u = 0; u < kTailUnroll; ++u) v[u] = ld_s4(hot_idx + np + i + u * stride);
+#pragma unroll
+        for (uint32_t u = 0; u < kTailUnroll; ++u) {
+            const uint32_t p = place(i + u * stride);
+            if (p < n) order[p] = v[u];
+        }
+    }
+    for (; i < total; i += stride) {
+        const uint32_t p = place(i);
+        if (p < n) order[p] = hot_idx[np + i];
+    }
+}
+
+constexpr uint32_t kLsdHotShare = 2048;
+static_assert(kLsdHotShare <= kLsdSetCands, "every qualifying key has a place in the candidate list");
+
+__global__ __launch_bounds__(256) void k_lsd_set_pick(const uint32_t* __restrict__ offsets, uint32_t nkeys, uint32_t n,
+                                                      uint32_t* __restrict__ lh) {
+    __shared__ unsigned long long cand[kLsdSetCands];
+    __shared__ uint32_t cn, cbase;
+    if (threadIdx.x == 0) cn = 0;
+    __syncthreads();
     for (uint32_t b = blockIdx.x * 256u + threadIdx.x; b < nkeys; b += gridDim.x * 256u) {
-        const unsigned long long c = (unsigned long long)(offsets[b + 1] - offsets[b]) << 32 | b;
-        best = c > best ? c : best;
-    }
-    best = wave_max_u64(best);
-    if ((threadIdx.x & 63u) == 0) wbest[threadIdx.x >> 6] = best;
-    __syncthreads();
+        const uint32_t c = offsets[b + 1] - offsets[b];
+        if ((uint64_t)c * kLsdHotShare >= n && c >= kHotMinCount) {
+            const uint32_t i = atomicAdd(&cn, 1u);
+            if (i < kLsdSetCands) cand[i] = (unsigned long long)~c << 32 | b;
+        }
+    }
+    __syncthreads();
+    const uint32_t m = min(cn, kLsdSetCands);
+    if (m == 0) return;
+    if (threadIdx.x == 0) cbase = atomicAdd(&lh[kLsdSetCandN], m);
+    __syncthreads();
+    unsigned long long* out = reinterpret_cast<unsigned long long*>(lh + kLsdSetCand);
+    for (uint32_t i = threadIdx.x; i < m; i += 256u)
+        if (cbase + i < kLsdSetCands) out[cbase + i] = cand[i];
+}
+
+__global__ __launch_bounds__(256) void k_lsd_set_pick_finish(uint32_t* __restrict__ lh, uint32_t* __restrict__ next_slot,
+                                                             uint32_t* __restrict__ host_word) {
+    __shared__ unsigned long long a[kLsdSetCands];
+    __shared__ uint32_t keys[256];
+    __shared__ SetLds tab;
+    const uint32_t m = min(lh[kLsdSetCandN], kLsdSetCands);
+    uint32_t P = 2;
+    while (P < m) P <<= 1;
+    const unsigned long long* in = reinterpret_cast<const unsigned long long*>(lh + kLsdSetCand);
+    for (uint32_t i = threadIdx.x; i < P; i += 256u) a[i] = i < m ? in[i] : ~0ull;
+    __syncthreads();
+    for (uint32_t k = 2; k <= P; k <<= 1) {
+        for (uint32_t j = k >> 1; j > 0; j >>= 1) {
+            for (uint32_t i = threadIdx.x; i < P; i += 256u) {
+                const uint32_t l = i ^ j;
+                if (l > i) {
+                    const unsigned long long x = a[i], y = a[l];
+                    if ((x > y) == ((i & k) == 0u)) {
+                        a[i] = y;
+                        a[l] = x;
+                    }
+                }
+            }
+            __syncthreads();
+        }
+    }
+    const uint32_t H = min(m, kLsdSetMax);
+    const uint32_t mine = threadIdx.x < H ? (uint32_t)a[threadIdx.x] : kNoHotKey;
+    keys[threadIdx.x] = kNoHotKey;
+    for (uint32_t i = threadIdx.x; i < kLsdSetTab; i += 256u) tab.tab[i] = kNoHotKey;
+    __syncthreads();
+    uint32_t rank = 0;
+    if (threadIdx.x < H) {
+        for (uint32_t j = 0; j < H; ++j) rank += (uint32_t)a[j] < mine ? 1u : 0u;
+        keys[rank] = mine;
+        uint32_t h = set_hash(mine);
+        while (atomicCAS(&tab.tab[h], kNoHotKey, (mine & kSetKeyMask) | rank << 24) != kNoHotKey)
+            h = (h + 1u) & (kLsdSetTab - 1u);
+    }
+    __syncthreads();
+    next_slot[threadIdx.x] = threadIdx.x == kLsdSetSize ? H : keys[threadIdx.x];
+    for (uint32_t i = threadIdx.x; i < kLsdSetTab; i += 256u) next_slot[kLsdSetTabK + i] = tab.tab[i];
     if (threadIdx.x == 0) {
-        for (uint32_t q = 1; q < kWaves; ++q) best = wbest[q] > best ? wbest[q] : best;
-        if (best >> 32) atomicMax(pick_word, best);
-    }
-}
-
-__global__ void k_lsd_pick_finish(unsigned long long* __restrict__ pick_word, uint32_t n, uint32_t* __restrict__ next_key,
-                                  uint32_t* __restrict__ host_word) {
-    if (threadIdx.x != 0) return;
-    const unsigned long long best = *pick_word;
-    *pick_word = 0;
-    const uint32_t c = (uint32_t)(best >> 32), k = (uint32_t)best;
-    const uint32_t key = ((uint64_t)c * kHotShare >= n && c >= kHotMinCount) ? k : kNoHotKey;
-    __hip_atomic_store(next_key, key, __ATOMIC_RELAXED, __HIP_MEMORY_SCOPE_AGENT);
-    if (host_word) __hip_atomic_store(host_word, key, __ATOMIC_RELAXED, __HIP_MEMORY_SCOPE_SYSTEM);
+        lh[kLsdSetCandN] = 0;
+        if (host_word) __hip_atomic_store(host_word, H, __ATOMIC_RELAXED, __HIP_MEMORY_SCOPE_SYSTEM);
+    }
 }
 
 uint32_t max_route_items(uint32_t n_act) {
@@ -3765,8 +3978,13 @@
             case OUT_PAIR_SMALL: ORL_RP(IN_ACT, OUT_PAIR, kMsdItemsSmall); break;
             case OUT_LSD_PAIR: ORL_RP(IN_ACT, OUT_PAIR, kItems); break;
             case OUT_PAIR_DIG: ORL_RP(IN_ACT, OUT_PAIR_DIG, kItems); break;
+            case OUT_PAIR_DIG_SET:
+                if constexpr (BITS == 9) ORL_RP(IN_ACT, OUT_PAIR_DIG_SET, kItems);
+                break;
             default: ORL_RP(IN_ACT, OUT_FINAL, kItems); break;
         }
+    } else if (out == OUT_FINAL_GAPS_SET) {
+        if constexpr (BITS == 7 || BITS == 8) ORL_RP(IN_PAIR, OUT_FINAL_GAPS_SET, kItems12);
     } else if (out == OUT_PAIR || out == OUT_LSD_PAIR) {
         ORL_RP(IN_PAIR, OUT_PAIR, kItems);
     } else if (out == OUT_PAIR_DIG) {
@@ -3891,6 +4109,13 @@
     return plan.shift[plan.passes - 1] <= 16 && n >= 2ull * (n_act + 2ull);
 }
 
+bool lsd_set_plan(const RadixPlan& plan) {
+    if (plan.passes < 2 || plan.bits[0] != 8) return false;
+    for (int p = 1; p < plan.passes; ++p)
+        if (plan.bits[p] > 8) return false;
+    return plan.bits[plan.passes - 1] >= 7;
+}
+
 bool hot_path_on(uint64_t n, uint32_t n_act, const Scratch& s) {
     static const bool off = [] {
         const char* e = getenv("ORL_NO_HOT");
@@ -3899,14 +4124,17 @@
     if (off || !s.hot || n < kHotMinBatch) return false;
     const BucketPlan bp = make_bucket_plan(n_act);
     if (bp.two_level) return bp.hb > 0;
-    return s.lsd_hot && lsd_gaps(bp.lsd, n, n_act);
-}
-
-bool hot_known(const Scratch& s) {
-    const bool on = s.hot_host && __atomic_load_n(s.hot_host, __ATOMIC_ACQUIRE) != kNoHotKey;
+    return s.lsd_hot && lsd_set_plan(bp.lsd) && lsd_gaps(bp.lsd, n, n_act);
+}
+
+bool hot_known(const Scratch& s, uint32_t n_act) {
+    const uint32_t none = make_bucket_plan(n_act).two_level ? kNoHotKey : 0u;
+    const bool on = s.hot_host && __atomic_load_n(s.hot_host, __ATOMIC_ACQUIRE) != none;
     s.hot_batches += on ? 1u : 0u;
     return on;
 }
+
+uint32_t* lsd_set_cur(const Scratch& s) { return s.lsd_hot + (s.hot_parity & 1u) * kLsdSetSlotWords; }
 
 int bucket_after_route(const uint32_t* d_act, uint32_t n, uint32_t n_act, uint32_t route_items, uint32_t* d_order,
                        uint32_t* d_offsets, const Scratch& s, hipStream_t st, bool hot, bool pick = false,
@@ -3938,9 +4166,9 @@
     const RadixPlan& plan = bp.lsd;
     const uint32_t row_step0 = kItems / route_items;
     const bool gaps = lsd_gaps(plan, n, n_act);
-    const bool lhot = hot && gaps && s.lsd_hot;
-    const bool lpick = pick && gaps && s.lsd_hot;
-    const uint32_t* hw = hot_cur(s);
+    const bool lhot = hot && gaps && s.lsd_hot && lsd_set_plan(plan);
+    const bool lpick = pick && gaps && s.lsd_hot && lsd_set_plan(plan);
+    const uint32_t* hw = s.lsd_hot ? lsd_set_cur(s) : nullptr;
     uint2* pbuf[2] = {s.pairs_a, s.pairs_b};
     uint8_t* dig = reinterpret_cast<uint8_t*>(s.sorted_keys);
     bool have_dig = false;
@@ -3949,11 +4177,13 @@
     const uint32_t ntiles12 = ceil_div(n, kRouteThreads * kItems12);
     const uint32_t ntl = t12 ? ntiles12 : ntiles;
     for (int p = 0; p < plan.passes; ++p) {
-        const uint32_t bins = 1u << plan.bits[p];
+        const bool hp = p == 0 && lhot;
+        const uint32_t pbits = hp ? 9u : (uint32_t)plan.bits[p];
+        const uint32_t bins = 1u << pbits;
         const uint32_t row_step = (p == 0) ? row_step0 : 1u;
         const uint32_t ntp = p == 0 ? ntiles : ntl;
         const uint32_t nrows = (p == 0) ? nrows0 : ntl;
-        const uint32_t* n_dev = (p > 0 && lhot) ? s.lsd_hot + 2 : nullptr;
+        const uint32_t* n_dev = (p > 0 && lhot) ? s.lsd_hot + kLsdSetNp : nullptr;
         if (p > 0 && t12)
             hipLaunchKernelGGL((k_hist_dig8_wave<3, 1>), dim3(ceil_div(ntl, kWaves)), dim3(256), 0, st, dig, n, bins, ntl,
                                s.tile_cnt, n_dev);
@@ -3963,18 +4193,18 @@
         else if (p > 0)
             hipLaunchKernelGGL(k_hist_pairs<false>, dim3(ntiles), dim3(256), 0, st, pbuf[(p - 1) & 1], n, n_act,
                                (uint32_t)plan.shift[p], bins, s.tile_cnt, nullptr, nullptr, n_dev);
-        col_scan(s.tile_hist, nrows, bins, row_step, s, st, (p == 0 && lhot) ? s.hot_rows : nullptr, 0, 0, p == 0 && self_cols);
-        if (p == 0 && lhot)
-            hipLaunchKernelGGL(k_lsd_hot_prep, dim3(1), dim3(64), 0, st, hw, s.col_tot + bins, n, s.lsd_hot);
+        col_scan(s.tile_hist, nrows, bins, row_step, s, st, nullptr, 0, 0, p == 0 && self_cols);
+        if (hp)
+            hipLaunchKernelGGL(k_lsd_set_prep, dim3(1), dim3(256), 0, st, hw, s.col_tot, n, s.lsd_hot);
         const bool last = p == plan.passes - 1;
         const bool wdig = !last && plan.bits[p + 1] <= 8;
         const void* kin = (p == 0) ? static_cast<const void*>(d_act) : static_cast<const void*>(pbuf[(p - 1) & 1]);
-        const int out = !last ? (wdig ? OUT_PAIR_DIG : OUT_LSD_PAIR) : gaps ? OUT_FINAL_GAPS : OUT_FINAL;
+        const int out = hp ? OUT_PAIR_DIG_SET : !last ? (wdig ? OUT_PAIR_DIG : OUT_LSD_PAIR)
+                           : lhot ? OUT_FINAL_GAPS_SET : gaps ? OUT_FINAL_GAPS : OUT_FINAL;
         const uint32_t dsel = wdig ? (uint32_t)plan.shift[p + 1] | ((uint32_t)plan.bits[p + 1] << 8) : 0u;
-        const bool hp = p == 0 && lhot;
-        launch_pass(host_rm(s.device), plan.bits[p], p == 0 ? IN_ACT : IN_PAIR, out, kin, n, n_act, (uint32_t)plan.shift[p],
+        launch_pass(host_rm(s.device), (int)pbits, p == 0 ? IN_ACT : IN_PAIR, out, kin, n, n_act, (uint32_t)plan.shift[p],
                     s.tile_hist, row_step, ntp, pbuf[p & 1], d_order, wdig ? reinterpret_cast<uint32_t*>(dig) : s.sorted_keys,
-                    st, hp ? hw : nullptr, hp ? s.hot_rows : nullptr, hp ? s.idx_a : nullptr, d_offsets, nb, s.gap_q, s.gap_cap,
+                    st, lhot ? hw : nullptr, nullptr, hp ? s.idx_a : nullptr, d_offsets, nb, s.gap_q, s.gap_cap,
                     dsel, (p > 0 && lhot) ? s.lsd_hot : nullptr, (p > 0 && t12) ? kItems12 : kItems);
         have_dig = wdig;
     }
@@ -3996,16 +4226,16 @@
         hipLaunchKernelGGL(k_offsets_tail, dim3(bins), dim3(256), 0, st, s.col_tot, s.sorted_keys + (size_t)ntiles * bins,
                            (uint32_t)plan.bits[lp], (uint32_t)plan.shift[lp], nb, d_offsets, s.gap_q, s.gap_cap);
         if (lhot) {
-            hipLaunchKernelGGL(k_lsd_hot_fix, dim3(std::min<uint32_t>(ceil_div(nb, 256u * 16u), 2048u)), dim3(256), 0, st, d_offsets,
-                               nb, s.lsd_hot);
-            hipLaunchKernelGGL(k_hot_tail, dim3(std::min<uint32_t>(ceil_div(n / 4u, 256u * kTailUnroll), 2048u)), dim3(256), 0,
-                               st, hw, s.lsd_hot + 1, n, n_act + 1, s.idx_a, d_offsets, d_order);
+            hipLaunchKernelGGL(k_lsd_set_fix, dim3(std::min<uint32_t>(ceil_div(nb, 256u * 16u), 2048u)), dim3(256), 0, st, d_offsets,
+                               nb, hw, s.lsd_hot);
+            hipLaunchKernelGGL(k_lsd_set_tail, dim3(std::min<uint32_t>(ceil_div(n, 256u * kTailUnroll), 2048u)), dim3(256), 0,
+                               st, hw, s.lsd_hot, n, n_act + 1, s.idx_a, d_offsets, d_order);
         }
         if (lpick) {
-            hipLaunchKernelGGL(k_lsd_pick, dim3(std::min<uint32_t>(ceil_div(n_act + 1u, 256u * 16u), 512u)), dim3(256), 0, st,
-                               d_offsets, n_act + 1u, s.pick_word);
-            hipLaunchKernelGGL(k_lsd_pick_finish, dim3(1), dim3(64), 0, st, s.pick_word, n, s.hot + ((s.hot_parity + 1u) & 1u),
-                               s.hot_host_dev);
+            hipLaunchKernelGGL(k_lsd_set_pick, dim3(std::min<uint32_t>(ceil_div(n_act + 1u, 256u * 16u), 1024u)), dim3(256), 0, st,
+                               d_offsets, n_act + 1u, n, s.lsd_hot);
+            hipLaunchKernelGGL(k_lsd_set_pick_finish, dim3(1), dim3(256), 0, st, s.lsd_hot,
+                               s.lsd_hot + ((s.hot_parity + 1u) & 1u) * kLsdSetSlotWords, s.hot_host_dev);
             s.hot_parity ^= 1u;
         }
         return (int)hipGetLastError();
@@ -4098,17 +4328,22 @@
     const uint32_t nwg = ceil_div(n, kRouteThreads * items);
     const RouteHist rh = route_hist(n_act);
     if (ev_begin) (void)hipEventRecord((hipEvent_t)ev_begin, st);
-    const bool hist = buckets && rh.on;
-    const bool pick = hist && hot_path_on(n, n_act, s);
-    const bool hot = pick && hot_known(s);
-    const uint32_t* hw = hot ? hot_cur(s) : nullptr;
-    uint32_t* hr = hot ? s.hot_rows : nullptr;
+    const bool bhist = buckets && rh.on;
+    const bool lsd = !make_bucket_plan(n_act).two_level;
+    const bool pick = bhist && !(lsd && sw && sw->n) && hot_path_on(n, n_act, s);
+    const bool hot = pick && hot_known(s, n_act);
+    const bool lset = hot && lsd, sep = lset && !ORL_LSD_SET_FUSED;
+    const bool hist = bhist && !sep;
+    const uint32_t* hw = lset ? lsd_set_cur(s) : hot ? hot_cur(s) : nullptr;
+    uint32_t* hr = hot && !lset ? s.hot_rows : nullptr;
     uint16_t* th = hist ? s.tile_cnt : nullptr;
-    const uint32_t bins = hist ? rh.bins : 1u, shift = hist ? rh.shift : 0u;
-    if (d_in_act && hist) return (int)hipErrorInvalidValue;
-#define ORL_ROUTE_L(H, W, Q, C, LR) hipLaunchKernelGGL((k_route<H, W, Q, C, LR>), dim3(nwg), dim3(kRouteThreads), 0, st, d_params,\
+    const uint32_t bins = !hist ? 1u : lset ? 512u : rh.bins, shift = hist && !lset ? rh.shift : 0u;
+    if (d_in_act && bhist) return (int)hipErrorInvalidValue;
+#define ORL_ROUTE_S(H, W, Q, C, LR, S) hipLaunchKernelGGL((k_route<(S && H != 0 && !C) ? 9 : H, W, Q, C, LR, (S && H != 0 && !C)>), dim3(nwg), \
+                                                   dim3(kRouteThreads), 0, st, d_params,                                              \
                                                    dv.dir, dv.mask, dv.cache, dv.cmask, dv.probe, dv.probe_bad, d_in,                 \
                                                    (uint32_t)n, excl, d_route, d_act, th, bins, shift, items, hw, hr, d_in_act)
+#define ORL_ROUTE_L(H, W, Q, C, LR) do { if (lset && hist) ORL_ROUTE_S(H, W, Q, C, LR, true); else ORL_ROUTE_S(H, W, Q, C, LR, false); } while (0)
 #define ORL_ROUTE_C(H, W, Q, C) do { if (dv.lru) ORL_ROUTE_L(H, W, Q, C, true); else ORL_ROUTE_L(H, W, Q, C, false); } while (0)
 #define ORL_ROUTE(H, W, Q) do { if (H == 0 && d_in_act) ORL_ROUTE_C(0, W, Q, true); else ORL_ROUTE_C(H, W, Q, false); } while (0)
 #define ORL_ROUTE_W(H, Q) do { if (fmt == 16) ORL_ROUTE(H, 16, Q); else if (fmt == 8) ORL_ROUTE(H, 8, Q); else ORL_ROUTE(H, 32, Q); } while (0)
@@ -4126,9 +4361,11 @@
 #undef ORL_ROUTE_SL
     } else if (dv.probe8) {
         const ProbeSlot* p8 = static_cast<const ProbeSlot*>(dv.probe8);
-#define ORL_ROUTE8L(H, W, C, LR) hipLaunchKernelGGL((k_route<H, W, 8, C, LR>), dim3(nwg), dim3(kRouteThreads), 0, st, d_params,   \
+#define ORL_ROUTE8S(H, W, C, LR, S) hipLaunchKernelGGL((k_route<(S && H != 0 && !C) ? 9 : H, W, 8, C, LR, (S && H != 0 && !C)>), dim3(nwg), \
+                                                dim3(kRouteThreads), 0, st, d_params,                                                \
                                                 dv.dir, dv.mask, dv.cache, dv.cmask, p8, nullptr, d_in, (uint32_t)n, excl, d_route,  \
                                                 d_act, th, bins, shift, items, hw, hr, d_in_act)
+#define ORL_ROUTE8L(H, W, C, LR) do { if (lset && hist) ORL_ROUTE8S(H, W, C, LR, true); else ORL_ROUTE8S(H, W, C, LR, false); } while (0)
 #define ORL_ROUTE8C(H, W, C) do { if (dv.lru) ORL_ROUTE8L(H, W, C, true); else ORL_ROUTE8L(H, W, C, false); } while (0)
 #define ORL_ROUTE8(H, W) do { if (H == 0 && d_in_act) ORL_ROUTE8C(0, W, true); else ORL_ROUTE8C(H, W, false); } while (0)
         if (hist) {
@@ -4139,6 +4376,7 @@
 #undef ORL_ROUTE8
 #undef ORL_ROUTE8C
 #undef ORL_ROUTE8L
+#undef ORL_ROUTE8S
     } else if (dv.probe) {
         if (hist) ORL_ROUTE_W(kMaxDigitBits, 16); else ORL_ROUTE_W(0, 16);
     } else {
@@ -4148,11 +4386,15 @@
 #undef ORL_ROUTE
 #undef ORL_ROUTE_C
 #undef ORL_ROUTE_L
+#undef ORL_ROUTE_S
     if (ev_end) (void)hipEventRecord((hipEvent_t)ev_end, st);
+    if (sep)
+        hipLaunchKernelGGL((k_hist_pairs<true, true>), dim3(ceil_div(n, kTile)), dim3(256), 0, st, d_act, (uint32_t)n, n_act, 0u,
+                           512u, s.tile_cnt, lsd_set_cur(s), nullptr);
     int e = (int)hipGetLastError();
     if (e) return e;
     if (!buckets) return 0;
-    return bucket_after_route(d_act, (uint32_t)n, n_act, items, d_order, d_offsets, s, st, hot, pick);
+    return bucket_after_route(d_act, (uint32_t)n, n_act, sep ? kItems : items, d_order, d_offsets, s, st, hot, pick);
 }
 
 int launch_fanout_route_bucket(const RouteParams* d_params, const DirView& dv, const orl_msg_hdr* d_direct, size_t n_direct,
@@ -4386,8 +4628,11 @@
     const RouteHist rh = route_hist(n_act);
     const uint32_t ntiles = ceil_div(n, kTile);
     const bool pick = rh.on && hot_path_on(n, n_act, s);
-    const bool hot = pick && hot_known(s);
-    if (rh.on)
+    const bool hot = pick && hot_known(s, n_act);
+    if (hot && !make_bucket_plan(n_act).two_level)
+        hipLaunchKernelGGL((k_hist_pairs<true, true>), dim3(ntiles), dim3(256), 0, st, d_act, (uint32_t)n, n_act, 0u, 512u,
+                           s.tile_cnt, lsd_set_cur(s), nullptr);
+    else if (rh.on)
         hipLaunchKernelGGL(k_hist_pairs<true>, dim3(ntiles), dim3(256), 0, st, d_act, (uint32_t)n, n_act, rh.shift, rh.bins,
                            s.tile_cnt, hot ? hot_cur(s) : nullptr, hot ? s.hot_rows : nullptr);
     int e = (int)hipGetLastError();
```
